# marcinp7/music-style-transfer

Hardware: AMD Instinct MI355X
Metric: style-transfer opt iters/sec (higher is better)
Workload: dtype f32; 1 GPU; one 30 s clip per GPU (BASELINE.json configs[1]): piano-roll C=4,R=16,T=4 (+percussion), full widths (980325 params), fwd+loss+bwd every step, Adam+StepLR every iter_size steps; clips_per_gpu=1, iter_size=2, hip_graph=True, graphs=one joint graph, accumulation=2 concurrent streams, launches_per_pass=77, parallelism=single GPU

## Files before the change

### __graft_entry__.py

```python
import os
import subprocess
import sys

ROOT = os.path.dirname(os.path.abspath(__file__))
PKG = os.path.join(ROOT, 'music-style-transfer_amd')
CSRC = os.path.join(PKG, 'csrc')
BUILD = os.path.join(PKG, 'build')
LIB = os.path.join(PKG, 'libmst_amd.so')
SOURCES = ['gemm', 'lstm', 'combine', 'notes', 'loss_optim', 'plan', 'audio', 'conv', 'lin']
for p in (ROOT, PKG):
    if p not in sys.path:
        sys.path.insert(0, p)


def _hipcc():
    for c in (os.environ.get('HIPCC'), '/opt/rocm/bin/hipcc', 'hipcc'):
        if c and (os.path.isabs(c) and os.path.exists(c) or not os.path.isabs(c)):
            return c
    raise RuntimeError('hipcc not found')


def _stale(target, deps):
    return not os.path.exists(target) or any(os.path.getmtime(d) > os.path.getmtime(target) for d in deps)


def build(force=False):
    os.makedirs(BUILD, exist_ok=True)
    hipcc = _hipcc()
    headers = [os.path.join(CSRC, 'mst_common.h'), os.path.join(ROOT, 'include', 'mst_amd.h')]
    procs, objs = [], []
    for s in SOURCES:
        src, obj = os.path.join(CSRC, s + '.hip'), os.path.join(BUILD, s + '.o')
        objs.append(obj)
        if force or _stale(obj, [src] + headers):
            cmd = [hipcc, '--offload-arch=gfx950', '-O3', '-std=c++17', '-fPIC', '-c', src, '-o', obj]
            procs.append((s, subprocess.Popen(cmd, stdout=subprocess.PIPE, stderr=subprocess.STDOUT)))
    for s, p in procs:
        out, _ = p.communicate()
        if p.returncode:
            raise RuntimeError(f'hipcc failed on {s}.hip:\n{out.decode()}')
    if force or _stale(LIB, objs):
        subprocess.run([hipcc, '--offload-arch=gfx950', '-shared', '-fPIC', '-o', LIB] + objs, check=True)
    import style
    from style import _native
    _native.Native(LIB)


def smoke():
    import numpy as np
    import torch
    from oracle import style_oracle as so
    from tools.synth import synth_clip
    from style import _native as nat
    if not os.path.exists(LIB):
        build()
    assert torch.cuda.is_available(), 'smoke() needs cuda:0'
    dev = torch.device('cuda:0')
    native = nat.get()
    C, R, T = 2, 2, 4
    dims = nat.Dims(C=C, R=R, T=T, beat=64, bar=128, nrf=8, style=256, melody=8, rhythm=32, instr=51,
                    n_instruments=41, has_unpitched=1)
    table = native.param_table(dims)
    g = torch.Generator().manual_seed(0)
    flat = torch.zeros(native.param_floats(dims))
    named = {}
    for name, off, shape in table:
        n = int(np.prod(shape))
        fan = shape[1] if len(shape) > 1 else shape[0]
        flat[off:off + n] = (torch.rand(n, generator=g) * 2 - 1) / fan ** 0.5
        named[name] = flat[off:off + n].view(*shape).clone().requires_grad_(True)
    clip = synth_clip(5, C, R, T, True)
    _, ref_losses = so.iteration(named, clip)
    plan = native.plan(dims, dev)
    plan.set_inputs(mode=clip['mode'], bpm=clip['bpm'], instr=clip['instruments_features'],
                    used=clip['used_instruments'], bpm_target=float(clip['bpm_int']))
    params = flat.to(dev)
    gparams = torch.zeros_like(params)
    losses = torch.zeros(nat.N_LOSSES, device=dev)
    plan.train_iteration(params, gparams, clip['pitched'].to(dev), clip['unpitched'].to(dev), losses)
    torch.cuda.synchronize()
    got = losses.cpu()
    for i, k in enumerate(nat.LOSS_KEYS):
        assert abs(float(got[i]) - ref_losses[k]) < 1e-4, (k, float(got[i]), ref_losses[k])
    gref = torch.cat([(named[n].grad if named[n].grad is not None else torch.zeros_like(named[n])).reshape(-1)
                      for n, _, _ in table])
    err = float((gparams.cpu() - gref).norm() / gref.norm())
    assert err < 1e-4, err
    print(f'smoke ok: total loss {float(got[0]):.6f} (oracle {ref_losses["total"]:.6f}), grad rel-L2 {err:.2e}')


if __name__ == '__main__':
    build()
    print('built', LIB)
```

### include/mst_amd.h

```cpp
#ifndef MST_AMD_H
#define MST_AMD_H
#include <stdint.h>

#ifdef __cplusplus
extern "C" {
#endif

typedef enum {
    MST_OK = 0,
    MST_ERR_ARG = -1,
    MST_ERR_UNSUPPORTED = -2,
    MST_ERR_LAUNCH = -3,
    MST_ERR_ALLOC = -4,
} mst_status;

typedef struct {
    int32_t C, R, T;
    int32_t beat, bar, nrf;
    int32_t style, melody, rhythm;
    int32_t instr;
    int32_t n_instruments;
    int32_t has_unpitched;
    int32_t clips;
} mst_dims;
// ... 39 lines not shown
enum { MST_DEV_OK = 0, MST_DEV_LSTM_TIMEOUT = 1  };
int32_t mst_plan_status(const mst_plan* p, float* ws, int32_t clear, int32_t* status, mst_stream stream);

int32_t mst_forward(const mst_plan* p, int32_t stage_mask, const float* params, float* ws,
                    const float* pitched, const float* unpitched, mst_stream stream);

int32_t mst_backward(const mst_plan* p, int32_t stage_mask, const float* params, float* gparams,
                     float* ws, const float* pitched, const float* unpitched, mst_stream stream);
int32_t mst_zero_grads(const mst_plan* p, int32_t stage_mask, float* ws, mst_stream stream);
int64_t mst_plan_zero_floats(const mst_plan* p, int32_t stage_mask);

#define MST_LOSS_SAVED 512
int64_t mst_loss_scratch_floats(void);
int32_t mst_total_loss_fwd(const float* pitched_pred, const float* pitched_target, int64_t n_pitched_pos,
                           const float* unpitched_pred, const float* unpitched_target, int64_t n_unpitched_pos,
                           const float* instr_logits, const float* instr_target, int32_t n_instr,
                           const float* mode_logits, const float* mode_target,
                           const float* bpm_pred, const float* bpm_target,
                           int32_t normalize, float* losses, float* saved, float* scratch, mst_stream stream);
int32_t mst_total_loss_bwd(const float* pitched_pred, const float* pitched_target, int64_t n_pitched_pos,
                           const float* unpitched_pred, const float* unpitched_target, int64_t n_unpitched_pos,
                           const float* instr_logits, const float* instr_target, int32_t n_instr,
                           const float* mode_logits, const float* mode_target,
                           const float* bpm_pred, const float* bpm_target,
                           const float* saved, const float* grad_losses,
                           float* g_pitched, float* g_unpitched, float* g_instr, float* g_mode, float* g_bpm,
                           mst_stream stream);

int32_t mst_train_iteration(const mst_plan* p, const float* params, float* gparams, float* ws,
                            const float* pitched, const float* unpitched, float* losses, mst_stream stream);

#define MST_MAX_XCHG 8
int32_t mst_tiled_phase_count(const mst_plan* p);
int32_t mst_tiled_phase(const mst_plan* p, int32_t phase, const float* params, float* gparams, float* ws,
                        const float* pitched, const float* unpitched, float* losses, int32_t is_root,
                        mst_stream stream, int64_t xoff[MST_MAX_XCHG], int64_t xlen[MST_MAX_XCHG], int32_t* nx);

int32_t mst_adam_step(float* params, float* grads, float* exp_avg, float* exp_avg_sq, int64_t n,
                      float* state, double lr0, double beta1, double beta2, double eps,
                      int32_t step_size, double gamma, int32_t zero_grad, mst_stream stream);

int32_t mst_adam_step2(float* params, float* grads, float* grads2, float* exp_avg, float* exp_avg_sq, int64_t n,
                       float* state, double lr0, double beta1, double beta2, double eps,
                       int32_t step_size, double gamma, int32_t zero_grad, mst_stream stream);

#define MST_GUARD_WORDS 8
int64_t mst_grad_guard_scratch_bytes(int64_t n);
int32_t mst_grad_norm(const float* grads, const float* grads2 , int64_t n, void* scratch, float* norm,
                      mst_stream stream);
int32_t mst_grad_norms(const float* grads, const float* grads2 , const int64_t* offsets, const int64_t* lengths,
                       int32_t count, float* norms, mst_stream stream);
int32_t mst_adam_step_guarded(float* params, float* grads, float* grads2 , float* exp_avg, float* exp_avg_sq,
                              int64_t n, float* state, float* guard, void* scratch, double lr0, double beta1, double beta2,
                              double eps, int32_t step_size, double gamma, double max_norm ,
                              int32_t skip_nonfinite, int32_t zero_grad, mst_stream stream);

int32_t mst_hard_output(float* x, float* out, int64_t n_pos, int32_t nfeat, mst_stream stream);

int32_t mst_clip_scatter(const int32_t* cells, const float* feats, const int32_t* counts, int32_t capacity, int32_t n_clips,
                         int64_t n_cells, int32_t nfeat, float* out, mst_stream stream);

typedef struct { int32_t first, count, src_bars, r0; } mst_window;
int32_t mst_clip_window(const int32_t* cells, const float* feats, const mst_window* win, int32_t n_clips, int32_t channels,
                        int32_t bars, int64_t bar_cells, int32_t nfeat, float* out, mst_stream stream);

enum { MST_ROLL_NONZERO = 0, MST_ROLL_HARD = 1 };
int64_t mst_roll_slices(int64_t n_cells);
int32_t mst_roll_count(const float* x, int64_t n_cells, int32_t nfeat, int32_t mode, int32_t* ws, mst_stream stream);
int32_t mst_roll_compact(const float* x, int64_t n_cells, int32_t nfeat, int32_t mode, const int32_t* ws,
                         int64_t capacity, int32_t* cells, float* feats, mst_stream stream);

#define MST_METRIC_WORDS 8
int64_t mst_roll_metrics_scratch_bytes(int64_t n_groups, int64_t group_cells);
int32_t mst_roll_metrics(const float* pred, const float* target, int64_t n_groups, int64_t group_cells,
                         int32_t nfeat, void* scratch, double* out, mst_stream stream);

int64_t mst_eval_scratch_bytes(const mst_plan* p);
int32_t mst_eval_iteration(const mst_plan* p, const float* params, float* ws, const float* pitched,
                           const float* unpitched, float* losses, double* metrics, void* scratch, mst_stream stream);

int32_t mst_plan_step_count(const mst_plan* p, int32_t stage_mask, int32_t backward);
int32_t mst_plan_step_info(const mst_plan* p, int32_t stage_mask, int32_t backward, int32_t* info );
int32_t mst_plan_step_carried(const mst_plan* p, int32_t stage_mask, int32_t backward, int32_t* carried);
int32_t mst_plan_step_gemms(const mst_plan* p, int32_t stage_mask, int32_t backward, int32_t step, int32_t* out, int32_t cap);
int32_t mst_plan_time_steps(const mst_plan* p, int32_t stage_mask, int32_t backward, const float* params,
                            float* gparams, float* ws, const float* pitched, const float* unpitched,
                            mst_stream stream, int32_t reps, float* ms, int32_t* kind, double* flops, double* bytes);

typedef struct mst_audio_plan mst_audio_plan;
mst_audio_plan* mst_audio_plan_create(int32_t n_fft , int32_t hop, int64_t n_samples, int32_t* status);
void mst_audio_plan_destroy(mst_audio_plan* p);
int32_t mst_audio_plan_info(const mst_audio_plan* p, int64_t out[6]);
int32_t mst_audio_stft(const mst_audio_plan* p, const float* audio, float* spec, float* mag, mst_stream stream);
int32_t mst_audio_gram(const mst_audio_plan* p, const float* feat, float* gram, float* ws, mst_stream stream);
int32_t mst_audio_style_iteration(const mst_audio_plan* p, float* x, const float* gram_style, float* grad, float* exp_avg,
                                  float* exp_avg_sq, float* state, float* ws, float* loss, double lr, mst_stream stream);

int32_t mst_debug_slab_columns_disjoint(int64_t off_x, int32_t width_x, int64_t off_y, int32_t width_y, int32_t ld);

const char* mst_version(void);

#ifdef __cplusplus
}
#endif
#endif
```

### music-style-transfer_amd/csrc/combine.hip

```cpp
#include "mst_common.h"

template <int MC = COMBINE_MAXC>
__device__ __forceinline__ void block_sum_multi(float* vals, int nv, float (*part)[COMBINE_MAXC + 1], float* red) {
    const int lane = threadIdx.x & 63, wv = threadIdx.x >> 6;
#pragma unroll
    for (int v = 0; v <= MC; ++v) {
        if (v < nv) {
            float x = vals[v];
#pragma unroll
            for (int o = 32; o > 0; o >>= 1) x += __shfl_xor(x, o);
            if (lane == 0) part[wv][v] = x;
        }
    }
    __syncthreads();
    if ((int)threadIdx.x < nv) red[threadIdx.x] = (part[0][threadIdx.x] + part[1][threadIdx.x]) + (part[2][threadIdx.x] + part[3][threadIdx.x]);
    __syncthreads();
}

__device__ __forceinline__ int64_t elem_off(const CombineDesc& d, int e) {
    const unsigned r = (unsigned)e / (unsigned)d.cols;
    return (int64_t)r * d.ld + (int)((unsigned)e - r * (unsigned)d.cols);
}

__global__ __launch_bounds__(256) void combine_sumsq_kernel(const CombineDesc* __restrict__ descs, Bases b) {
    const CombineDesc d = descs[blockIdx.y];
    if ((int)blockIdx.x >= d.nblk) return;
    __shared__ float part[4][COMBINE_MAXC + 1];
    __shared__ float red[COMBINE_MAXC + 1];
    const float* x = b.p[SP_WS] + d.x_off;
    const int64_t n = (int64_t)d.rows * d.cols;
    float acc[COMBINE_MAXC + 1];
#pragma unroll
    for (int c = 0; c <= COMBINE_MAXC; ++c) acc[c] = 0.f;
    for (int e = blockIdx.x * 256 + threadIdx.x; e < (int)n; e += d.nblk * 256) {
        const int64_t eo = elem_off(d, e);
#pragma unroll
        for (int c = 0; c < COMBINE_MAXC; ++c) {
            if (c < d.Cn) { const float v = x[(int64_t)c * d.cs + eo]; acc[c] = fmaf(v, v, acc[c]); }
        }
    }
    block_sum_multi(acc, d.Cn, part, red);
    if ((int)threadIdx.x < d.Cn) b.p[SP_TMP][d.part_off + blockIdx.x * (COMBINE_MAXC + 1) + threadIdx.x] = red[threadIdx.x];
}

__global__ __launch_bounds__(256) void combine_apply_kernel(const CombineDesc* __restrict__ descs, Bases b) {
    const CombineDesc d = descs[blockIdx.y];
    if ((int)blockIdx.x >= d.nblk) return;
    __shared__ float nrm[COMBINE_MAXC + 1];
    __shared__ float part[4][COMBINE_MAXC + 1];
    __shared__ float red[COMBINE_MAXC + 1];
    float* ws = b.p[SP_WS];
    float* tmp = b.p[SP_TMP];
    {
        float vals[COMBINE_MAXC + 1];
#pragma unroll
        for (int c = 0; c <= COMBINE_MAXC; ++c)
            vals[c] = (c < d.Cn && (int)threadIdx.x < d.nblk) ? tmp[d.part_off + threadIdx.x * (COMBINE_MAXC + 1) + c] : 0.f;
        block_sum_multi(vals, d.Cn, part, red);
    }
    if ((int)threadIdx.x < d.Cn) nrm[threadIdx.x] = sqrtf(1.f + red[threadIdx.x]);
    __syncthreads();
    if (threadIdx.x == 0) {
        float S = 0.f;
        for (int c = 0; c < d.Cn; ++c) S += nrm[c];
        nrm[COMBINE_MAXC] = S;
    }
    __syncthreads();
    if (blockIdx.x == 0 && (int)threadIdx.x <= d.Cn)
        tmp[d.stats_off + threadIdx.x] = (int)threadIdx.x < d.Cn ? nrm[threadIdx.x] : nrm[COMBINE_MAXC];
    const float S = nrm[COMBINE_MAXC];
    const int64_t n = (int64_t)d.rows * d.cols;
    for (int e = blockIdx.x * 256 + threadIdx.x; e < (int)n; e += d.nblk * 256) {
        const int64_t eo = elem_off(d, e);
        float acc = 0.f;
        for (int c = 0; c < d.Cn; ++c) acc += ws[d.x_off + (int64_t)c * d.cs + eo] * nrm[c];
        ws[d.out_off + e] = acc / S;
    }
}

__global__ __launch_bounds__(256) void combine_bwd_reduce_kernel(const CombineDesc* __restrict__ descs, Bases b) {
    const CombineDesc d = descs[blockIdx.y];
    if ((int)blockIdx.x >= d.nblk) return;
    __shared__ float part[4][COMBINE_MAXC + 1];
    __shared__ float red[COMBINE_MAXC + 1];
    const float* ws = b.p[SP_WS];
    const float* gr = b.p[SP_GRAD];
    const int64_t n = (int64_t)d.rows * d.cols;
    float acc[COMBINE_MAXC + 1];
#pragma unroll
    for (int c = 0; c <= COMBINE_MAXC; ++c) acc[c] = 0.f;
    for (int e = blockIdx.x * 256 + threadIdx.x; e < (int)n; e += d.nblk * 256) {
        const int64_t eo = elem_off(d, e);
        const float g = gr[d.gout_off + e];
#pragma unroll
        for (int c = 0; c < COMBINE_MAXC; ++c) {
            if (c < d.Cn) acc[c] = fmaf(g, ws[d.x_off + (int64_t)c * d.cs + eo], acc[c]);
        }
        acc[COMBINE_MAXC] = fmaf(g, ws[d.out_off + e], acc[COMBINE_MAXC]);
    }
    float vals[COMBINE_MAXC + 1];
#pragma unroll
    for (int c = 0; c < COMBINE_MAXC; ++c) vals[c] = acc[c];
    vals[COMBINE_MAXC] = 0.f;
#pragma unroll
    for (int c = 0; c <= COMBINE_MAXC; ++c) if (c == d.Cn) vals[c] = acc[COMBINE_MAXC];
    block_sum_multi(vals, d.Cn + 1, part, red);
    if ((int)threadIdx.x <= d.Cn) b.p[SP_TMP][d.part_off + blockIdx.x * (COMBINE_MAXC + 1) + threadIdx.x] = red[threadIdx.x];
}

__global__ __launch_bounds__(256) void combine_bwd_apply_kernel(const CombineDesc* __restrict__ descs, Bases b) {
    const CombineDesc d = descs[blockIdx.y];
    if ((int)blockIdx.x >= d.nblk) return;
    __shared__ float coef[COMBINE_MAXC + 1];
    __shared__ float nc_s[COMBINE_MAXC + 1];
    const float* ws = b.p[SP_WS];
    float* gr = b.p[SP_GRAD];
    const float* tmp = b.p[SP_TMP];
    __shared__ float part[4][COMBINE_MAXC + 1];
    {
        float vals[COMBINE_MAXC + 1];
#pragma unroll
        for (int c = 0; c <= COMBINE_MAXC; ++c)
            vals[c] = (c <= d.Cn && (int)threadIdx.x < d.nblk) ? tmp[d.part_off + threadIdx.x * (COMBINE_MAXC + 1) + c] : 0.f;
        block_sum_multi(vals, d.Cn + 1, part, coef);
    }
    if ((int)threadIdx.x <= d.Cn) nc_s[threadIdx.x] = tmp[d.stats_off + threadIdx.x];
    __syncthreads();
    const float S = nc_s[d.Cn];
    const float bsum = coef[d.Cn];
    __shared__ float fa_s[COMBINE_MAXC], fb_s[COMBINE_MAXC];
    if ((int)threadIdx.x < d.Cn) {
        const float nc = nc_s[threadIdx.x];
        fa_s[threadIdx.x] = nc / S; fb_s[threadIdx.x] = ((coef[threadIdx.x] - bsum) / S) / nc;
    }
    __syncthreads();
    const int64_t n = (int64_t)d.rows * d.cols;
    for (int e = blockIdx.x * 256 + threadIdx.x; e < (int)n; e += d.nblk * 256) {
        const int64_t eo = elem_off(d, e);
        const float g = gr[d.gout_off + e];
        for (int c = 0; c < d.Cn; ++c) {
            const float x = ws[d.x_off + (int64_t)c * d.cs + eo];
            float* gx = gr + d.gx_off + (int64_t)c * d.cs + eo;
            const float v = fmaf(g, fa_s[c], fb_s[c] * x);
            *gx = d.first ? v : *gx + v;
        }
    }
}

template <int MC>
__global__ __launch_bounds__(256) void combine_small_fwd_kernel(const CombineDesc* __restrict__ descs, Bases b) {
    const CombineDesc d = descs[blockIdx.x];
    __shared__ float nrm[COMBINE_MAXC + 1];
    __shared__ float part[4][COMBINE_MAXC + 1];
    __shared__ float red[COMBINE_MAXC + 1];
    float* ws = b.p[SP_WS];
    float* tmp = b.p[SP_TMP];
    const int n = d.rows * d.cols;
    float acc[MC + 1];
#pragma unroll
    for (int c = 0; c <= MC; ++c) acc[c] = 0.f;
    constexpr int U = MC <= 4 ? 4 : 1;
    for (int e0 = threadIdx.x; e0 < n; e0 += 256 * U) {
        float v[U][MC];
#pragma unroll
        for (int u = 0; u < U; ++u) {
            const int e = e0 + 256 * u;
            const bool ok = e < n;
            const int64_t eo = elem_off(d, ok ? e : 0);
#pragma unroll
            for (int c = 0; c < MC; ++c) v[u][c] = (ok && c < d.Cn) ? ws[d.x_off + (int64_t)c * d.cs + eo] : 0.f;
        }
#pragma unroll
        for (int u = 0; u < U; ++u) {
#pragma unroll
            for (int c = 0; c < MC; ++c) acc[c] = fmaf(v[u][c], v[u][c], acc[c]);
        }
    }
    block_sum_multi<MC>(acc, d.Cn, part, red);
    if ((int)threadIdx.x < d.Cn) nrm[threadIdx.x] = sqrtf(1.f + red[threadIdx.x]);
    __syncthreads();
    if (threadIdx.x == 0) {
        float S = 0.f;
        for (int c = 0; c < d.Cn; ++c) S += nrm[c];
        nrm[COMBINE_MAXC] = S;
    }
    __syncthreads();
    if ((int)threadIdx.x <= d.Cn) tmp[d.stats_off + threadIdx.x] = (int)threadIdx.x < d.Cn ? nrm[threadIdx.x] : nrm[COMBINE_MAXC];
    const float S = nrm[COMBINE_MAXC];
    for (int e0 = threadIdx.x; e0 < n; e0 += 256 * U) {
        float v[U][MC];
#pragma unroll
        for (int u = 0; u < U; ++u) {
            const int e = e0 + 256 * u;
            const bool ok = e < n;
            const int64_t eo = elem_off(d, ok ? e : 0);
#pragma unroll
            for (int c = 0; c < MC; ++c) v[u][c] = (ok && c < d.Cn) ? ws[d.x_off + (int64_t)c * d.cs + eo] : 0.f;
        }
#pragma unroll
        for (int u = 0; u < U; ++u) {
            const int e = e0 + 256 * u;
            float a = 0.f;
#pragma unroll
            for (int c = 0; c < MC; ++c) if (c < d.Cn) a += v[u][c] * nrm[c];
            if (e < n) ws[d.out_off + e] = a / S;
        }
    }
}

template <int MC>
__global__ __launch_bounds__(256) void combine_small_bwd_kernel(const CombineDesc* __restrict__ descs, Bases b) {
    const CombineDesc d = descs[blockIdx.x];
    __shared__ float coef[COMBINE_MAXC + 1];
    __shared__ float nc_s[COMBINE_MAXC + 1];
    __shared__ float part[4][COMBINE_MAXC + 1];
    const float* ws = b.p[SP_WS];
    float* gr = b.p[SP_GRAD];
    const float* tmp = b.p[SP_TMP];
    const int n = d.rows * d.cols;
    float acc[MC + 1];
#pragma unroll
    for (int c = 0; c <= MC; ++c) acc[c] = 0.f;
    constexpr int U = MC <= 4 ? 4 : 1;
    for (int e0 = threadIdx.x; e0 < n; e0 += 256 * U) {
        float v[U][MC], g[U], o[U];
#pragma unroll
        for (int u = 0; u < U; ++u) {
            const int e = e0 + 256 * u;
            const bool ok = e < n;
            const int64_t eo = elem_off(d, ok ? e : 0);
            g[u] = ok ? gr[d.gout_off + e] : 0.f;
            o[u] = ok ? ws[d.out_off + e] : 0.f;
#pragma unroll
            for (int c = 0; c < MC; ++c) v[u][c] = (ok && c < d.Cn) ? ws[d.x_off + (int64_t)c * d.cs + eo] : 0.f;
        }
#pragma unroll
        for (int u = 0; u < U; ++u) {
            if (e0 + 256 * u < n) {
#pragma unroll
                for (int c = 0; c < MC; ++c) if (c < d.Cn) acc[c] = fmaf(g[u], v[u][c], acc[c]);
                acc[MC] = fmaf(g[u], o[u], acc[MC]);
            }
        }
    }
    float vals[MC + 1];
#pragma unroll
    for (int c = 0; c < MC; ++c) vals[c] = acc[c];
    vals[MC] = 0.f;
#pragma unroll
    for (int c = 0; c <= MC; ++c) if (c == d.Cn) vals[c] = acc[MC];
    block_sum_multi<MC>(vals, d.Cn + 1, part, coef);
    if ((int)threadIdx.x <= d.Cn) nc_s[threadIdx.x] = tmp[d.stats_off + threadIdx.x];
    __syncthreads();
    const float S = nc_s[d.Cn];
    const float bsum = coef[d.Cn];
    float fa[MC], fb[MC];
#pragma unroll
    for (int c = 0; c < MC; ++c) {
        const float nc = c < d.Cn ? nc_s[c] : 1.f;
        fa[c] = nc / S; fb[c] = c < d.Cn ? ((coef[c] - bsum) / S) / nc : 0.f;
    }
    for (int e0 = threadIdx.x; e0 < n; e0 += 256 * U) {
        float x[U][MC], old[U][MC], g[U];
        int64_t eo[U];
#pragma unroll
        for (int u = 0; u < U; ++u) {
            const int e = e0 + 256 * u;
            const bool ok = e < n;
            eo[u] = elem_off(d, ok ? e : 0);
            g[u] = ok ? gr[d.gout_off + e] : 0.f;
#pragma unroll
            for (int c = 0; c < MC; ++c) {
                const bool okc = ok && c < d.Cn;
                x[u][c] = okc ? ws[d.x_off + (int64_t)c * d.cs + eo[u]] : 0.f;
                old[u][c] = (okc && !d.first) ? gr[d.gx_off + (int64_t)c * d.cs + eo[u]] : 0.f;
            }
        }
#pragma unroll
        for (int u = 0; u < U; ++u) {
            if (e0 + 256 * u < n) {
#pragma unroll
                for (int c = 0; c < MC; ++c) {
                    if (c < d.Cn) {
                        const float v = fmaf(g[u], fa[c], fb[c] * x[u][c]);
                        gr[d.gx_off + (int64_t)c * d.cs + eo[u]] = d.first ? v : old[u][c] + v;
                    }
                }
            }
        }
    }
}

int launch_combine_fwd(const CombineDesc* dev, int count, int max_nblk, int all_small, Bases b, hipStream_t s) {
    if (count <= 0) return 0;
    if (all_small) {
        if (all_small == 2) hipLaunchKernelGGL(combine_small_fwd_kernel<4>, dim3(count), dim3(256), 0, s, dev, b);
        else hipLaunchKernelGGL(combine_small_fwd_kernel<COMBINE_MAXC>, dim3(count), dim3(256), 0, s, dev, b);
        return (int)hipGetLastError();
    }
    hipLaunchKernelGGL(combine_sumsq_kernel, dim3(max_nblk, count), dim3(256), 0, s, dev, b);
    hipLaunchKernelGGL(combine_apply_kernel, dim3(max_nblk, count), dim3(256), 0, s, dev, b);
    return (int)hipGetLastError();
}

int launch_combine_bwd(const CombineDesc* dev, int count, int max_nblk, int all_small, Bases b, hipStream_t s) {
    if (count <= 0) return 0;
    if (all_small) {
        if (all_small == 2) hipLaunchKernelGGL(combine_small_bwd_kernel<4>, dim3(count), dim3(256), 0, s, dev, b);
        else hipLaunchKernelGGL(combine_small_bwd_kernel<COMBINE_MAXC>, dim3(count), dim3(256), 0, s, dev, b);
        return (int)hipGetLastError();
    }
    hipLaunchKernelGGL(combine_bwd_reduce_kernel, dim3(max_nblk, count), dim3(256), 0, s, dev, b);
    hipLaunchKernelGGL(combine_bwd_apply_kernel, dim3(max_nblk, count), dim3(256), 0, s, dev, b);
    return (int)hipGetLastError();
}

int launch_combine_phase(const CombineDesc* dev, int nblk, int which, Bases b, hipStream_t s) {
    if (which == 0) hipLaunchKernelGGL(combine_sumsq_kernel, dim3(nblk, 1), dim3(256), 0, s, dev, b);
    else if (which == 1) hipLaunchKernelGGL(combine_apply_kernel, dim3(nblk, 1), dim3(256), 0, s, dev, b);
    else if (which == 2) hipLaunchKernelGGL(combine_bwd_reduce_kernel, dim3(nblk, 1), dim3(256), 0, s, dev, b);
    else hipLaunchKernelGGL(combine_bwd_apply_kernel, dim3(nblk, 1), dim3(256), 0, s, dev, b);
    return (int)hipGetLastError();
}

__global__ __launch_bounds__(256) void copy_rows_kernel(const CopyDesc* __restrict__ dp, int backward, Bases b) {
    const CopyDesc d = dp[0];
    const int total = d.na * d.nb * d.cols;
    for (int e = blockIdx.x * 256 + threadIdx.x; e < total; e += gridDim.x * 256) {
        const int j = e % d.cols, ab = e / d.cols, bb = ab % d.nb, a = ab / d.nb;
        const int64_t so = d.src_off + (int64_t)a * d.src_sa + (int64_t)bb * d.src_sb + j;
        const int64_t dof = d.dst_off + (int64_t)a * d.dst_sa + (int64_t)bb * d.dst_sb + j;
        if (!backward) b.p[SP_WS][dof] = b.p[SP_WS][so];
        else { float* g = b.p[SP_GRAD] + so; const float v = b.p[SP_GRAD][dof]; *g = d.first ? v : *g + v; }
    }
}

int launch_copy_rows(const CopyDesc* dev, const CopyDesc& host, int backward, Bases b, hipStream_t s) {
    const int total = host.na * host.nb * host.cols;
    int nb = (total + 255) / 256;
    if (nb > 1024) nb = 1024;
    if (nb < 1) return 0;
    hipLaunchKernelGGL(copy_rows_kernel, dim3(nb), dim3(256), 0, s, dev, backward, b);
    return (int)hipGetLastError();
}

__global__ __launch_bounds__(64) void fold_kernel(const FoldDesc* __restrict__ dp, int spread, Bases b) {
    const FoldDesc d = dp[0];
    float* part = b.p[d.space] + d.part_off;
    float* sum = b.p[SP_TMP] + d.sum_off;
    for (int c = threadIdx.x; c < d.ncols; c += 64) {
        if (!spread) {
            float a = 0.f;
            for (int r = 0; r < d.nrows; ++r) a += part[(int64_t)r * d.row_stride + (int64_t)c * d.col_stride];
            sum[c] = a;
        } else {
            part[(int64_t)c * d.col_stride] = sum[c];
            for (int r = 1; r < d.nrows; ++r) part[(int64_t)r * d.row_stride + (int64_t)c * d.col_stride] = 0.f;
        }
    }
}

int launch_fold(const FoldDesc* dev, int spread, Bases b, hipStream_t s) {
    hipLaunchKernelGGL(fold_kernel, dim3(1), dim3(64), 0, s, dev, spread, b);
    return (int)hipGetLastError();
}
```

### music-style-transfer_amd/csrc/gemm.hip

```cpp
#include "mst_common.h"

__device__ __forceinline__ float act_fwd(int act, float z, int col) {
    if (act == ACT_LEAKY) return z > 0.f ? z : z * LEAKY;
    if (act == ACT_SIGOUT) { float s = 1.f / (1.f + expf(-z)); return col == 0 ? 6.f * s : s; }
    if (act == ACT_BPM) { float s = 1.f / (1.f + expf(-z)); return s * 150.f + 50.f; }
    return z;
}

__device__ __forceinline__ float act_bwd(int act, float y, int col) {
    if (act == ACT_LEAKY) return y > 0.f ? 1.f : LEAKY;
    if (act == ACT_SIGOUT) return col == 0 ? y * (1.f - y * (1.f / 6.f)) : y * (1.f - y);
    if (act == ACT_BPM) { float s = (y - 50.f) * (1.f / 150.f); return 150.f * s * (1.f - s); }
    return 1.f;
}

typedef const MST_GLOBAL_AS float* gcptr;
#define GEMM_PAD 1

template <int KIND>
__device__ __forceinline__ int off_of(const Operand& o, int i, int j, bool& ok) {
    if constexpr (KIND == OPK_DENSE) {
        return i * (int)o.si + j * (int)o.sj;
    } else if constexpr (KIND == OPK_ACTGRAD) {
        return o.transposed ? j * o.ld + i : i * o.ld + j;
    } else if constexpr (KIND == OPK_IM2COL) {
        const int p = i >> 3, oc = i & 7;
        const int f = j / (CONV_K * NPF), rem = j - f * (CONV_K * NPF);
        const int e = (NDEG * oc - CONV_PAD) * NPF + rem;
        ok = ok & (e >= 0) & (e < NPN * NPF);
        return p * (NF * NPN * NPF) + f * (NPN * NPF) + e;
    } else if constexpr (KIND == OPK_PERMW) {
        if (o.pb == CONV_K && o.pc == NPF) {
            constexpr int BC = CONV_K * NPF;
            const int a = i / BC, rem = i - a * BC;
            const int bb = rem / NPF, c = rem - bb * NPF;
            return j * o.ld + a * BC + c * CONV_K + bb;
        }
        if (o.pb == NUN && o.pc == NUF) {
            constexpr int BC = NUN * NUF;
            const int a = i / BC, rem = i - a * BC;
            const int bb = rem / NUF, c = rem - bb * NUF;
            return j * o.ld + a * BC + c * NUN + bb;
        }
        const int bc = o.pb * o.pc;
        const int a = i / bc, rem = i - a * bc;
        const int bb = rem / o.pc, c = rem - bb * o.pc;
        return j * o.ld + a * bc + c * o.pb + bb;
    } else {
        return (j >> 3) * (o.oc * NOCT) + i * NOCT + (j & 7);
    }
}

template <int OK>
__device__ __forceinline__ void store_out(const GemmDesc& d, float* cbase, const float* bias, int m, int n, int split, float acc) {
    const OutSpec& o = d.out;
    if constexpr (OK == OUT_STORE) {
        float v = acc;
        if (bias) v += o.bias_div > 0 ? bias[(unsigned)((m / o.bias_div) * o.bias_ld + n)] : bias[n];
        cbase[(unsigned)(m * o.ldc + n)] = act_fwd(o.act, v, n);
    } else if constexpr (OK == OUT_ACCUM) {
        float* c = cbase + (unsigned)(m * o.ldc + n);
        *c = o.first ? acc : *c + acc;
    } else if constexpr (OK == OUT_CONV) {
        cbase[(unsigned)((m >> 3) * o.ldc + n * NOCT + (m & 7))] = act_fwd(ACT_LEAKY, acc + bias[n], 0);
    } else if constexpr (OK == OUT_SLAB) {
        const unsigned idx = n < o.wcols ? (unsigned)(m * o.wcols + n) : (unsigned)(d.M * o.wcols + m);
        cbase[(int64_t)split * o.slab_stride + idx] = acc;
    } else {
        unsigned idx;
        if (n < o.wcols) {
            int a, bb, c, bc;
            if (o.pb == CONV_K && o.pc == NPF) { bc = CONV_K * NPF; a = n / (CONV_K * NPF); const int rem = n - a * (CONV_K * NPF); bb = rem / NPF; c = rem - bb * NPF; }
            else if (o.pb == NUN && o.pc == NUF) { bc = NUN * NUF; a = n / (NUN * NUF); const int rem = n - a * (NUN * NUF); bb = rem / NUF; c = rem - bb * NUF; }
            else { bc = o.pb * o.pc; a = n / bc; const int rem = n - a * bc; bb = rem / o.pc; c = rem - bb * o.pc; }
            idx = (unsigned)(m * o.wcols + a * bc + c * o.pb + bb);
        } else {
            idx = (unsigned)(d.M * o.wcols + m);
        }
        cbase[(int64_t)split * o.slab_stride + idx] = acc;
    }
}

template <int AK, int BKIND, int OK, int AKF, int BKF, int KD>
// ... 449 lines not shown
                for (int kk = 0; kk < MF_KD / 2; ++kk) {
                    const int k = kk * 2 + (lane >> 5);
                    acc = __builtin_amdgcn_mfma_f32_32x32x2f32(As[k][bm * 32 + (lane & 31)], Bs[k][bn * 32 + (lane & 31)], acc, 0, 0, 0);
                }
            } else {
                for (int kk = kk0; kk < min(kk0 + per, live); ++kk) {
                    const int k = kk * 2 + (lane >> 5);
                    acc = __builtin_amdgcn_mfma_f32_32x32x2f32(As[k][bm * 32 + (lane & 31)], Bs[k][bn * 32 + (lane & 31)], acc, 0, 0, 0);
                }
            }
        }
        if (last_k) {
            if (nsl > 1) {
                float* part = smem + buf * 2 * TILE_F;
                MST_LDS_BARRIER();
                if (ks > 0) {
#pragma unroll
                    for (int r = 0; r < 16; ++r) part[((ks - 1) * nblk + blk) * 1024 + r * 64 + lane] = acc[r];
                }
                MST_LDS_BARRIER();
                if (ks == 0) {
                    for (int q = 0; q < nsl - 1; ++q) {
#pragma unroll
                        for (int r = 0; r < 16; ++r) acc[r] += part[(q * nblk + blk) * 1024 + r * 64 + lane];
                    }
                }
            }
            const int n = tn * MF_BN + bn * 32 + (lane & 31);
            if ((ks == 0) & (tm * MF_BM + bm * 32 < M) & (tn * MF_BN + bn * 32 < N)) {
#pragma unroll
                for (int r = 0; r < 16; ++r) {
                    const int m = tm * MF_BM + bm * 32 + (r & 3) + 8 * (r >> 2) + 4 * (lane >> 5);
                    if (m < M && n < N) store_out<OK>(d, cbase, bias, m, n, split, acc[r]);
                }
            }
#pragma unroll
            for (int r = 0; r < 16; ++r) acc[r] = 0.f;
        }
        if (!more) break;
        t = nt; kt = nkt; buf ^= 1;
    }
}

__global__ __launch_bounds__(MF_THREADS, 4) void gemm_mfma_kernel(const GemmDesc* __restrict__ descs, const int* __restrict__ owner, int count, int blocks_per_clip, Bases b) {
    __shared__ float smem[2 * 2 * MF_KD * (MF_BM + GEMM_PAD)];
    float (*As)[MF_BM + GEMM_PAD] = reinterpret_cast<float (*)[MF_BM + GEMM_PAD]>(smem);
    float (*Bs)[MF_BN + GEMM_PAD] = reinterpret_cast<float (*)[MF_BN + GEMM_PAD]>(smem + MF_KD * (MF_BM + GEMM_PAD));
    const int clip = blockIdx.x / blocks_per_clip, lb = blockIdx.x - clip * blocks_per_clip;
    const int lo = owner[lb];
    const GemmDesc d = descs[clip * count + lo];
    const int local = lb - d.blk_begin;
    const int ntile = ((d.M + MF_BM - 1) / MF_BM) * ((d.N + MF_BN - 1) / MF_BN);
    const int run = d.run > 0 ? d.run : 1, nruns = (ntile + run - 1) / run;
    const int split = local / nruns, t_begin = (local - split * nruns) * run, t_end = min(ntile, t_begin + run);
    switch (d.variant) {
    case GV_LIN_FWD: gemm_fast_body<OPK_DENSE, OUT_STORE, 1, 1>(d, b, t_begin, t_end, split, smem); break;
    case GV_LIN_DW: gemm_fast_body<OPK_ACTGRAD, OUT_SLAB, 0, 0>(d, b, t_begin, t_end, split, smem); break;
    case GV_LIN_DW_PERM: gemm_fast_body<OPK_ACTGRAD, OUT_PERMW_SLAB, 0, 0>(d, b, t_begin, t_end, split, smem); break;
    case GV_LIN_DA: gemm_fast_body<OPK_ACTGRAD, OUT_ACCUM, 1, 0>(d, b, t_begin, t_end, split, smem); break;
    case GV_HH_DW: gemm_fast_body<OPK_DENSE, OUT_SLAB, 0, 0>(d, b, t_begin, t_end, split, smem); break;
    case GV_LIN_DA_RAW: gemm_fast_body<OPK_DENSE, OUT_ACCUM, 1, 0>(d, b, t_begin, t_end, split, smem); break;
    default:
        for (int tile = t_begin; tile < t_end; ++tile) {
            if (tile > t_begin) __syncthreads();
            if (d.variant == GV_LIN_FWD_PERM) gemm_mfma_body<OPK_DENSE, OPK_PERMW, OUT_STORE, 1, 1>(d, b, tile, split, As, Bs);
            else if (d.variant == GV_CONV_FWD) gemm_mfma_body<OPK_IM2COL, OPK_PERMW, OUT_CONV, 1, 1>(d, b, tile, split, As, Bs);
            else if (d.variant == GV_CONV_DW) {
                if (d.fold_rows) gemm_mfma_body<OPK_CONVGRAD, OPK_IM2COL, OUT_PERMW_SLAB, 1, 0, true>(d, b, tile, split, As, Bs);
                else gemm_mfma_body<OPK_CONVGRAD, OPK_IM2COL, OUT_PERMW_SLAB, 1, 0>(d, b, tile, split, As, Bs);
            }
        }
        break;
    }
}

int gemm_tile_edge(int mfma) { return mfma ? MF_BM : GEMM_BM; }
int gemm_blocks(const GemmDesc& g, int mfma) {
    const int edge = gemm_tile_edge(mfma);
    const int ntile = ((g.M + edge - 1) / edge) * ((g.N + edge - 1) / edge);
    const int run = (mfma && g.run > 1) ? g.run : 1;
    return ((ntile + run - 1) / run) * g.ksplit;
}

template <int WV> __device__ __forceinline__ void gather_rows(const GatherDesc& d, const int blk, const int nblk, const Bases& b);
__device__ __forceinline__ void segred_group(const SegRedDesc* __restrict__ descs, const int members, const int clip, const int lb, const int t, const Bases& b);

__global__ __launch_bounds__(GEMM_THREADS) void gemm_kernel(const GemmDesc* __restrict__ descs, const int* __restrict__ owner, int count, int blocks_per_clip, Bases b, GemmRiders r) {
    constexpr int TILE_F = GEMM_BK * (GEMM_BM + GEMM_PAD), RED_F = (GEMM_THREADS / 64) * GEMM_BM * GEMM_BN;
    __shared__ float smem[(2 * TILE_F > RED_F) ? 2 * TILE_F : RED_F];
    float (*As)[GEMM_BM + GEMM_PAD] = reinterpret_cast<float (*)[GEMM_BM + GEMM_PAD]>(smem);
    float (*Bs)[GEMM_BN + GEMM_PAD] = reinterpret_cast<float (*)[GEMM_BN + GEMM_PAD]>(smem + TILE_F);
    const int clip = blockIdx.x / blocks_per_clip;
    int lb = blockIdx.x - clip * blocks_per_clip;
    const int seg_blocks = (r.seg_groups + 3) >> 2, gat_blocks = r.gat_members * r.gat_blocks;
    if (lb < seg_blocks) {
        const int grp = lb * 4 + (threadIdx.x >> 8);
        if (grp < r.seg_groups) segred_group(r.segreds, r.seg_members, clip, grp, threadIdx.x & 255, b);
        return;
    }
    lb -= seg_blocks;
    if (lb < gat_blocks) {
        const int m = lb / r.gat_blocks;
        gather_rows<GATHER_RIDER_ROWS>(r.gathers[clip * r.gat_members + m], lb - m * r.gat_blocks, r.gat_blocks, b);
        return;
    }
    lb -= gat_blocks;
    const int lo = owner[lb];
    const GemmDesc d = descs[clip * count + lo];
    const int local = lb - d.blk_begin;
    const int ntile = ((d.M + GEMM_BM - 1) / GEMM_BM) * ((d.N + GEMM_BN - 1) / GEMM_BN);
    const int tile = local % ntile, split = local / ntile;
#define GEMM_CASE(V, A_, B_, O_, AF_, BF_)                                                          \
    case (V) * 3 + 0: gemm_body<A_, B_, O_, AF_, BF_, 32>(d, b, tile, split, As, Bs); break;           \
    case (V) * 3 + 1: gemm_body<A_, B_, O_, AF_, BF_, 64>(d, b, tile, split, As, Bs); break;           \
    case (V) * 3 + 2: gemm_body<A_, B_, O_, AF_, BF_, 128>(d, b, tile, split, As, Bs); break;
    switch (d.variant * 3 + d.kdsel) {
        GEMM_CASE(GV_LIN_FWD, OPK_DENSE, OPK_DENSE, OUT_STORE, 1, 1)
        GEMM_CASE(GV_LIN_FWD_PERM, OPK_DENSE, OPK_PERMW, OUT_STORE, 1, 1)
        GEMM_CASE(GV_LIN_DW, OPK_ACTGRAD, OPK_DENSE, OUT_SLAB, 0, 0)
        GEMM_CASE(GV_LIN_DW_PERM, OPK_ACTGRAD, OPK_DENSE, OUT_PERMW_SLAB, 0, 0)
        GEMM_CASE(GV_LIN_DA, OPK_ACTGRAD, OPK_DENSE, OUT_ACCUM, 1, 0)
        GEMM_CASE(GV_CONV_FWD, OPK_IM2COL, OPK_PERMW, OUT_CONV, 1, 1)
        GEMM_CASE(GV_CONV_DW, OPK_CONVGRAD, OPK_IM2COL, OUT_PERMW_SLAB, 1, 0)
        GEMM_CASE(GV_HH_DW, OPK_DENSE, OPK_DENSE, OUT_SLAB, 0, 0)
        GEMM_CASE(GV_LIN_DA_RAW, OPK_DENSE, OPK_DENSE, OUT_ACCUM, 1, 0)
    default: break;
    }
#undef GEMM_CASE
}

int gemm_variant(const GemmDesc& g) {
    const int a = g.A.kind, bk = g.B.kind, o = g.out.kind;
    if (a == OPK_DENSE && bk == OPK_DENSE && o == OUT_STORE) return GV_LIN_FWD;
    if (a == OPK_DENSE && bk == OPK_PERMW && o == OUT_STORE) return GV_LIN_FWD_PERM;
    if (a == OPK_ACTGRAD && bk == OPK_DENSE && o == OUT_SLAB) return GV_LIN_DW;
    if (a == OPK_ACTGRAD && bk == OPK_DENSE && o == OUT_PERMW_SLAB) return GV_LIN_DW_PERM;
    if (a == OPK_ACTGRAD && bk == OPK_DENSE && o == OUT_ACCUM) return GV_LIN_DA;
    if (a == OPK_IM2COL && bk == OPK_PERMW && o == OUT_CONV) return GV_CONV_FWD;
    if (a == OPK_CONVGRAD && bk == OPK_IM2COL && o == OUT_PERMW_SLAB) return GV_CONV_DW;
    if (a == OPK_DENSE && bk == OPK_DENSE && o == OUT_SLAB) return GV_HH_DW;
    if (a == OPK_DENSE && bk == OPK_DENSE && o == OUT_ACCUM) return GV_LIN_DA_RAW;
    return -1;
}

int gemm_rider_blocks(const GemmRiders& r) { return (r.seg_groups + 3) / 4 + r.gat_members * r.gat_blocks; }

int launch_gemm(const GemmDesc* dev_descs, const int* dev_owner, int members, int blocks_per_clip, int clips, int mfma, Bases b, hipStream_t s, const GemmRiders* riders) {
    if (members <= 0 || blocks_per_clip <= 0 || clips <= 0) return 0;
    GemmRiders r = riders ? *riders : GemmRiders{};
    if (mfma && gemm_rider_blocks(r)) return (int)hipErrorInvalidValue;
    blocks_per_clip += gemm_rider_blocks(r);
    if (mfma) hipLaunchKernelGGL(gemm_mfma_kernel, dim3(blocks_per_clip * clips), dim3(MF_THREADS), 0, s, dev_descs, dev_owner, members, blocks_per_clip, b);
    else hipLaunchKernelGGL(gemm_kernel, dim3(blocks_per_clip * clips), dim3(GEMM_THREADS), 0, s, dev_descs, dev_owner, members, blocks_per_clip, b, r);
    return (int)hipGetLastError();
}

template <int WV>
__device__ __forceinline__ void gather_rows(const GatherDesc& d, const int blk, const int nblk, const Bases& b) {
    const int lane = threadIdx.x & 63, wv = (threadIdx.x >> 6) & (WV - 1);
    for (int row = blk * WV + wv; row < d.rows; row += nblk * WV) {
        unsigned t = (unsigned)row;
        int rc[4];
        rc[3] = t % (unsigned)d.d[3]; t /= (unsigned)d.d[3];
        rc[2] = t % (unsigned)d.d[2]; t /= (unsigned)d.d[2];
        rc[1] = t % (unsigned)d.d[1]; rc[0] = t / (unsigned)d.d[1];
        float* out = b.p[SP_WS] + d.out_off + (int64_t)row * d.K;
        if (d.sum) {
            for (int w = lane; w < d.K; w += 64) {
                float a = 0.f;
                for (int sIdx = 0; sIdx < d.nseg; ++sIdx) {
                    const Seg& sg = d.seg[sIdx];
                    const int srow = rc[0] * sg.s[0] + rc[1] * sg.s[1] + rc[2] * sg.s[2] + rc[3] * sg.s[3];
                    a += b.p[sg.space][sg.off + (int64_t)srow * sg.ld + w];
                }
                out[w] = a;
            }
            continue;
        }
        for (int sIdx = 0; sIdx < d.nseg; ++sIdx) {
            const Seg& sg = d.seg[sIdx];
            const int srow = rc[0] * sg.s[0] + rc[1] * sg.s[1] + rc[2] * sg.s[2] + rc[3] * sg.s[3];
            const float* src = b.p[sg.space] + sg.off + (int64_t)srow * sg.ld;
            for (int w = lane; w < sg.width; w += 64) out[sg.start + w] = src[w];
        }
    }
}

__global__ __launch_bounds__(256) void gather_kernel(const GatherDesc* __restrict__ descs, Bases b) {
    gather_rows<4>(descs[blockIdx.y], blockIdx.x, gridDim.x, b);
}

int launch_gather(const GatherDesc* dev, int count, int max_rows, Bases b, hipStream_t s) {
    if (count <= 0) return 0;
    int gx = (max_rows + 3) / 4;
    if (gx > 2048) gx = 2048;
    hipLaunchKernelGGL(gather_kernel, dim3(gx, count), dim3(256), 0, s, dev, b);
    return (int)hipGetLastError();
}

#define SEGRED_CHUNK 64
template <int E, int R>
__device__ __forceinline__ void segred_body(const SegRedDesc& d, const int item, const Bases& b) {
    const int wgrp = (d.width + E - 1) / E;
    if (item >= d.nidx * d.nchunk * wgrp) return;
    const int w = (item % wgrp) * E, ne = min(E, d.width - w);
    int t = item / wgrp;
    const int chunk = t % d.nchunk, idx = t / d.nchunk;
    int kc[4];
    t = idx;
#pragma unroll
    for (int q = 3; q >= 0; --q) { kc[q] = t % d.kd[q]; t /= d.kd[q]; }
    int rd[4], nred = 1;
#pragma unroll
    for (int q = 0; q < 4; ++q) { rd[q] = d.kd[q] == 1 ? d.d[q] : 1; nred *= rd[q]; }
    const int r_begin = chunk * SEGRED_CHUNK, r_end = min(nred, r_begin + SEGRED_CHUNK);
    int cr[4];
    t = r_begin;
#pragma unroll
    for (int q = 3; q >= 0; --q) { cr[q] = t % rd[q]; t /= rd[q]; }
    const float* src = b.p[SP_GRAD] + d.src_off + d.start + w;
    const float* ysrc = b.p[SP_WS] + d.y_off + d.start + w;
    const int64_t s3 = d.src_ld, s2 = s3 * d.d[3], s1 = s2 * d.d[2], s0 = s1 * d.d[1];
    const int64_t w3 = s2 - rd[3] * s3, w2 = s1 - rd[2] * s2, w1 = s0 - rd[1] * s1;
    int64_t roff = (kc[0] + cr[0]) * s0 + (kc[1] + cr[1]) * s1 + (kc[2] + cr[2]) * s2 + (kc[3] + cr[3]) * s3;
    auto offset = [&]() { return roff; };
    auto advance = [&]() {
        roff += s3;
        if (++cr[3] == rd[3]) { cr[3] = 0; roff += w3; if (++cr[2] == rd[2]) { cr[2] = 0; roff += w2; if (++cr[1] == rd[1]) { cr[1] = 0; roff += w1; ++cr[0]; } } }
    };
    float acc[E];
#pragma unroll
    for (int j = 0; j < E; ++j) acc[j] = 0.f;
    typedef float sr_f4 __attribute__((ext_vector_type(4), aligned(4)));
    auto ldE = [&](const float* p, float (&dst)[E]) {
        if (E == 4 && ne == 4) {
            const sr_f4 t = *reinterpret_cast<const sr_f4*>(p);
// ... 154 lines not shown
```

### music-style-transfer_amd/csrc/mst_common.h

```cpp
#pragma once
#include <hip/hip_runtime.h>
#include <stdint.h>

#include "../../include/mst_amd.h"

#ifndef MST_GLOBAL_AS
#define MST_GLOBAL_AS __attribute__((address_space(1)))
#endif
#ifndef MST_CONST_AS
#define MST_CONST_AS __attribute__((address_space(4)))
#endif
#ifndef MST_UNIFORM
#define MST_UNIFORM(x) __builtin_amdgcn_readfirstlane(x)
#endif
#ifndef MST_FAST_EXP
#define MST_FAST_EXP(x) __expf(x)
#define MST_FAST_RCP(x) __builtin_amdgcn_rcpf(x)
#define MST_PIN(x) asm volatile("" : "+v"(x))
#endif
#ifndef MST_PIN_SGPR
#if defined(__AMDGCN__)
#define MST_PIN_SGPR(p) asm volatile("" : "+s"(p))
#else
#define MST_PIN_SGPR(p) ((void)(p))
// ... 19 lines not shown
#define NUF 2
#define NOCT 8
#define NDEG 7
#define NPN 56
#define NUN 47
#define CONV_K 14
#define CONV_PAD 4
#define LEAKY 0.01f

enum { SP_WS = 0, SP_PAR = 1, SP_GPAR = 2, SP_EXT0 = 3, SP_EXT1 = 4, SP_GRAD = 5, SP_TMP = 6, SP_COUNT = 7 };
enum { MST_BF_LOSS_FUSED = 1,
       MST_BF_ALL_STAGES = 2 };
struct Bases { float* p[SP_COUNT]; int32_t flags; };

enum { ACT_NONE = 0, ACT_LEAKY = 1, ACT_SIGOUT = 2, ACT_BPM = 3 };

enum { OPK_DENSE = 0, OPK_ACTGRAD = 2, OPK_IM2COL = 3, OPK_PERMW = 4, OPK_CONVGRAD = 5 };
#define MAX_SEG 6
struct Seg {
    int32_t space, ld, start, width;
    int64_t off;
    int32_t s[4];
};
struct Operand {
    int32_t kind;
    int32_t space;
    int64_t off;
    int64_t si, sj;
    int32_t ones_at;
    int32_t kfast;
    int32_t space2, ld, act, transposed;
    int64_t off2;
    int32_t oc;
    int32_t pb, pc;
};
enum { OUT_STORE = 0, OUT_ACCUM = 1, OUT_CONV = 2, OUT_SLAB = 3, OUT_PERMW_SLAB = 4 };
struct OutSpec {
    int32_t kind, space, ldc, act;
    int64_t off;
    int32_t bias_space;
    int64_t bias_off;
    int64_t slab_stride;
    int32_t first;
    int32_t wcols;
    int32_t pb, pc;
    int32_t bias_div, bias_ld;
};
struct GemmDesc {
    int32_t M, N, K, ksplit;
    int32_t variant;
    int32_t blk_begin;
    int32_t kdsel;
    int32_t run;
    int32_t fold_rows;
    int64_t acs, acs2, bcs;
    int32_t clip_rows;
    Operand A, B;
    OutSpec out;
};

struct GatherDesc {
    int32_t rows, K, nseg;
    int32_t sum;
    int32_t d[4];
    int64_t out_off;
    Seg seg[MAX_SEG];
};

struct SegRedDesc {
    int64_t src_off; int32_t src_ld; int32_t start, width;
    int64_t dst_off; int32_t dst_ld;
    int32_t d[4];
    int32_t s[4];
    int32_t nidx;
    int32_t kd[4];
    int32_t nchunk;
    int64_t part_off;
    int32_t blk_begin;
    int32_t first;
    int32_t act;
    int64_t y_off;
};

struct GemmRiders {
    const SegRedDesc* segreds; int32_t seg_members, seg_groups;
    const GatherDesc* gathers; int32_t gat_members, gat_blocks;
};

struct LstmDesc {
    int32_t B, S, H, reverse;
    int64_t zx_off;
    int64_t whh_off, bhh_off;
    int64_t out_off; int32_t out_ld;
    int64_t gates_off, c_off, hprev_off;
    int64_t tc_off;
    int64_t gout_off;
    int64_t gzx_off;
    int64_t whht_off;
    int32_t multi;
    int64_t xch_off;
    int64_t status_off;
};
#define LSTM_NB 12
#define LSTM_MH 192
#define LSTM_L2H 256
#define LSTM_WH 1024
static inline int lstm_band(int H) { return H <= 64 ? 0 : (H <= LSTM_L2H ? 1 : 2); }
static inline bool lstm_hidden_supported(int H) { return H >= 1 && H <= LSTM_WH; }

#define COMBINE_MAXC 32
#define COMBINE_MAXBLK 256
#define COMBINE_SMALL 4096
struct CombineDesc {
    int32_t Cn, rows, cols, ld;
    int64_t x_off, cs;
    int64_t out_off;
    int64_t stats_off;
    int64_t part_off;
    int64_t gx_off, gout_off;
    int32_t nblk;
    int32_t first;
};

struct NotesDesc {
    int32_t C, Q;
    int32_t W, CW, ML;
    int64_t oct_off, deg_off;
    int64_t rt_oct_off, rt_deg_off;
    int64_t it_oct_off, it_deg_off;
    int64_t x_off; int32_t x_space;
    int64_t mel_off, g_mel_off;
    int64_t wm_off;
    int64_t ml_off;
    int64_t wc_off, bc_off, wl_off, bl_off;
    int64_t out_off;
    int64_t g_out_off, g_oct_off, g_deg_off, g_ml_off;
    int64_t slab_off; int32_t slab_stride; int32_t nblk;
    int64_t itp_oct_off, itp_deg_off, loss_saved_off, loss_gl_off;
    int32_t fhn;
    int32_t nwc;
    int64_t part_off;
    int64_t stats_off;
};

struct ConvDesc {
    int32_t P, clips, OC, splits;
    int64_t rows_per_split;
    int64_t x1_off, clip_stride;
    int64_t wp_off;
    int64_t w_off, b_off;
    int64_t slab_off, slab_stride;
};
int launch_conv_prep(const ConvDesc& d, Bases b, hipStream_t s);
int launch_conv_fwd(const ConvDesc& d, Bases b, hipStream_t s);
int launch_conv_dw(const ConvDesc& d, Bases b, hipStream_t s);

typedef float mst_f32x16 __attribute__((ext_vector_type(16)));
template <int KT, bool M1 = true, bool N1 = true, int PA = 0, int PB = 0>
__device__ __forceinline__ void mst_mfma_ktile_2x2(const float (*As)[PA], const float (*Bs)[PB], int arow, int bcol, int l31, int kh,
                                                   mst_f32x16 (&acc)[2][2]) {
    float a0[2], a1[2], b0[2], b1[2];
    a0[0] = As[kh][arow + l31]; b0[0] = Bs[kh][bcol + l31];
    if (M1) a1[0] = As[kh][arow + 32 + l31];
    if (N1) b1[0] = Bs[kh][bcol + 32 + l31];
#pragma unroll
    for (int s = 0; s < KT / 2; ++s) {
        const int c = s & 1, n = c ^ 1;
        if (s + 1 < KT / 2) {
            const int k = 2 * (s + 1) + kh;
            a0[n] = As[k][arow + l31]; b0[n] = Bs[k][bcol + l31];
            if (M1) a1[n] = As[k][arow + 32 + l31];
            if (N1) b1[n] = Bs[k][bcol + 32 + l31];
        }
        __builtin_amdgcn_sched_barrier(0);
        acc[0][0] = __builtin_amdgcn_mfma_f32_32x32x2f32(a0[c], b0[c], acc[0][0], 0, 0, 0);
        if (N1) acc[0][1] = __builtin_amdgcn_mfma_f32_32x32x2f32(a0[c], b1[c], acc[0][1], 0, 0, 0);
        if (M1) acc[1][0] = __builtin_amdgcn_mfma_f32_32x32x2f32(a1[c], b0[c], acc[1][0], 0, 0, 0);
        if (M1 && N1) acc[1][1] = __builtin_amdgcn_mfma_f32_32x32x2f32(a1[c], b1[c], acc[1][1], 0, 0, 0);
        __builtin_amdgcn_sched_barrier(0);
    }
}


struct LinDesc {
    int32_t rows, K, N, act, xgrad, clips;
    int32_t x_space, x_ld; int64_t x_off, x_cs;
    int32_t y_ld; int64_t y_off, y_cs;
    int64_t gx_cs;
    int64_t w_off, b_off;
    int64_t slab_off, slab_stride, rows_per_split; int32_t splits;
    int32_t first[2];
};
int launch_lin_fwd(const LinDesc& d, Bases b, hipStream_t s);
int launch_lin_dx(const LinDesc& d, Bases b, int first, hipStream_t s);
int launch_lin_dw(const LinDesc& d, Bases b, hipStream_t s);
int lin_dw_tiles(const LinDesc& d);

struct RowLinDesc {
    int32_t rows, kin, nout, act, xgrad;
    int64_t x_off, y_off;
    int64_t w_off, b_off;
    int64_t slab_off; int32_t slab_stride, nblk;
    int32_t first;
};

struct CopyDesc { int64_t src_off, dst_off; int32_t na, nb, cols, src_sa, src_sb, dst_sa, dst_sb, first; };
struct FoldDesc { int32_t space, nrows, row_stride, ncols, col_stride, pad; int64_t part_off, sum_off ; };
int launch_copy_rows(const CopyDesc* dev, const CopyDesc& host, int backward, Bases b, hipStream_t s);
int launch_fold(const FoldDesc* dev, int spread, Bases b, hipStream_t s);
int launch_combine_phase(const CombineDesc* dev, int nblk, int which, Bases b, hipStream_t s);

struct SlabEntry { int64_t dst, src, stride; int32_t count, splits; int32_t reps; int64_t rep_stride; int32_t width, dst_ld; int32_t single;
                   int64_t base;  };
struct SlabBlock { int32_t entry, start; };

struct Sizes {
    int OC, PCE_IL, H, HB;
    int SE_L, SE_IL, SE_ML, SE_BL;
    int ME_BL, ME_BRL, ME_IL, ME_CW, MEL;
    int RH, PRE_BL, PRE_BRL, PRE_CL, PRE_IL, PRE_ML, PRE_BPL, URE_CL;
    int SIM_BL, NRF, SIM_SI, SIM_RI, SIM_SM, SIM_RM, SIM_SB, SIM_RB, NI;
    int PSA_SL, PSA_RL, PSA_IL, PSA_ML, USA_SL, USA_RL;
    int I, STYLE, BAR;
};
Sizes mst_sizes(const mst_dims& d);

enum { GV_LIN_FWD, GV_LIN_FWD_PERM, GV_LIN_DW, GV_LIN_DW_PERM, GV_LIN_DA, GV_CONV_FWD, GV_CONV_DW, GV_HH_DW, GV_LIN_DA_RAW };
int launch_gather(const GatherDesc* dev, int count, int max_rows, Bases b, hipStream_t s);
int gemm_variant(const GemmDesc& g);
int launch_gemm(const GemmDesc* dev_descs, const int* dev_owner, int members, int blocks_per_clip, int clips, int mfma, Bases b, hipStream_t s,
                const GemmRiders* riders = nullptr);
int gemm_rider_blocks(const GemmRiders& r);
int gemm_tile_edge(int mfma);
int gemm_blocks(const GemmDesc& g, int mfma);
int launch_segred(const SegRedDesc* dev_descs, int members, int blocks_per_clip, int clips, int stage2_blocks, Bases b, hipStream_t s);
int launch_segred2(const SegRedDesc* dev_descs, int count, int stage2_blocks, Bases b, hipStream_t s);
int launch_lstm_transpose(const LstmDesc* dev_descs, int count, int maxH, int multi, Bases b, hipStream_t s);
int launch_lstm_fwd(const LstmDesc* dev_descs, int count, int maxB, int maxH, int multi, Bases b, hipStream_t s);
int launch_lstm_bwd(const LstmDesc* dev_descs, int count, int maxB, int maxH, int multi, Bases b, hipStream_t s);
int lstm_multi_blocks_per_cu();
int launch_combine_fwd(const CombineDesc* dev_descs, int count, int max_nblk, int all_small, Bases b, hipStream_t s);
int launch_combine_bwd(const CombineDesc* dev_descs, int count, int max_nblk, int all_small, Bases b, hipStream_t s);
int launch_me_sumsq(const NotesDesc* dev, const NotesDesc& host, int count, Bases b, hipStream_t s);
int launch_me_notes_fwd(const NotesDesc* dev, const NotesDesc& host, int count, Bases b, hipStream_t s);
int launch_me_bwd_reduce(const NotesDesc* dev, const NotesDesc& host, int count, Bases b, hipStream_t s);
int launch_me_notes_bwd(const NotesDesc* dev, const NotesDesc& host, int count, Bases b, hipStream_t s);
int launch_psa_notes_fwd(const NotesDesc* dev, const NotesDesc& host, int count, Bases b, hipStream_t s);
int launch_psa_notes_bwd(const NotesDesc* dev, const NotesDesc& host, int count, Bases b, hipStream_t s);
int psa_bwd_waves(int C);
struct LossBatch { int32_t clips; int64_t ws, grad, tmp, ext0, ext1; };
int loss_fwd_partials(const float* pp, const float* pt, int64_t np, const float* up, const float* ut, int64_t nu, float* scratch,
                      hipStream_t s);
int loss_fwd_tail(int64_t np, int64_t nu, int has_u, const float* il, const float* it, int ni, const float* mlg, const float* mt,
                  const float* bp, const float* bt, int normalize, float* losses, float* saved, float* scratch, hipStream_t s,
                  float* gl_onehot, float* losses_out);
int loss_blocks(int64_t n);
int loss_fwd_batched(const float* pp, const float* pt, int64_t np, const float* up, const float* ut, int64_t nu, const float* il,
                     const float* it, int ni, const float* mlg, const float* mt, const float* bp, const float* bt, int normalize,
                     float* losses, float* saved, float* scratch, LossBatch lb, hipStream_t s,
                     float* gl_onehot ,
                     float* losses_out );
int loss_bwd_batched(const float* pp, const float* pt, int64_t np, const float* up, const float* ut, int64_t nu, const float* il,
                     const float* it, int ni, const float* mlg, const float* mt, const float* bp, const float* bt,
                     const float* saved, const float* gl, float* gp, float* gu, float* gi, float* gm, float* gb, LossBatch lb,
                     hipStream_t s, float info_scale = 1.f );
int launch_roll_metrics(const float* pred, const float* target, int64_t n_groups, int64_t group_cells, int nfeat, int gpc,
                        int64_t pred_cs, int64_t tgt_cs, void* scratch, hipStream_t s);
struct EvalMetricsArgs {
    const void* part_p; int64_t slices_p, cells_p;
    const void* part_u; int64_t slices_u, cells_u;
    int32_t C, ni;
    const float *il, *it, *mlg, *mt, *bp, *bt;
    int64_t ws_stride;
    double* out;
};
int launch_eval_metrics_finish(const EvalMetricsArgs& a, int clips, hipStream_t s);
bool rowlin_supported(int kin, int nout);
int launch_rowlin_fwd(const RowLinDesc* dev, const RowLinDesc& host, int count, Bases b, hipStream_t s);
int launch_rowlin_bwd(const RowLinDesc* dev, const RowLinDesc& host, int count, Bases b, hipStream_t s);
int launch_slab_reduce(const SlabEntry* dev, const SlabBlock* blocks, int nblocks, Bases b, hipStream_t s);
struct ZeroChunk { int64_t off; int32_t len; int32_t pad; };
int launch_zero(const ZeroChunk* dev, int nchunks, int clips, float* grad_base, int64_t clip_stride, hipStream_t s);
bool notes_widths_supported(int W, int CW, int ML);

#define GEMM_BM 32
#define GEMM_BN 32
#define GEMM_BK 128
#define GEMM_THREADS 1024
#define GATHER_RIDER_ROWS (GEMM_THREADS / 64)
```

### music-style-transfer_amd/csrc/plan.hip

```cpp
#include <cmath>
#include <cstdio>
#include <cstdlib>
#include <cstring>
#include <map>
#include <string>
#include <array>
#include <vector>

#include "mst_common.h"

#define MST_ALIGN_UP(n) (((n) + 63) / 64 * 64)

static int mean_size(double a, double b, double factor = 1.0) { return (int)std::ceil(((a + b) / 2.0) * factor); }

Sizes mst_sizes(const mst_dims& d) {
    Sizes z{};
    z.I = d.instr; z.STYLE = d.style; z.BAR = d.bar; z.H = d.beat; z.HB = d.bar / 2; z.RH = d.rhythm;
    z.MEL = d.melody; z.NRF = d.nrf; z.NI = d.n_instruments;
    z.OC = mean_size(NF * NPF, d.beat);
    z.PCE_IL = mean_size(d.instr, d.beat);
    z.SE_L = mean_size(d.bar, d.style);
    z.SE_IL = mean_size(d.instr, d.style, .25);
    z.SE_ML = mean_size(2, d.style, .1);
    z.SE_BL = mean_size(d.style, 1, .05);
// ... 114 lines not shown
    t.lin(m + ".octave_linear", NPF * 6 * NOCT, z.PSA_SL + z.PSA_RL + z.PSA_IL);
    t.lin(m + ".scale_degree_linear", NPF * 6 * NDEG, z.PSA_SL + z.PSA_RL + z.PSA_IL);
    t.lin(m + ".melody_linear", z.PSA_ML, z.MEL);
    t.lin(m + ".linear", NPF, NPF * 6 + z.PSA_ML);
    m = "unpitched_style_applier";
    t.lin(m + ".style_linear", NF * z.USA_SL, z.STYLE);
    t.lin(m + ".rhythm_linear", z.USA_RL, z.RH);
    t.lin(m + ".notes_linear", NUN * NUF * 4, z.USA_SL + z.USA_RL);
    t.lin(m + ".linear", NUF, NUF * 4);
}

static bool widths_supported(const Sizes& z) {
    for (const int h : {z.H, z.HB, z.SE_L, z.SIM_BL, z.NRF})
        if (!lstm_hidden_supported(h)) return false;
    return notes_widths_supported(z.MEL, z.ME_CW, z.PSA_ML);
}

static bool dims_ok(const mst_dims* d) {
    return d && d->C >= 1 && d->C <= COMBINE_MAXC && d->C <= 24 && d->R >= 1 && d->T >= 1 && d->beat >= 1 && d->bar >= 2 &&
           d->bar % 2 == 0 && d->nrf >= 1 && d->style >= 1 && d->melody >= 1 && d->rhythm >= 1 && d->instr >= 1 &&
           d->n_instruments >= 1 && d->clips >= 0 && d->clips <= 4096;
}

extern "C" int32_t mst_param_count(const mst_dims* d) {
    if (!dims_ok(d)) return MST_ERR_ARG;
    ParamTable t; build_params(*d, mst_sizes(*d), t);
    return (int32_t)t.v.size();
}
extern "C" int64_t mst_param_floats(const mst_dims* d) {
    if (!dims_ok(d)) return MST_ERR_ARG;
    ParamTable t; build_params(*d, mst_sizes(*d), t);
    return t.top;
}
extern "C" int32_t mst_param_info(const mst_dims* d, int32_t i, char* name, int32_t cap, int64_t* off, int32_t* ndim,
                                  int32_t shape[3]) {
    if (!dims_ok(d) || !name || !off || !ndim || !shape) return MST_ERR_ARG;
    ParamTable t; build_params(*d, mst_sizes(*d), t);
    if (i < 0 || i >= (int)t.v.size()) return MST_ERR_ARG;
    const PInfo& p = t.v[i];
    snprintf(name, cap, "%s", p.name.c_str());
    *off = p.off; *ndim = p.ndim;
    for (int k = 0; k < 3; ++k) shape[k] = p.shape[k];
    return MST_OK;
}

struct T { int64_t off; int rows, cols, ld; };
struct SegIn { int space; int64_t off; int ld, width; int s[4]; bool grad; };
enum { K_GEMM, K_GATHER, K_SEGRED, K_LSTM_F, K_LSTM_B, K_COMB_F, K_COMB_B, K_ME_F, K_ME_B, K_PSA_F, K_PSA_B, K_LSTM_T, K_ROW_F, K_ROW_B,
       K_ME_SQ, K_ME_RED,
       K_COMB_F1, K_COMB_F2, K_COMB_B1, K_COMB_B2, K_COPY_F, K_COPY_B, K_FOLD, K_SPREAD, K_XCHG,
       K_GEMM_FOLD,
       K_CONV_P, K_CONV_F, K_CONV_W,
       K_LIN_F, K_LIN_A, K_LIN_W,
       K_COUNT };
enum { F_GEMM, F_GATHER, F_SEGRED, F_LSTM, F_COMB, F_NOTES, F_ROWLIN, F_COPY, F_FOLD, F_XCHG, F_CONV, F_LIN };
struct KindInfo { int kind, fam, sched, per_clip, merge; };
static constexpr KindInfo KINDS[] = {
    {K_GEMM, F_GEMM, 1, 1, 1},     {K_GATHER, F_GATHER, 1, 1, 1}, {K_SEGRED, F_SEGRED, 1, 1, 1}, {K_LSTM_F, F_LSTM, 1, 1, 1},
    {K_LSTM_B, F_LSTM, 1, 1, 1},   {K_COMB_F, F_COMB, 1, 1, 1},   {K_COMB_B, F_COMB, 1, 1, 1},   {K_ME_F, F_NOTES, 1, 1, 0},
    {K_ME_B, F_NOTES, 1, 1, 0},    {K_PSA_F, F_NOTES, 1, 1, 0},   {K_PSA_B, F_NOTES, 1, 1, 0},   {K_LSTM_T, F_LSTM, 1, 1, 1},
    {K_ROW_F, F_ROWLIN, 1, 1, 0},  {K_ROW_B, F_ROWLIN, 1, 1, 0},  {K_ME_SQ, F_NOTES, 1, 1, 0},   {K_ME_RED, F_NOTES, 1, 1, 0},
    {K_COMB_F1, F_COMB, 1, 1, 0},  {K_COMB_F2, F_COMB, 1, 1, 0},  {K_COMB_B1, F_COMB, 1, 1, 0},  {K_COMB_B2, F_COMB, 1, 1, 0},
    {K_COPY_F, F_COPY, 0, 0, 0},   {K_COPY_B, F_COPY, 0, 0, 0},   {K_FOLD, F_FOLD, 0, 0, 0},     {K_SPREAD, F_FOLD, 0, 0, 0},
    {K_XCHG, F_XCHG, 0, 0, 0},     {K_GEMM_FOLD, F_GEMM, 1, 0, 1}, {K_CONV_P, F_CONV, 0, 0, 0},  {K_CONV_F, F_CONV, 0, 0, 0},
    {K_CONV_W, F_CONV, 0, 0, 0},   {K_LIN_F, F_LIN, 0, 0, 0},     {K_LIN_A, F_LIN, 0, 0, 0},     {K_LIN_W, F_LIN, 0, 0, 0}};
static constexpr bool kinds_in_order(int i = 0) { return i == K_COUNT || (KINDS[i].kind == i && kinds_in_order(i + 1)); }
static_assert(sizeof(KINDS) / sizeof(KINDS[0]) == K_COUNT && kinds_in_order(), "KINDS[k] describes step kind k, for every k");

template <class D>
static int up(const std::vector<D>& v, D** dev) {
    *dev = nullptr;
    if (v.empty()) return 0;
    if (hipMalloc((void**)dev, v.size() * sizeof(D)) != hipSuccess) return MST_ERR_ALLOC;
    if (hipMemcpy(*dev, v.data(), v.size() * sizeof(D), hipMemcpyHostToDevice) != hipSuccess) return MST_ERR_ALLOC;
    return 0;
}
template <class D> struct DescTable {
    std::vector<D> host, sched;
    D* dev = nullptr;
    int upload() { return up(sched.empty() ? host : sched, &dev); }
    void release() { hipFree(dev); dev = nullptr; }
};

struct Riders { int seg_first = 0, seg_members = 0, seg_groups = 0, seg_stage2 = 0, gat_first = 0, gat_members = 0, gat_rows = 0; };
struct Step { int kind, first, count, a, b, stage; int c = 0; int lvl = 0; int chain = -1; int signal = -1; int wait[3] = {-1, -1, -1};
              int carried = 0; Riders ride; };
struct Acc { int space; int64_t lo, hi; bool w; bool accum = false, dense = true; };
struct Op { int stage; std::vector<Step> fwd, bwd; };

static int stage_idx(int stage) { return stage == MST_STAGE_EXTRACT ? 0 : stage == MST_STAGE_INFO ? 1 : 2; }

struct mst_plan {
    mst_dims d; Sizes z; ParamTable pt;
    DescTable<GemmDesc> gemms; DescTable<GatherDesc> gathers; DescTable<SegRedDesc> segreds; DescTable<LstmDesc> lstms;
    DescTable<CombineDesc> combines; DescTable<NotesDesc> notes; DescTable<RowLinDesc> rowlins;
    DescTable<ConvDesc> convs; DescTable<LinDesc> lins; DescTable<CopyDesc> copies; DescTable<FoldDesc> folds;
    std::vector<SlabEntry> slabs[3];
    std::vector<Op> ops;
    std::vector<Step> sched[2];
    std::vector<Step> sched_all[2];
    const std::vector<Step>& list(int mask, int backward) const { return mask == MST_STAGE_ALL ? sched_all[backward ? 1 : 0] : sched[backward ? 1 : 0]; }
    std::vector<int> s_gemm_owner; int* d_gemm_owner = nullptr;
    std::map<std::string, T> named;
    int64_t act_top = 0, tmp_top = 0;
    SlabEntry* d_slabs[3] = {nullptr, nullptr, nullptr};
    std::vector<SlabBlock> slab_blocks[3]; SlabBlock* d_slab_blocks[3] = {nullptr, nullptr, nullptr};
    std::vector<SlabEntry> slabs_all; SlabEntry* d_slabs_all = nullptr;
    std::vector<SlabBlock> slab_blocks_all; SlabBlock* d_slab_blocks_all = nullptr;
    bool slabs_all_ok = false;
    T t_losses, t_saved, t_gl; int64_t loss_scratch = 0;
    std::vector<ZeroChunk> zero_stage[3], zero_all;
    ZeroChunk* d_zero_stage[3] = {nullptr, nullptr, nullptr}; ZeroChunk* d_zero_all = nullptr;
    int err = 0;
    mst_plan_options opt{};
    int mfma = 0;

    bool tiled() const { return opt.tile_rows > 0; }
    bool mixes() const { return !mfma && !tiled() && opt.branches != 1 && !opt.no_merge; }
    int Rl() const { return tiled() ? opt.tile_rows : d.R; }
    int P() const { return d.C * Rl() * d.T; }
    int Q() const { return Rl() * d.T; }
    struct Xchg { int space; int64_t off; int32_t len; };
    std::vector<Xchg> xchgs;
    bool tags_in_zero = false;
    std::vector<ZeroChunk> zero_fwd; ZeroChunk* d_zero_fwd = nullptr;
    int64_t loss_sum_off = 0;
    int loss_fold[2] = {-1, -1};
    struct Phase { int what; int pass; int begin, end; int nx; int xchg[MST_MAX_XCHG]; };
    std::vector<Phase> phases;
    int K() const { return d.clips > 1 ? d.clips : 1; }
    static int device_cus() {
#ifdef HIPSIM
        return 16;
#else
        int dev = 0, cus = 0;
        if (hipGetDevice(&dev) != hipSuccess || hipDeviceGetAttribute(&cus, hipDeviceAttributeMultiprocessorCount, dev) != hipSuccess) return 0;
        return cus;
#endif
    }
    static int coresident_slots() {
        const int per_cu = lstm_multi_blocks_per_cu();
        return per_cu > 1 ? (per_cu - 1) * device_cus() : 0;
    }
    int64_t status_off = 0;
    enum { N_SIDE = 3, N_SETS = 4, N_EVENTS = 96 };
    struct SideSet { hipStream_t owner = nullptr; bool used = false; hipStream_t side[N_SIDE] = {}; hipEvent_t ev_fork = nullptr, ev_join[N_SIDE] = {}, ev[N_EVENTS] = {}; };
    mutable SideSet sides[N_SETS];
    bool branches = false;
    SideSet* side_set(hipStream_t main) const {
        for (SideSet& q : sides) if (q.used && q.owner == main) return &q;
        hipStreamCaptureStatus cs = hipStreamCaptureStatusNone;
        if (hipStreamIsCapturing(main, &cs) != hipSuccess || cs != hipStreamCaptureStatusNone) return nullptr;
        for (SideSet& q : sides) {
            if (q.used) continue;
            bool ok = hipEventCreateWithFlags(&q.ev_fork, hipEventDisableTiming) == hipSuccess;
            for (int i = 0; i < N_SIDE; ++i)
                ok = ok && hipStreamCreateWithFlags(&q.side[i], hipStreamNonBlocking) == hipSuccess &&
                     hipEventCreateWithFlags(&q.ev_join[i], hipEventDisableTiming) == hipSuccess;
            for (int i = 0; i < n_signals; ++i) ok = ok && hipEventCreateWithFlags(&q.ev[i], hipEventDisableTiming) == hipSuccess;
            if (!ok) return nullptr;
            q.used = true; q.owner = main;
            return &q;
        }
        return nullptr;
    }
    int64_t ext0_stride() const { return (int64_t)P() * NF * NPN * NPF; }
    int64_t ext1_stride() const { return (int64_t)Q() * NF * NUN * NUF; }
    int64_t shift(int space, int k) const {
        switch (space) {
        case SP_WS: case SP_GRAD: return (int64_t)k * act_top;
        case SP_TMP: return (int64_t)k * tmp_top;
        case SP_EXT0: return (int64_t)k * ext0_stride();
        case SP_EXT1: return (int64_t)k * ext1_stride();
        default: return 0;
        }
    }
    GemmDesc reloc(GemmDesc g, int k) const {
        for (Operand* o : {&g.A, &g.B}) {
            o->off += shift(o->space, k);
            if (o->kind == OPK_ACTGRAD || o->kind == OPK_CONVGRAD) o->off2 += shift(o->space2, k);
        }
        g.out.off += shift(g.out.space, k);
        if (g.out.bias_space >= 0) g.out.bias_off += shift(g.out.bias_space, k);
        return g;
    }
    GatherDesc reloc(GatherDesc g, int k) const {
        g.out_off += shift(SP_WS, k);
        for (int i = 0; i < g.nseg; ++i) g.seg[i].off += shift(g.seg[i].space, k);
        return g;
    }
    SegRedDesc reloc(SegRedDesc r, int k) const {
        r.src_off += shift(SP_GRAD, k); r.dst_off += shift(SP_GRAD, k); r.part_off += shift(SP_TMP, k); r.y_off += shift(SP_WS, k);
        return r;
    }
    LstmDesc reloc(LstmDesc l, int k) const {
        const int64_t a = shift(SP_WS, k), t = shift(SP_TMP, k);
        l.zx_off += a; l.out_off += a; l.gout_off += a; l.gzx_off += a;
        l.gates_off += t; l.c_off += t; l.hprev_off += t; l.tc_off += t; l.xch_off += t;
        return l;
    }
    CombineDesc reloc(CombineDesc c, int k) const {
        const int64_t a = shift(SP_WS, k), t = shift(SP_TMP, k);
        c.x_off += a; c.out_off += a; c.gx_off += a; c.gout_off += a; c.stats_off += t; c.part_off += t;
        return c;
    }
    RowLinDesc reloc(RowLinDesc r, int k) const {
        r.x_off += shift(SP_WS, k); r.y_off += shift(SP_WS, k); r.slab_off += shift(SP_TMP, k);
// ... 924 lines not shown
    for (int i = 0; i < n; ++i) {
        accesses(seq[i], acc[i]);
        for (int j = 0; j < i; ++j)
            if (level[j] >= level[i] && conflicts(acc[i], acc[j])) level[i] = level[j] + 1;
        if (level[i] > maxlevel) maxlevel = level[i];
    }
    std::vector<char> done(n, 0);
    for (int lv = 0; lv <= maxlevel; ++lv) {
        const size_t lv_begin = out.size();
        for (int i = 0; i < n; ++i) {
            if (done[i] || level[i] != lv) continue;
            const Step& s0 = seq[i];
            const KindInfo& ki = KINDS[s0.kind];
            const bool mergeable = !opt.no_merge && ki.merge, is_lstm = ki.fam == F_LSTM;
            Step m = s0; m.count = 0; m.lvl = lv;
            std::vector<int> members;
            for (int j = i; j < n; ++j) {
                if (done[j] || level[j] != lv) continue;
                const Step& s = seq[j];
                if (s.kind != s0.kind || (!across_stages && s.stage != s0.stage)) continue;
                if (is_lstm && lstm_band(s.b) != lstm_band(s0.b)) continue;
                if (is_lstm && j != i && (lstms.host[s.first].multi || lstms.host[s0.first].multi)) continue;
                if (j != i && !mergeable) continue;
                done[j] = 1;
                for (int q = 0; q < s.count; ++q) members.push_back(s.first + q);
                m.stage |= s.stage;
                if (s.a > m.a) m.a = s.a;
                if (s.b > m.b) m.b = s.b;
            }
            const bool shared_T = s0.kind == K_LSTM_T && !lstms.host[s0.first].multi;
            const int reps = ki.per_clip && !shared_T ? K() : 1;
            if (ki.sched)
                with_sched_table(ki.fam, [&](auto& t) {
                    m.first = (int)t.sched.size();
                    for (int k = 0; k < reps; ++k)
                        for (int idx : members) t.sched.push_back(reloc(t.host[idx], k));
                });
            m.count = (int)members.size() * reps;
            if (ki.fam == F_GEMM) {
                for (int q = 0; q < m.count; ++q) {
                    GemmDesc& g = gemms.sched[m.first + q];
                    g.variant = gemm_variant(g);
                    if (g.fold_rows) {
                        g.acs = shift(g.A.space, 1); g.acs2 = (g.A.kind == OPK_ACTGRAD || g.A.kind == OPK_CONVGRAD) ? shift(g.A.space2, 1) : 0; g.bcs = shift(g.B.space, 1);
                        if ((uint64_t)std::max(g.acs, std::max(g.acs2, g.bcs)) * (uint64_t)K() > 0xFFFFFFFFull) err = MST_ERR_UNSUPPORTED;
                    }
                    if (g.clip_rows) {
                        g.M = K();
                        if (g.A.kind == OPK_DENSE) g.A.si = shift(g.A.space, 1);
                        else g.A.ld = (int32_t)shift(g.A.space, 1);
                        g.out.ldc = (int32_t)shift(g.out.space, 1);
                        if ((uint64_t)act_top * (uint64_t)K() > 0x7FFFFFFFull) err = MST_ERR_UNSUPPORTED;
                    }
                    const int kr = (g.K + g.ksplit - 1) / g.ksplit;
                    g.kdsel = kr <= 32 ? 0 : (kr <= 64 ? 1 : 2);
                    g.run = (mfma && opt.gemm_run > 1) ? opt.gemm_run : 1;
                    if (g.variant < 0) err = MST_ERR_UNSUPPORTED;
                }
                const int nm = (int)members.size();
                int total = 0;
                m.c = (int)s_gemm_owner.size();
                for (int q = 0; q < nm; ++q) {
                    const int nb = gemm_blocks(gemms.sched[m.first + q], mfma);
                    for (int k = 0; k < reps; ++k) gemms.sched[m.first + k * nm + q].blk_begin = total;
                    total += nb;
                    s_gemm_owner.insert(s_gemm_owner.end(), nb, q);
                }
                m.a = total; m.b = nm;
            }
            if (m.kind == K_SEGRED) {
                const int nm = (int)members.size();
                int total = 0;
                for (int q = 0; q < nm; ++q) {
                    const SegRedDesc& r0 = segreds.sched[m.first + q];
                    for (int k = 0; k < reps; ++k) segreds.sched[m.first + k * nm + q].blk_begin = total;
                    total += (r0.nidx * r0.nchunk * r0.width + 255) / 256;
                }
                m.a = total;
            }
            out.push_back(m);
        }
        if (!mixes()) continue;
        for (size_t e = lv_begin; e < out.size(); ++e) {
            if (out[e].kind != K_GATHER && out[e].kind != K_SEGRED) continue;
            for (size_t c = lv_begin; c < out.size(); ++c) {
                Step& g = out[c];
                if (g.kind != K_GEMM || (!across_stages && g.stage != out[e].stage)) continue;
                const Step& s = out[e];
                if (s.kind == K_GATHER && !g.ride.gat_members) { g.ride.gat_first = s.first; g.ride.gat_members = s.count / K(); g.ride.gat_rows = s.a; }
                else if (s.kind == K_SEGRED && !g.ride.seg_members) { g.ride.seg_first = s.first; g.ride.seg_members = s.count / K(); g.ride.seg_groups = s.a; g.ride.seg_stage2 = s.b; }
                else continue;
                out[e].carried = 1;
                break;
            }
        }
    }
}

static bool covered(const std::vector<Acc>& have, int64_t lo, int64_t hi) {
    int64_t at = lo;
    bool moved = true;
    while (at < hi && moved) {
        moved = false;
        for (const Acc& a : have)
            if (a.lo <= at && a.hi > at) { at = a.hi; moved = true; }
    }
    return at >= hi;
}
static bool touches(const std::vector<Acc>& have, int64_t lo, int64_t hi) {
    for (const Acc& a : have) if (a.lo < hi && lo < a.hi) return true;
    return false;
}

void mst_plan::first_writers(std::vector<Step>& list, size_t begin, bool per_stage, std::vector<Acc>& zero) {
    std::vector<Acc> have;
    auto external = [&](const char* name) {
        auto it = named.find(name);
        if (it != named.end()) have.push_back(Acc{SP_GRAD, it->second.off, it->second.off + MST_ALIGN_UP((int64_t)it->second.rows * it->second.cols), true});
    };
    for (const char* nm : {"pitched_pred", "unpitched_pred", "instruments_pred", "mode_pred", "bpm_pred"}) external(nm);
    if (per_stage) for (const char* nm : {"style", "melody", "rhythm"}) external(nm);
    for (size_t si = begin; si < list.size(); ++si) {
        Step& m = list[si];
        const int reps = KINDS[m.kind].per_clip ? K() : 1, nm = m.count / reps;
        for (int q = 0; q < nm; ++q) {
            std::vector<Acc> acc;
            Step one = m; one.first = m.first + q; one.count = 1;
            accesses(one, acc, true);
            for (const Acc& a : acc) {
                if (a.space != SP_GRAD || a.w) continue;
                if (!covered(have, a.lo, a.hi)) { Acc z = a; z.w = true; z.space = m.stage; zero.push_back(z); have.push_back(a); }
            }
            int first = 0;
            bool accum = false;
            for (const Acc& a : acc) {
                if (a.space != SP_GRAD || !a.w) continue;
                if (!a.accum) { if (a.dense) have.push_back(a); continue; }
                accum = true;
                if (a.dense && !touches(have, a.lo, a.hi)) { first = 1; have.push_back(a); }
                else if (!covered(have, a.lo, a.hi)) { Acc z = a; z.space = m.stage; zero.push_back(z); have.push_back(a); }
            }
            if (!accum) continue;
            for (int k = 0, idx = m.first + q; k < reps; ++k, idx += nm) {
                switch (KINDS[m.kind].fam) {
                case F_GEMM: gemms.sched[idx].out.first = first; break;     case F_SEGRED: segreds.sched[idx].first = first; break;
                case F_COMB: combines.sched[idx].first = first; break;      case F_ROWLIN: rowlins.sched[idx].first = first; break;
                case F_COPY: copies.host[idx].first = first; break;         case F_LIN: lins.host[idx].first[per_stage ? 0 : 1] = first; break;
                }
            }
        }
    }
}

bool mst_plan::assign_streams(std::vector<Step>& L) {
    const int n = (int)L.size(), NS = 1 + N_SIDE;
    std::vector<std::vector<Acc>> acc(n);
    for (int i = 0; i < n; ++i) accesses(L[i], acc[i], true);
    auto dur = [&](const Step& st) {
        switch (st.kind) {
        case K_LSTM_F: case K_LSTM_B: return lstms.sched[st.first].multi ? 30.0 : 15.0;
        case K_ME_F: case K_ME_B: case K_PSA_F: case K_PSA_B: return 18.0;
        case K_GEMM: case K_GEMM_FOLD: return st.count > 8 ? 10.0 : 5.0;
        case K_SEGRED: return 9.0;
        default: return 5.0;
        }
    };
    const double EDGE_IN = 2.0, EDGE_X = 6.0;
    std::vector<double> fin(n, 0.0);
    std::vector<int> str(n, 0);
    double ready[1 + N_SIDE] = {};
    std::vector<std::array<int, 1 + N_SIDE>> clock(n);
    int tail[1 + N_SIDE]; for (int q = 0; q < NS; ++q) tail[q] = -1;
    for (int i = 0; i < n; ++i) {
        std::vector<int> preds;
        for (int j = 0; j < i; ++j) if (conflicts(acc[i], acc[j])) preds.push_back(j);
        int best = 0; double best_start = 1e30;
        for (int q = 0; q < NS; ++q) {
            double start = ready[q];
            for (int j : preds) start = std::max(start, fin[j] + (str[j] == q ? 0.0 : EDGE_X));
            if (start < best_start - 1e-9) { best_start = start; best = q; }
        }
        const int q = best;
        str[i] = q; L[i].chain = q;
        fin[i] = best_start + dur(L[i]) + EDGE_IN; ready[q] = fin[i];
        std::array<int, 1 + N_SIDE> ck; ck.fill(-1);
        if (tail[q] >= 0) { ck = clock[tail[q]]; ck[q] = tail[q]; }
        int need[1 + N_SIDE]; for (int r = 0; r < NS; ++r) need[r] = -1;
        for (int j : preds) if (str[j] != q && j > ck[str[j]]) need[str[j]] = std::max(need[str[j]], j);
        int nw = 0;
        for (int r = 0; r < NS; ++r) {
            if (need[r] < 0) continue;
            const int j = need[r];
            if (L[j].signal < 0) { if (n_signals >= N_EVENTS) return false; L[j].signal = n_signals++; }
            L[i].wait[nw++] = L[j].signal;
            for (int t = 0; t < NS; ++t) ck[t] = std::max(ck[t], clock[j][t]);
            ck[r] = std::max(ck[r], j);
        }
        clock[i] = ck; tail[q] = i;
    }
    for (int i = 0; i < n; ++i)
        for (int j = 0; j < i; ++j)
            if (conflicts(acc[i], acc[j]) && !(str[j] == str[i] || clock[i][str[j]] >= j)) return false;
    return true;
}

void mst_plan::schedule() {
    mfma = opt.gemm_tile == 64 ? 1 : (opt.gemm_tile == 32 ? 0 : (K() >= 6));
    std::vector<Step> fwd, bwd;
    for (auto& op : ops) for (auto s : op.fwd) { s.stage = op.stage; fwd.push_back(s); }
    for (size_t i = ops.size(); i-- > 0;) for (auto s : ops[i].bwd) { s.stage = ops[i].stage; bwd.push_back(s); }
    schedule_pass(fwd, sched[0], false);
    schedule_pass(bwd, sched[1], false);
    branches = opt.branches == 1 && !tiled();
    schedule_pass(fwd, sched_all[0], true);
    schedule_pass(bwd, sched_all[1], true);
    std::vector<Acc> zs, za;
    first_writers(sched[1], 0, true, zs);
    first_writers(sched_all[1], 0, false, za);
    if (branches && !(assign_streams(sched_all[0]) && assign_streams(sched_all[1]))) {
        branches = false;
        for (int ps = 0; ps < 2; ++ps) for (Step& st : sched_all[ps]) { st.chain = -1; st.signal = -1; st.wait[0] = st.wait[1] = st.wait[2] = -1; }
    }
    auto chunks = [&](const std::vector<Acc>& z, int stage_mask, std::vector<ZeroChunk>& out) {
        for (const Acc& a : z) {
            if (!(a.space & stage_mask)) continue;
            for (int64_t at = a.lo; at < a.hi; at += 16384) out.push_back(ZeroChunk{at, (int32_t)std::min<int64_t>(16384, a.hi - at), 0});
        }
    };
    for (int st = 0; st < 3; ++st) chunks(zs, 1 << st, zero_stage[st]);
    chunks(za, MST_STAGE_ALL, zero_all);
    if (K() == 1)
        for (const LstmDesc& l : lstms.host)
            if (l.multi) { zero_all.push_back(ZeroChunk{act_top + l.xch_off, (int32_t)(2 * (2 * l.H + 8 * l.H)), 0}); tags_in_zero = true; }
    if (!tiled()) return;
    {
        const bool U = d.has_unpitched != 0;
        loss_sum_off = tmp(16);
        const int64_t np = (int64_t)P() * NF * NPN, nu = U ? (int64_t)Q() * NF * NUN : 0;
        FoldDesc f{}; f.space = SP_TMP; f.part_off = loss_scratch; f.nrows = loss_blocks(np); f.row_stride = 8; f.ncols = 7; f.col_stride = 1;
        f.sum_off = loss_sum_off;
        loss_fold[0] = (int)folds.host.size(); folds.host.push_back(f);
        f.part_off = loss_scratch + (mst_loss_scratch_floats() - 64) / 2; f.nrows = U ? loss_blocks(nu) : 1; f.sum_off = loss_sum_off + 8;
        loss_fold[1] = (int)folds.host.size(); folds.host.push_back(f);
    }
    auto mk = [](int what, int pass, int begin, int end) { Phase ph{}; ph.what = what; ph.pass = pass; ph.begin = begin; ph.end = end; ph.nx = 0; return ph; };
    auto split = [&](int pass) {
        const std::vector<Step>& L = sched_all[pass];
        int begin = 0;
        Phase cur = mk(0, pass, 0, 0);
        auto touches_pending = [&](const Step& st) {
            if (!cur.nx) return false;
            std::vector<Acc> acc;
            accesses(st, acc, true);
            for (int q = 0; q < cur.nx; ++q) {
                const Xchg& x = xchgs[cur.xchg[q]];
                for (const Acc& a : acc)
                    if (a.space == x.space && a.lo < x.off + x.len && x.off < a.hi) return true;
            }
            return false;
        };
        for (int i = 0; i < (int)L.size(); ++i) {
            const bool is_x = L[i].kind == K_XCHG;
            if ((is_x && cur.nx == MST_MAX_XCHG) || (!is_x && touches_pending(L[i]))) {
                cur.begin = begin; cur.end = i;
                phases.push_back(cur);
                begin = i; cur = mk(0, pass, 0, 0);
            }
            if (is_x) cur.xchg[cur.nx++] = L[i].first;
        }
        cur.begin = begin; cur.end = (int)L.size();
        phases.push_back(cur);
    };
    split(0);
    const int lx = (int)xchgs.size();
    xchgs.push_back(Xchg{SP_TMP, loss_sum_off, 16});
    { Phase ph = mk(1, 0, 0, 0); ph.nx = 1; ph.xchg[0] = lx; phases.push_back(ph); }
    phases.push_back(mk(2, 0, 0, 0));
    split(1);
}

static bool slab_columns_disjoint(int64_t off_x, int width_x, int64_t off_y, int width_y, int ld) {
    const int64_t cx = off_x % ld, cy = off_y % ld;
    if (cx + width_x > ld || cy + width_y > ld) return false;
    return cx + width_x <= cy || cy + width_y <= cx;
}
extern "C" int32_t mst_debug_slab_columns_disjoint(int64_t off_x, int32_t width_x, int64_t off_y, int32_t width_y, int32_t ld) {
    return slab_columns_disjoint(off_x, width_x, off_y, width_y, ld) ? 1 : 0;
}

int mst_plan::upload() {
    int e = 0;
    e |= gemms.upload(); e |= gathers.upload(); e |= segreds.upload(); e |= lstms.upload();
    e |= combines.upload(); e |= notes.upload(); e |= rowlins.upload();
    e |= up(s_gemm_owner, &d_gemm_owner);
    e |= copies.upload(); e |= folds.upload(); e |= up(zero_fwd, &d_zero_fwd);
    for (int st = 0; st < 3; ++st) e |= up(zero_stage[st], &d_zero_stage[st]);
    e |= up(zero_all, &d_zero_all);
    for (int s = 0; s < 3; ++s) {
        for (auto& ent : slabs[s]) { ent.reps = ent.single ? 1 : K(); ent.rep_stride = tmp_top; }
        e |= up(slabs[s], &d_slabs[s]);
        for (size_t i = 0; i < slabs[s].size(); ++i)
            for (int st = 0; st < slabs[s][i].count; st += 64) slab_blocks[s].push_back(SlabBlock{(int)i, st});
        e |= up(slab_blocks[s], &d_slab_blocks[s]);
    }
    {
        std::vector<std::pair<int64_t, int64_t>> spans;
        for (int s = 0; s < 3; ++s)
            for (auto& ent : slabs[s]) {
                const int64_t hi = ent.width > 0 ? ent.dst + (int64_t)(ent.count / ent.width - 1) * ent.dst_ld + ent.width : ent.dst + ent.count;
                spans.push_back({ent.dst, hi});
                slabs_all.push_back(ent);
            }
        slabs_all_ok = true;
        for (size_t i = 0; i < slabs_all.size() && slabs_all_ok; ++i)
            for (size_t j = i + 1; j < slabs_all.size() && slabs_all_ok; ++j) {
                const SlabEntry& x = slabs_all[i]; const SlabEntry& y = slabs_all[j];
                if (spans[i].second <= spans[j].first || spans[j].second <= spans[i].first) continue;
                slabs_all_ok = x.width > 0 && y.width > 0 && x.dst_ld == y.dst_ld && x.base == y.base &&
                               slab_columns_disjoint(x.dst - x.base, x.width, y.dst - y.base, y.width, x.dst_ld);
            }
        for (size_t i = 0; i < slabs_all.size(); ++i)
            for (int st = 0; st < slabs_all[i].count; st += 64) slab_blocks_all.push_back(SlabBlock{(int)i, st});
        e |= up(slabs_all, &d_slabs_all);
        e |= up(slab_blocks_all, &d_slab_blocks_all);
    }
    return e ? MST_ERR_ALLOC : MST_OK;
}

extern "C" int32_t mst_widths_supported(const mst_dims* d) {
    if (!dims_ok(d)) return MST_ERR_ARG;
    return widths_supported(mst_sizes(*d)) ? MST_OK : MST_ERR_UNSUPPORTED;
}

extern "C" mst_plan* mst_plan_create(const mst_dims* d, int32_t* status) { return mst_plan_create_ex(d, nullptr, status); }

extern "C" mst_plan* mst_plan_create_ex(const mst_dims* d, const mst_plan_options* opt, int32_t* status) {
    int32_t dummy; if (!status) status = &dummy;
    if (!dims_ok(d)) { *status = MST_ERR_ARG; return nullptr; }
    if (opt && ((opt->gemm_tile != 0 && opt->gemm_tile != 32 && opt->gemm_tile != 64) || opt->gemm_run < 0 || opt->gemm_run > 64)) { *status = MST_ERR_ARG; return nullptr; }
    if (opt && (opt->lstm_flavour < 0 || opt->lstm_flavour > 2 || opt->dense_flavour < 0 || opt->dense_flavour > 2 || opt->branches < 0 || opt->branches > 1)) { *status = MST_ERR_ARG; return nullptr; }
    if (opt && (opt->tile_rows < 0 || opt->tile_r0 < 0 || (opt->tile_rows > 0 && (opt->tile_r0 + opt->tile_rows > d->R || d->clips > 1)))) {
        *status = MST_ERR_ARG; return nullptr;
    }
    mst_plan* p = new mst_plan();
    if (opt) p->opt = *opt;
    p->d = *d; p->z = mst_sizes(*d);
    if (p->d.clips < 1) p->d.clips = 1;
    build_params(*d, p->z, p->pt);
    p->build();
    if (!p->err) p->schedule();
    if (p->err) { *status = p->err; delete p; return nullptr; }
    int e = p->upload();
    if (e) { *status = e; mst_plan_destroy(p); return nullptr; }
    *status = MST_OK;
    return p;
}

extern "C" void mst_plan_destroy(mst_plan* p) {
    if (!p) return;
    p->gemms.release(); p->gathers.release(); p->segreds.release(); p->lstms.release(); p->combines.release(); p->notes.release();
    p->rowlins.release(); p->copies.release(); p->folds.release();
    hipFree(p->d_gemm_owner); hipFree(p->d_zero_all); hipFree(p->d_zero_fwd);
    for (int st = 0; st < 3; ++st) hipFree(p->d_zero_stage[st]);
    for (int s = 0; s < 3; ++s) { hipFree(p->d_slabs[s]); hipFree(p->d_slab_blocks[s]); }
    hipFree(p->d_slabs_all); hipFree(p->d_slab_blocks_all);
    for (mst_plan::SideSet& q : p->sides) {
        if (q.ev_fork) hipEventDestroy(q.ev_fork);
        for (int i = 0; i < mst_plan::N_SIDE; ++i) { if (q.ev_join[i]) hipEventDestroy(q.ev_join[i]); if (q.side[i]) hipStreamDestroy(q.side[i]); }
        for (hipEvent_t e : q.ev) if (e) hipEventDestroy(e);
    }
    delete p;
}

extern "C" int64_t mst_plan_workspace_floats(const mst_plan* p) { return p ? (int64_t)p->K() * (2 * p->act_top + p->tmp_top) : MST_ERR_ARG; }

extern "C" int32_t mst_plan_gemm_tile(const mst_plan* p) { return p ? (p->mfma ? 64 : 32) : MST_ERR_ARG; }

extern "C" int32_t mst_plan_layout(const mst_plan* p, int64_t out[4]) {
    if (!p || !out) return MST_ERR_ARG;
    out[0] = p->K(); out[1] = p->act_top; out[2] = p->tmp_top; out[3] = (int64_t)p->K() * p->act_top;
    return MST_OK;
}

extern "C" int32_t mst_plan_tensor(const mst_plan* p, const char* name, int64_t* off, int64_t* goff, int64_t* numel) {
    if (!p || !name) return MST_ERR_ARG;
    auto it = p->named.find(name);
    if (it == p->named.end()) return MST_ERR_ARG;
    if (off) *off = it->second.off;
    if (goff) *goff = (int64_t)p->K() * p->act_top + it->second.off;
    if (numel) *numel = (int64_t)it->second.rows * it->second.cols;
    return MST_OK;
}

extern "C" int32_t mst_plan_launch_count(const mst_plan* p, int32_t mask, int32_t backward) {
    if (!p) return MST_ERR_ARG;
    int n = 0;
    for (auto& s : p->list(mask, backward)) {
        if (!(s.stage & mask)) continue;
        const int stage2 = (((s.kind == K_COMB_F || s.kind == K_COMB_B) && s.b != 0) || (s.kind == K_SEGRED && s.b > 0)) ? 1 : 0;
        n += (s.carried ? 0 : 1) + stage2;
    }
    if (backward) for (int s = 0; s < 3; ++s) if ((mask >> s) & 1) n += 1;
    return n;
}

static Bases make_bases(const mst_plan* p, const float* params, float* gparams, float* ws, const float* pitched,
                        const float* unpitched) {
    Bases b;
    b.p[SP_WS] = ws; b.p[SP_PAR] = const_cast<float*>(params); b.p[SP_GPAR] = gparams;
    b.p[SP_EXT0] = const_cast<float*>(pitched); b.p[SP_EXT1] = const_cast<float*>(unpitched);
    b.p[SP_GRAD] = ws + (int64_t)p->K() * p->act_top; b.p[SP_TMP] = ws + 2 * (int64_t)p->K() * p->act_top;
    b.flags = 0;
    return b;
}

static int run_step(const mst_plan* p, const Step& s, const Bases& b, hipStream_t st) {
    if (s.carried) return 0;
    switch (s.kind) {
    case K_GEMM: case K_GEMM_FOLD: {
        const Riders& q = s.ride;
        const int clips = s.count / s.b, gat_blocks = std::min(512, (q.gat_rows + GATHER_RIDER_ROWS - 1) / GATHER_RIDER_ROWS);
        const GemmRiders r{p->segreds.dev + q.seg_first, q.seg_members, q.seg_groups, p->gathers.dev + q.gat_first, q.gat_members, gat_blocks};
        const int e = launch_gemm(p->gemms.dev + s.first, p->d_gemm_owner + s.c, s.b, s.a, clips, p->mfma, b, st, &r);
        return e ? e : launch_segred2(p->segreds.dev + q.seg_first, q.seg_members * clips, q.seg_stage2, b, st);
    }
    case K_GATHER: return launch_gather(p->gathers.dev + s.first, s.count, s.a, b, st);
    case K_SEGRED: return launch_segred(p->segreds.dev + s.first, s.count / p->K(), s.a, p->K(), s.b, b, st);
    case K_LSTM_T: return launch_lstm_transpose(p->lstms.dev + s.first, s.count, s.b, p->lstms.sched[s.first].multi, b, st);
    case K_LSTM_F: return launch_lstm_fwd(p->lstms.dev + s.first, s.count, s.a, s.b, p->lstms.sched[s.first].multi, b, st);
    case K_LSTM_B: return launch_lstm_bwd(p->lstms.dev + s.first, s.count, s.a, s.b, p->lstms.sched[s.first].multi, b, st);
    case K_COMB_F: return launch_combine_fwd(p->combines.dev + s.first, s.count, s.a, s.b == 0 ? (p->d.C <= 4 ? 2 : 1) : 0, b, st);
    case K_COMB_B: return launch_combine_bwd(p->combines.dev + s.first, s.count, s.a, s.b == 0 ? (p->d.C <= 4 ? 2 : 1) : 0, b, st);
    case K_COMB_F1: return launch_combine_phase(p->combines.dev + s.first, s.a, 0, b, st);
    case K_COMB_F2: return launch_combine_phase(p->combines.dev + s.first, s.a, 1, b, st);
    case K_COMB_B1: return launch_combine_phase(p->combines.dev + s.first, s.a, 2, b, st);
    case K_COMB_B2: return launch_combine_phase(p->combines.dev + s.first, s.a, 3, b, st);
    case K_COPY_F: return launch_copy_rows(p->copies.dev + s.first, p->copies.host[s.first], 0, b, st);
    case K_COPY_B: return launch_copy_rows(p->copies.dev + s.first, p->copies.host[s.first], 1, b, st);
    case K_FOLD: return launch_fold(p->folds.dev + s.first, 0, b, st);
    case K_SPREAD: return launch_fold(p->folds.dev + s.first, 1, b, st);
    case K_XCHG: return MST_ERR_UNSUPPORTED;
    case K_LIN_F: case K_LIN_A: case K_LIN_W: {
        LinDesc l = p->lins.host[s.first];
        l.x_cs = p->shift(l.x_space, 1); l.y_cs = p->act_top; l.gx_cs = p->act_top;
        if (s.kind == K_LIN_F) return launch_lin_fwd(l, b, st);
        if (s.kind == K_LIN_W) return launch_lin_dw(l, b, st);
        return launch_lin_dx(l, b, l.first[(b.flags & MST_BF_ALL_STAGES) ? 1 : 0], st);
    }
    case K_CONV_P: { ConvDesc c = p->convs.host[s.first]; c.clip_stride = p->act_top; return launch_conv_prep(c, b, st); }
    case K_CONV_F: { ConvDesc c = p->convs.host[s.first]; c.clip_stride = p->act_top; return launch_conv_fwd(c, b, st); }
    case K_CONV_W: { ConvDesc c = p->convs.host[s.first]; c.clip_stride = p->act_top; return launch_conv_dw(c, b, st); }
    case K_ROW_F: return launch_rowlin_fwd(p->rowlins.dev + s.first, p->rowlins.sched[s.first], s.count, b, st);
    case K_ROW_B: return launch_rowlin_bwd(p->rowlins.dev + s.first, p->rowlins.sched[s.first], s.count, b, st);
    case K_ME_SQ: return launch_me_sumsq(p->notes.dev + s.first, p->notes.sched[s.first], s.count, b, st);
    case K_ME_RED: return launch_me_bwd_reduce(p->notes.dev + s.first, p->notes.sched[s.first], s.count, b, st);
    case K_ME_F: return launch_me_notes_fwd(p->notes.dev + s.first, p->notes.sched[s.first], s.count, b, st);
    case K_ME_B: return launch_me_notes_bwd(p->notes.dev + s.first, p->notes.sched[s.first], s.count, b, st);
    case K_PSA_F: return launch_psa_notes_fwd(p->notes.dev + s.first, p->notes.sched[s.first], s.count, b, st);
    case K_PSA_B: return launch_psa_notes_bwd(p->notes.dev + s.first, p->notes.sched[s.first], s.count, b, st);
    }
    return MST_ERR_ARG;
}

static int run_pass(const mst_plan* p, const std::vector<Step>& list, int mask, const Bases& b0, hipStream_t main, bool tags_cleared = false) {
    Bases b = b0;
    if (mask == MST_STAGE_ALL) b.flags |= MST_BF_ALL_STAGES;
    auto runs = [&](const Step& s) {
        if (!(s.stage & mask)) return false;
        if (tags_cleared && s.kind == K_LSTM_T && p->lstms.sched[s.first].multi) return false;
        return true;
    };
    mst_plan::SideSet* ss = (p->branches && mask == MST_STAGE_ALL) ? p->side_set(main) : nullptr;
    bool forked = false, used[mst_plan::N_SIDE] = {};
    for (auto& s : list) {
        if (!runs(s)) continue;
        hipStream_t st = main;
        if (ss) {
            if (s.chain > 0) {
                const int c = s.chain - 1;
                if (!forked) { if (hipEventRecord(ss->ev_fork, main) != hipSuccess) return MST_ERR_LAUNCH; forked = true; }
                if (!used[c]) { if (hipStreamWaitEvent(ss->side[c], ss->ev_fork, 0) != hipSuccess) return MST_ERR_LAUNCH; used[c] = true; }
                st = ss->side[c];
            }
            for (int w = 0; w < 3; ++w)
                if (s.wait[w] >= 0 && hipStreamWaitEvent(st, ss->ev[s.wait[w]], 0) != hipSuccess) return MST_ERR_LAUNCH;
        }
        int e = run_step(p, s, b, st);
        if (e) return e < 0 ? e : MST_ERR_LAUNCH;
        if (ss && s.signal >= 0 && hipEventRecord(ss->ev[s.signal], st) != hipSuccess) return MST_ERR_LAUNCH;
    }
    if (ss)
        for (int c = 0; c < mst_plan::N_SIDE; ++c)
            if (used[c] && (hipEventRecord(ss->ev_join[c], ss->side[c]) != hipSuccess || hipStreamWaitEvent(main, ss->ev_join[c], 0) != hipSuccess)) return MST_ERR_LAUNCH;
    return MST_OK;
}

extern "C" int32_t mst_forward(const mst_plan* p, int32_t mask, const float* params, float* ws, const float* pitched,
                               const float* unpitched, mst_stream stream) {
    if (!p || !params || !ws) return MST_ERR_ARG;
    if ((mask & MST_STAGE_EXTRACT) && (!pitched || (p->d.has_unpitched && !unpitched))) return MST_ERR_ARG;
    const Bases b = make_bases(p, params, nullptr, ws, pitched, unpitched);
    return run_pass(p, p->list(mask, 0), mask, b, (hipStream_t)stream);
}

extern "C" int32_t mst_plan_status(const mst_plan* p, float* ws, int32_t clear, int32_t* status, mst_stream stream) {
    if (!p || !ws || !status) return MST_ERR_ARG;
    if (hipStreamSynchronize((hipStream_t)stream) != hipSuccess) return MST_ERR_LAUNCH;
    int32_t word = 0;
    if (hipMemcpy(&word, ws + p->status_off, sizeof(word), hipMemcpyDeviceToHost) != hipSuccess) return MST_ERR_LAUNCH;
    *status = word;
    if (clear && word) {
        const int32_t zero = 0;
        if (hipMemcpy(ws + p->status_off, &zero, sizeof(zero), hipMemcpyHostToDevice) != hipSuccess) return MST_ERR_LAUNCH;
    }
    return MST_OK;
}

extern "C" int32_t mst_zero_grads(const mst_plan* p, int32_t mask, float* ws, mst_stream stream) {
    if (!p || !ws) return MST_ERR_ARG;
    float* g = ws + (int64_t)p->K() * p->act_top;
    if ((mask & MST_STAGE_ALL) == MST_STAGE_ALL)
        return launch_zero(p->d_zero_all, (int)p->zero_all.size(), p->K(), g, p->act_top, (hipStream_t)stream) ? MST_ERR_LAUNCH : MST_OK;
    for (int s = 0; s < 3; ++s) {
        if (!((mask >> s) & 1)) continue;
        if (launch_zero(p->d_zero_stage[s], (int)p->zero_stage[s].size(), p->K(), g, p->act_top, (hipStream_t)stream)) return MST_ERR_LAUNCH;
    }
    return MST_OK;
}

static int32_t backward_impl(const mst_plan* p, int32_t mask, const float* params, float* gparams, float* ws,
                             const float* pitched, const float* unpitched, mst_stream stream, int32_t flags) {
    if (!p || !params || !gparams || !ws) return MST_ERR_ARG;
    if ((mask & MST_STAGE_EXTRACT) && (!pitched || (p->d.has_unpitched && !unpitched))) return MST_ERR_ARG;
    Bases b = make_bases(p, params, gparams, ws, pitched, unpitched);
    b.flags = flags;
    {
        int e = run_pass(p, p->list(mask, 1), mask, b, (hipStream_t)stream);
        if (e) return e;
    }
    if ((mask & MST_STAGE_ALL) == MST_STAGE_ALL && p->slabs_all_ok)
        return launch_slab_reduce(p->d_slabs_all, p->d_slab_blocks_all, (int)p->slab_blocks_all.size(), b, (hipStream_t)stream) ? MST_ERR_LAUNCH : MST_OK;
    for (int s = 2; s >= 0; --s) {
        if (!((mask >> s) & 1)) continue;
        if (launch_slab_reduce(p->d_slabs[s], p->d_slab_blocks[s], (int)p->slab_blocks[s].size(), b, (hipStream_t)stream))
            return MST_ERR_LAUNCH;
    }
    return MST_OK;
}

extern "C" int32_t mst_backward(const mst_plan* p, int32_t mask, const float* params, float* gparams, float* ws,
                                const float* pitched, const float* unpitched, mst_stream stream) {
    return backward_impl(p, mask, params, gparams, ws, pitched, unpitched, stream, 0);
}

extern "C" int32_t mst_train_iteration(const mst_plan* p, const float* params, float* gparams, float* ws,
                                       const float* pitched, const float* unpitched, float* losses, mst_stream stream) {
    if (!p || !params || !gparams || !ws || !pitched) return MST_ERR_ARG;
    hipStream_t st = (hipStream_t)stream;
    int e = mst_zero_grads(p, MST_STAGE_ALL, ws, stream);
    if (e) return e;
    if (p->d.has_unpitched && !unpitched) return MST_ERR_ARG;
    e = run_pass(p, p->list(MST_STAGE_ALL, 0), MST_STAGE_ALL, make_bases(p, params, nullptr, ws, pitched, unpitched), st, p->tags_in_zero);
    if (e) return e;
    const bool U = p->d.has_unpitched != 0;
    const int K = p->K();
    float* g = ws + (int64_t)K * p->act_top;
    auto at = [&](const char* n) { return p->named.at(n).off; };
    const int64_t np = (int64_t)p->P() * NF * NPN, nu = U ? (int64_t)p->Q() * NF * NUN : 0;
    float* lscratch = ws + 2 * (int64_t)K * p->act_top + p->loss_scratch;
    const LossBatch lb = {K, p->act_top, p->act_top, p->tmp_top, p->ext0_stride(), p->ext1_stride()};
    e = loss_fwd_batched(ws + at("pitched_pred"), pitched, np, U ? ws + at("unpitched_pred") : nullptr, U ? unpitched : nullptr,
                         nu, ws + at("instruments_pred"), ws + at("used_instruments"), p->z.NI, ws + at("mode_pred"),
                         ws + at("mode"), ws + at("bpm_pred"), ws + at("bpm_target"), 1, ws + p->t_losses.off,
                         ws + p->t_saved.off, lscratch, lb, st, ws + p->t_gl.off, losses);
    if (e) return e;
    e = loss_bwd_batched(ws + at("pitched_pred"), pitched, np, U ? ws + at("unpitched_pred") : nullptr, U ? unpitched : nullptr,
                         nu, ws + at("instruments_pred"), ws + at("used_instruments"), p->z.NI, ws + at("mode_pred"),
                         ws + at("mode"), ws + at("bpm_pred"), ws + at("bpm_target"), ws + p->t_saved.off,
                         ws + p->t_gl.off, nullptr ,
                         U ? g + at("unpitched_pred") : nullptr,
                         g + at("instruments_pred"), g + at("mode_pred"), g + at("bpm_pred"), lb, st);
    if (e) return e;
    e = backward_impl(p, MST_STAGE_ALL, params, gparams, ws, pitched, unpitched, stream, MST_BF_LOSS_FUSED);
    if (e) return e;
    return hipGetLastError() == hipSuccess ? MST_OK : MST_ERR_LAUNCH;
}

static int64_t eval_slices(const mst_plan* p, bool pitched) {
    return mst_roll_slices(pitched ? (int64_t)p->Q() * NF * NPN : (int64_t)p->Q() * NF * NUN);
}

extern "C" int64_t mst_eval_scratch_bytes(const mst_plan* p) {
    if (!p) return MST_ERR_ARG;
    if (p->tiled()) return MST_ERR_UNSUPPORTED;
    return 32 * (int64_t)p->K() * ((int64_t)p->d.C * eval_slices(p, true) + (p->d.has_unpitched ? eval_slices(p, false) : 0));
}

extern "C" int32_t mst_eval_iteration(const mst_plan* p, const float* params, float* ws, const float* pitched,
                                      const float* unpitched, float* losses, double* metrics, void* scratch, mst_stream stream) {
    if (!p || !params || !ws || !pitched || !metrics || !scratch || ((uintptr_t)metrics & 7) || ((uintptr_t)scratch & 7)) return MST_ERR_ARG;
    if (p->tiled()) return MST_ERR_UNSUPPORTED;
    if (p->d.has_unpitched && !unpitched) return MST_ERR_ARG;
    hipStream_t st = (hipStream_t)stream;
    int e = run_pass(p, p->list(MST_STAGE_ALL, 0), MST_STAGE_ALL, make_bases(p, params, nullptr, ws, pitched, unpitched), st);
    if (e) return e;
    const bool U = p->d.has_unpitched != 0;
    const int K = p->K(), C = p->d.C;
    auto at = [&](const char* n) { return p->named.at(n).off; };
    const int64_t np = (int64_t)p->P() * NF * NPN, nu = U ? (int64_t)p->Q() * NF * NUN : 0;
    float* lscratch = ws + 2 * (int64_t)K * p->act_top + p->loss_scratch;
    const LossBatch lb = {K, p->act_top, p->act_top, p->tmp_top, p->ext0_stride(), p->ext1_stride()};
    e = loss_fwd_batched(ws + at("pitched_pred"), pitched, np, U ? ws + at("unpitched_pred") : nullptr, U ? unpitched : nullptr,
                         nu, ws + at("instruments_pred"), ws + at("used_instruments"), p->z.NI, ws + at("mode_pred"),
                         ws + at("mode"), ws + at("bpm_pred"), ws + at("bpm_target"), 1, ws + p->t_losses.off,
                         ws + p->t_saved.off, lscratch, lb, st, ws + p->t_gl.off, losses);
    if (e) return e;
    EvalMetricsArgs a{};
    a.part_p = scratch; a.slices_p = eval_slices(p, true); a.cells_p = np / C;
    e = launch_roll_metrics(ws + at("pitched_pred"), pitched, (int64_t)K * C, a.cells_p, NPF, C, p->act_top, p->ext0_stride(), scratch, st);
    if (e) return e;
    if (U) {
        void* su = (char*)scratch + 32 * (int64_t)K * C * a.slices_p;
        a.part_u = su; a.slices_u = eval_slices(p, false); a.cells_u = nu;
        e = launch_roll_metrics(ws + at("unpitched_pred"), unpitched, K, nu, NUF, 1, p->act_top, p->ext1_stride(), su, st);
        if (e) return e;
    }
    a.C = C; a.ni = p->z.NI;
    a.il = ws + at("instruments_pred"); a.it = ws + at("used_instruments"); a.mlg = ws + at("mode_pred"); a.mt = ws + at("mode");
    a.bp = ws + at("bpm_pred"); a.bt = ws + at("bpm_target"); a.ws_stride = p->act_top; a.out = metrics;
    return launch_eval_metrics_finish(a, K, st);
}


extern "C" int32_t mst_tiled_phase_count(const mst_plan* p) { return p ? (int32_t)p->phases.size() : MST_ERR_ARG; }

extern "C" int32_t mst_tiled_phase(const mst_plan* p, int32_t phase, const float* params, float* gparams, float* ws,
                                   const float* pitched, const float* unpitched, float* losses, int32_t is_root,
                                   mst_stream stream, int64_t* xoff, int64_t* xlen, int32_t* nx) {
    if (!p || !p->tiled() || phase < 0 || phase >= (int)p->phases.size() || !params || !gparams || !ws || !pitched || !xoff || !xlen || !nx)
        return MST_ERR_ARG;
    hipStream_t st = (hipStream_t)stream;
    const mst_plan::Phase& ph = p->phases[phase];
    Bases b = make_bases(p, params, gparams, ws, pitched, unpitched);
    b.flags |= MST_BF_ALL_STAGES;
    const bool U = p->d.has_unpitched != 0;
// ... 54 lines not shown
        }
        break;
    case K_GATHER:
        for (int i = 0; i < s.count; ++i) { const GatherDesc& g = p->gathers.sched[s.first + i]; b += 8.0 * g.rows * g.K; }
        break;
    case K_LIN_F: case K_LIN_A: case K_LIN_W: {
        const LinDesc& l = p->lins.host[s.first];
        const double rows = (double)l.clips * l.rows;
        f = 2.0 * rows * l.N * l.K;
        b = 4.0 * (rows * l.K + rows * l.N * (s.kind == K_LIN_F ? 1.0 : 2.0) + (double)l.N * l.K);
        break;
    }
    case K_CONV_F: case K_CONV_W: {
        const ConvDesc& c = p->convs.host[s.first];
        const double rows = (double)c.clips * c.P * NOCT, kk = NF * NPF * CONV_K;
        f = 2.0 * rows * c.OC * kk;
        b = 4.0 * (rows / NOCT * NF * NPN * NPF + rows * c.OC * (s.kind == K_CONV_F ? 1.0 : 2.0) + c.OC * kk);
        break;
    }
    case K_SEGRED:
        for (int i = 0; i < s.count; ++i) {
            const SegRedDesc& r = p->segreds.sched[s.first + i];
            const double rows = (double)r.d[0] * r.d[1] * r.d[2] * r.d[3];
            f += rows * r.width; b += 4.0 * (rows * r.width + 2.0 * r.nidx * r.width);
        }
        break;
    case K_LSTM_F: case K_LSTM_B:
        for (int i = 0; i < s.count; ++i) {
            const LstmDesc& l = p->lstms.sched[s.first + i];
            f += (double)l.B * l.S * (8.0 * l.H * l.H + 30.0 * l.H);
            b += 4.0 * ((double)l.B * l.S * 11.0 * l.H + 4.0 * l.H * l.H);
        }
        break;
    case K_COMB_F: case K_COMB_B:
        for (int i = 0; i < s.count; ++i) {
            const CombineDesc& c = p->combines.sched[s.first + i];
            const double n = (double)c.rows * c.cols;
            f += n * c.Cn * (s.kind == K_COMB_F ? 4.0 : 8.0);
            b += 4.0 * n * (s.kind == K_COMB_F ? 2.0 * c.Cn + 1 : 4.0 * c.Cn + 2);
        }
        break;
    case K_ROW_F: case K_ROW_B:
        for (int i = 0; i < s.count; ++i) {
            const RowLinDesc& r = p->rowlins.sched[s.first + i];
            const double mm = 2.0 * r.rows * r.kin * r.nout;
            f += s.kind == K_ROW_F ? mm : 2.0 * mm;
            b += 4.0 * r.rows * (s.kind == K_ROW_F ? r.kin + r.nout : 2.0 * r.kin + 2.0 * r.nout + (r.xgrad ? r.kin : 0));
        }
        break;
    case K_ME_SQ: case K_ME_F: case K_ME_RED: case K_ME_B: {
        const NotesDesc& n = p->notes.sched[s.first];
        const double pos = (double)n.C * n.Q * NF * NPN * s.count, mel = pos / n.C * n.W;
        const double per = 2.0 * n.W + 2.0 * n.CW * NPF + 2.0 * n.W * (n.W + n.CW);
        if (s.kind == K_ME_SQ) { f = pos * (per + 2.0 * n.W); b = 4.0 * pos * NPF; }
        else if (s.kind == K_ME_F) { f = pos * 2.0 * n.W; b = 4.0 * (pos * NPF + mel); }
        else if (s.kind == K_ME_RED) { f = pos * 2.0 * n.W; b = 4.0 * (pos * NPF + 2.0 * mel); }
        else { f = pos * per * 2.0; b = 4.0 * (pos * NPF + mel); }
        break;
    }
    case K_PSA_F: case K_PSA_B: {
        const NotesDesc& n = p->notes.sched[s.first];
        const double pos = (double)n.C * n.Q * NF * NPN * s.count;
        const double per = 2.0 * 30 + 2.0 * NPF * (30 + n.ML);
        f = pos * per * (s.kind == K_PSA_F ? 1.0 : 3.0);
        b = 4.0 * (pos * NPF * (s.kind == K_PSA_F ? 1.0 : 2.0) + (double)s.count * n.C * n.Q * NF * 450 * (s.kind == K_PSA_F ? 1.0 : 2.0) +
                   (double)s.count * n.Q * NF * NPN * n.ML * (s.kind == K_PSA_F ? 1.0 : 2.0));
        break;
    }
    }
    *flops = f; *bytes = b;
}

extern "C" int64_t mst_plan_zero_floats(const mst_plan* p, int32_t mask) {
    if (!p) return MST_ERR_ARG;
    int64_t n = 0;
    if ((mask & MST_STAGE_ALL) == MST_STAGE_ALL) { for (auto& c : p->zero_all) n += c.len; return n; }
    for (int s = 0; s < 3; ++s) if ((mask >> s) & 1) for (auto& c : p->zero_stage[s]) n += c.len;
    return n;
}

extern "C" int32_t mst_plan_step_carried(const mst_plan* p, int32_t mask, int32_t backward, int32_t* carried) {
    if (!p || !carried) return MST_ERR_ARG;
    int n = 0;
    for (auto& s : p->list(mask, backward)) if (s.stage & mask) carried[n++] = !s.carried ? 0 : ((s.kind == K_SEGRED && s.b > 0) ? 2 : 1);
    return n;
}

extern "C" int32_t mst_plan_step_count(const mst_plan* p, int32_t mask, int32_t backward) {
    if (!p) return MST_ERR_ARG;
    int n = 0;
    for (auto& s : p->list(mask, backward)) if (s.stage & mask) ++n;
    return n;
}

extern "C" int32_t mst_plan_step_info(const mst_plan* p, int32_t mask, int32_t backward, int32_t* info ) {
    if (!p || !info) return MST_ERR_ARG;
    std::vector<const Step*> steps;
    for (auto& s : p->list(mask, backward)) if (s.stage & mask) steps.push_back(&s);
    int idx = 0;
    for (const Step* s : steps) {
        int32_t* o = info + 8 * idx++;
        o[0] = o[1] = o[2] = o[3] = 0; o[4] = s->count; o[5] = s->kind; o[6] = s->lvl; o[7] = s->chain;
        if (s->kind == K_GEMM || s->kind == K_GEMM_FOLD) { const GemmDesc& g = p->gemms.sched[s->first]; o[0] = g.M; o[1] = g.N; o[2] = g.K; o[3] = g.ksplit; }
        else if (KINDS[s->kind].fam == F_LIN) { const LinDesc& l = p->lins.host[s->first]; o[0] = l.rows; o[1] = l.N; o[2] = l.K; o[3] = l.splits; }
        else if (s->kind == K_LSTM_F || s->kind == K_LSTM_B) { const LstmDesc& l = p->lstms.sched[s->first]; o[0] = l.B; o[1] = l.S; o[2] = l.H; o[3] = l.multi; }
        else if (s->kind == K_GATHER) { const GatherDesc& g = p->gathers.sched[s->first]; o[0] = g.rows; o[1] = g.K; o[2] = g.nseg; }
        else if (s->kind == K_SEGRED) { const SegRedDesc& r = p->segreds.sched[s->first]; o[0] = s->a; o[1] = r.width; o[2] = r.d[0] * r.d[1] * r.d[2] * r.d[3]; }
        else if (s->kind == K_COMB_F || s->kind == K_COMB_B) { const CombineDesc& c = p->combines.sched[s->first]; o[0] = c.Cn; o[1] = c.rows; o[2] = c.cols; o[3] = c.nblk; }
    }
    return idx;
}

extern "C" int32_t mst_plan_step_gemms(const mst_plan* p, int32_t mask, int32_t backward, int32_t step, int32_t* out, int32_t cap) {
    if (!p || !out) return MST_ERR_ARG;
    int idx = 0;
    for (auto& s : p->list(mask, backward)) {
        if (!(s.stage & mask)) continue;
        if (idx++ != step) continue;
        if (s.kind != K_GEMM && s.kind != K_GEMM_FOLD) return 0;
        int n = 0;
        for (int q = 0; q < s.b && n < cap; ++q, ++n) {
            const GemmDesc& g = p->gemms.sched[s.first + q];
            int32_t* o = out + 6 * n;
            o[0] = g.M; o[1] = g.N; o[2] = g.K; o[3] = g.ksplit; o[4] = g.fold_rows; o[5] = gemm_blocks(g, p->mfma);
        }
        return n;
    }
    return MST_ERR_ARG;
}

extern "C" int32_t mst_plan_time_steps(const mst_plan* p, int32_t mask, int32_t backward, const float* params, float* gparams,
                                       float* ws, const float* pitched, const float* unpitched, mst_stream stream,
                                       int32_t reps, float* ms, int32_t* kind, double* flops, double* bytes) {
    if (!p || !params || !ws || !ms || !kind || !flops || !bytes || reps < 1) return MST_ERR_ARG;
    hipStream_t st = (hipStream_t)stream;
    Bases b = make_bases(p, params, gparams, ws, pitched, unpitched);
    if (backward && !p->tiled()) b.flags = MST_BF_LOSS_FUSED;
    if ((mask & MST_STAGE_ALL) == MST_STAGE_ALL) b.flags |= MST_BF_ALL_STAGES;
    hipEvent_t e0, e1;
    if (hipEventCreate(&e0) != hipSuccess || hipEventCreate(&e1) != hipSuccess) return MST_ERR_ALLOC;
    std::vector<const Step*> steps;
    for (auto& s : p->list(mask, backward)) if (s.stage & mask) steps.push_back(&s);
    int idx = 0;
    for (const Step* s : steps) {
        if (s->carried) {
            ms[idx] = 0.f; kind[idx] = s->kind;
            step_cost(p, *s, &flops[idx], &bytes[idx]);
            ++idx;
            continue;
        }
        run_step(p, *s, b, st);
        hipEventRecord(e0, st);
        for (int r = 0; r < reps; ++r) run_step(p, *s, b, st);
        hipEventRecord(e1, st);
        hipEventSynchronize(e1);
        float t = 0.f;
        hipEventElapsedTime(&t, e0, e1);
        ms[idx] = t / reps; kind[idx] = s->kind == K_GEMM_FOLD ? K_GEMM : s->kind;
        step_cost(p, *s, &flops[idx], &bytes[idx]);
        ++idx;
    }
    hipEventDestroy(e0); hipEventDestroy(e1);
    return idx;
}

extern "C" const char* mst_version(void) { return "mst_amd 0.1 (gfx950)"; }
```

### music-style-transfer_amd/style/_native.py

```python
import collections
import ctypes as C
import os

import torch

_HERE = os.path.dirname(os.path.abspath(__file__))
DEFAULT_LIB = os.path.join(os.path.dirname(_HERE), 'libmst_amd.so')

STAGE_EXTRACT, STAGE_INFO, STAGE_APPLY, STAGE_ALL = 1, 2, 4, 7
LOSS_SAVED = 512
LOSS_KEYS = [
    'total', 'channels_loss_total', 'channels_loss_pitched_total', 'channels_loss_pitched_notes_loss',
    'channels_loss_pitched_velocity_loss', 'channels_loss_pitched_duration_loss',
    'channels_loss_pitched_accidentals_loss', 'channels_loss_unpitched_total',
    'channels_loss_unpitched_notes_loss', 'channels_loss_unpitched_velocity_loss',
    'channels_loss_unpitched_duration_loss', 'song_info_loss_total', 'song_info_loss_instruments_loss',
    'song_info_loss_mode_loss', 'song_info_loss_bpm_loss',
]
N_LOSSES = len(LOSS_KEYS)


class MstError(RuntimeError):
    pass

# ... 9 lines not shown
class PlanOptions(C.Structure):
    _fields_ = [('gemm_tile', C.c_int32), ('no_merge', C.c_int32), ('gemm_run', C.c_int32), ('tile_r0', C.c_int32),
                ('tile_rows', C.c_int32), ('lstm_flavour', C.c_int32), ('dense_flavour', C.c_int32), ('branches', C.c_int32)]


DEV_LSTM_TIMEOUT = 1
ROLL_NONZERO, ROLL_HARD = 0, 1
WINDOW_WORDS = 4
METRIC_WORDS = 8


def describe_status(word):
    parts = []
    if word & DEV_LSTM_TIMEOUT:
        parts.append('a granule of the multi-workgroup LSTM exchange did not arrive within 0.2 s (MST_DEV_LSTM_TIMEOUT): the '
                     'launch was not fully resident — something else occupied the GPU next to a batched plan; results since then '
                     'are NaN.  Plan option lstm_flavour=1 (MST_LSTM_FLAVOUR=1) takes the single-workgroup kernels')
    if word & ~DEV_LSTM_TIMEOUT:
        parts.append(f'unknown status bits {word & ~DEV_LSTM_TIMEOUT:#x}')
    return '; '.join(parts)


def options_from_env():
    ge = os.environ.get('MST_GEMM')
    if ge not in (None, '', 'mfma', 'valu'):
        raise MstError(f'MST_GEMM={ge!r}: expected mfma or valu')
    return dict(gemm_tile={'mfma': 64, 'valu': 32}.get(ge, 0), no_merge=int(bool(os.environ.get('MST_NO_MERGE'))),
                gemm_run=int(os.environ.get('MST_GEMM_RUN', '0')), lstm_flavour=int(os.environ.get('MST_LSTM_FLAVOUR', '0')),
                dense_flavour=int(os.environ.get('MST_DENSE_FLAVOUR', '0')), branches=int(os.environ.get('MST_BRANCHES', '0')))


_P = C.c_void_p
_SIGS = {
    'mst_param_count': (C.c_int32, [C.POINTER(Dims)]),
    'mst_param_floats': (C.c_int64, [C.POINTER(Dims)]),
    'mst_param_info': (C.c_int32, [C.POINTER(Dims), C.c_int32, C.c_char_p, C.c_int32, C.POINTER(C.c_int64),
                                   C.POINTER(C.c_int32), C.POINTER(C.c_int32 * 3)]),
    'mst_widths_supported': (C.c_int32, [C.POINTER(Dims)]),
    'mst_plan_create': (_P, [C.POINTER(Dims), C.POINTER(C.c_int32)]),
    'mst_plan_create_ex': (_P, [C.POINTER(Dims), C.POINTER(PlanOptions), C.POINTER(C.c_int32)]),
    'mst_plan_gemm_tile': (C.c_int32, [_P]),
    'mst_plan_destroy': (None, [_P]),
    'mst_plan_workspace_floats': (C.c_int64, [_P]),
    'mst_plan_tensor': (C.c_int32, [_P, C.c_char_p, C.POINTER(C.c_int64), C.POINTER(C.c_int64), C.POINTER(C.c_int64)]),
    'mst_plan_launch_count': (C.c_int32, [_P, C.c_int32, C.c_int32]),
    'mst_plan_layout': (C.c_int32, [_P, C.POINTER(C.c_int64 * 4)]),
    'mst_plan_status': (C.c_int32, [_P, _P, C.c_int32, C.POINTER(C.c_int32), _P]),
    'mst_debug_slab_columns_disjoint': (C.c_int32, [C.c_int64, C.c_int32, C.c_int64, C.c_int32, C.c_int32]),
    'mst_forward': (C.c_int32, [_P, C.c_int32, _P, _P, _P, _P, _P]),
    'mst_backward': (C.c_int32, [_P, C.c_int32, _P, _P, _P, _P, _P, _P]),
    'mst_zero_grads': (C.c_int32, [_P, C.c_int32, _P, _P]),
    'mst_plan_zero_floats': (C.c_int64, [_P, C.c_int32]),
    'mst_loss_scratch_floats': (C.c_int64, []),
    'mst_total_loss_fwd': (C.c_int32, [_P, _P, C.c_int64, _P, _P, C.c_int64, _P, _P, C.c_int32, _P, _P, _P, _P,
                                       C.c_int32, _P, _P, _P, _P]),
    'mst_total_loss_bwd': (C.c_int32, [_P, _P, C.c_int64, _P, _P, C.c_int64, _P, _P, C.c_int32, _P, _P, _P, _P,
                                       _P, _P, _P, _P, _P, _P, _P, _P]),
    'mst_train_iteration': (C.c_int32, [_P, _P, _P, _P, _P, _P, _P, _P]),
    'mst_tiled_phase_count': (C.c_int32, [_P]),
    'mst_tiled_phase': (C.c_int32, [_P, C.c_int32, _P, _P, _P, _P, _P, _P, C.c_int32, _P, C.POINTER(C.c_int64 * 8), C.POINTER(C.c_int64 * 8),
                        C.POINTER(C.c_int32)]),
    'mst_adam_step': (C.c_int32, [_P, _P, _P, _P, C.c_int64, _P, C.c_double, C.c_double, C.c_double, C.c_double,
                                  C.c_int32, C.c_double, C.c_int32, _P]),
    'mst_adam_step2': (C.c_int32, [_P, _P, _P, _P, _P, C.c_int64, _P, C.c_double, C.c_double, C.c_double, C.c_double,
                                   C.c_int32, C.c_double, C.c_int32, _P]),
    'mst_grad_guard_scratch_bytes': (C.c_int64, [C.c_int64]),
    'mst_grad_norm': (C.c_int32, [_P, _P, C.c_int64, _P, _P, _P]),
    'mst_grad_norms': (C.c_int32, [_P, _P, _P, _P, C.c_int32, _P, _P]),
    'mst_adam_step_guarded': (C.c_int32, [_P, _P, _P, _P, _P, C.c_int64, _P, _P, _P, C.c_double, C.c_double, C.c_double, C.c_double,
                                          C.c_int32, C.c_double, C.c_double, C.c_int32, C.c_int32, _P]),
    'mst_hard_output': (C.c_int32, [_P, _P, C.c_int64, C.c_int32, _P]),
    'mst_clip_scatter': (C.c_int32, [_P, _P, _P, C.c_int32, C.c_int32, C.c_int64, C.c_int32, _P, _P]),
    'mst_clip_window': (C.c_int32, [_P, _P, _P, C.c_int32, C.c_int32, C.c_int32, C.c_int64, C.c_int32, _P, _P]),
    'mst_roll_slices': (C.c_int64, [C.c_int64]),
    'mst_roll_count': (C.c_int32, [_P, C.c_int64, C.c_int32, C.c_int32, _P, _P]),
    'mst_roll_compact': (C.c_int32, [_P, C.c_int64, C.c_int32, C.c_int32, _P, C.c_int64, _P, _P, _P]),
    'mst_roll_metrics_scratch_bytes': (C.c_int64, [C.c_int64, C.c_int64]),
    'mst_roll_metrics': (C.c_int32, [_P, _P, C.c_int64, C.c_int64, C.c_int32, _P, _P, _P]),
    'mst_eval_scratch_bytes': (C.c_int64, [_P]),
    'mst_eval_iteration': (C.c_int32, [_P, _P, _P, _P, _P, _P, _P, _P, _P]),
    'mst_plan_step_count': (C.c_int32, [_P, C.c_int32, C.c_int32]),
    'mst_plan_step_info': (C.c_int32, [_P, C.c_int32, C.c_int32, _P]),
    'mst_plan_step_carried': (C.c_int32, [_P, C.c_int32, C.c_int32, _P]),
    'mst_plan_step_gemms': (C.c_int32, [_P, C.c_int32, C.c_int32, C.c_int32, _P, C.c_int32]),
    'mst_plan_time_steps': (C.c_int32, [_P, C.c_int32, C.c_int32, _P, _P, _P, _P, _P, _P, C.c_int32, _P, _P, _P, _P]),
    'mst_audio_plan_create': (_P, [C.c_int32, C.c_int32, C.c_int64, C.POINTER(C.c_int32)]),
    'mst_audio_plan_destroy': (None, [_P]),
    'mst_audio_plan_info': (C.c_int32, [_P, C.POINTER(C.c_int64 * 6)]),
    'mst_audio_stft': (C.c_int32, [_P, _P, _P, _P, _P]),
    'mst_audio_gram': (C.c_int32, [_P, _P, _P, _P, _P]),
    'mst_audio_style_iteration': (C.c_int32, [_P, _P, _P, _P, _P, _P, _P, _P, _P, C.c_double, _P]),
    'mst_version': (C.c_char_p, []),
}


def ptr(t):
    if t is None:
        return None
    if t.dtype != torch.float32 or not t.is_contiguous():
        raise MstError('mst_amd kernels take contiguous float32 tensors')
    return t.data_ptr()


def check(status, what):
    if status != 0:
        names = {-1: 'MST_ERR_ARG', -2: 'MST_ERR_UNSUPPORTED', -3: 'MST_ERR_LAUNCH', -4: 'MST_ERR_ALLOC'}
        raise MstError(f'{what} failed: {names.get(status, status)}')


class Native:
    def __init__(self, path=None):
        path = path or DEFAULT_LIB
        if not os.path.exists(path):
            raise MstError(
                f'{path} not found: the HIP library has not been built. Run `python -c "import __graft_entry__ as g; '
                f'g.build()"` (hipcc --offload-arch=gfx950). There is no CPU fallback.')
        self.path = path
        self.lib = C.CDLL(path)
        for name, (res, args) in _SIGS.items():
            fn = getattr(self.lib, name)
            fn.restype, fn.argtypes = res, args
        self._plans = collections.OrderedDict()
        self._plan_cap = int(os.environ.get('MST_PLAN_CACHE', '16'))

    def param_table(self, dims):
        n = self.lib.mst_param_count(C.byref(dims))
        if n <= 0:
            raise MstError('bad dims')
        out = []
        buf = C.create_string_buffer(256)
        off, nd, shp = C.c_int64(), C.c_int32(), (C.c_int32 * 3)()
        for i in range(n):
            check(self.lib.mst_param_info(C.byref(dims), i, buf, 256, C.byref(off), C.byref(nd), C.byref(shp)), 'mst_param_info')
            out.append((buf.value.decode(), off.value, tuple(shp[k] for k in range(nd.value))))
        return out

    def param_floats(self, dims):
        return self.lib.mst_param_floats(C.byref(dims))

    def clip_scatter(self, cells, feats, counts, out, n_cells, nfeat, n_clips=1, capacity=None, stream=None):
        if capacity is None:
            capacity = cells.numel() // n_clips
        addr = lambda t: t if t is None or isinstance(t, int) else t.data_ptr()
        check(self.lib.mst_clip_scatter(addr(cells), addr(feats), addr(counts), int(capacity), int(n_clips), int(n_cells), int(nfeat),
                                        addr(out), stream), 'mst_clip_scatter')

    def clip_window(self, cells, feats, win, out, n_clips, channels, bars, bar_cells, nfeat, stream=None):
        addr = lambda t: t if t is None or isinstance(t, int) else t.data_ptr()
        check(self.lib.mst_clip_window(addr(cells), addr(feats), addr(win), int(n_clips), int(channels), int(bars), int(bar_cells),
                                       int(nfeat), addr(out), stream), 'mst_clip_window')

    def roll_slices(self, n_cells):
        n = self.lib.mst_roll_slices(int(n_cells))
        if n <= 0:
            raise MstError(f'mst_roll_slices({n_cells}): need 1 <= n_cells < 2**31')
        return n

    def roll_count(self, x, n_cells, nfeat, mode, ws, stream=None):
        addr = lambda t: t if t is None or isinstance(t, int) else t.data_ptr()
        check(self.lib.mst_roll_count(addr(x), int(n_cells), int(nfeat), int(mode), addr(ws), stream), 'mst_roll_count')

    def roll_compact(self, x, n_cells, nfeat, mode, ws, capacity, cells, feats, stream=None):
        addr = lambda t: t if t is None or isinstance(t, int) else t.data_ptr()
        check(self.lib.mst_roll_compact(addr(x), int(n_cells), int(nfeat), int(mode), addr(ws), int(capacity), addr(cells), addr(feats),
                                        stream), 'mst_roll_compact')

# ... 73 lines not shown
        return torch.zeros_like(self.ws)

    def acquire_ws(self):
        return self._free_ws.pop() if self._free_ws else self.new_ws()

    def release_ws(self, ws):
        if ws is not self.ws and len(self._free_ws) < self.WS_POOL_CAP:
            self._free_ws.append(ws)

    def view(self, name, shape=None, ws=None, clip=0):
        off, _, n = self.slot(name)
        off += clip * self.clip_stride
        t = (self.ws if ws is None else ws)[off:off + n]
        return t.view(*shape) if shape is not None else t

    def grad(self, name, shape=None, ws=None, clip=0):
        _, goff, n = self.slot(name)
        goff += clip * self.clip_stride
        t = (self.ws if ws is None else ws)[goff:goff + n]
        return t.view(*shape) if shape is not None else t

    def set_inputs(self, mode=None, bpm=None, instr=None, used=None, bpm_target=None, ws=None, clip=0):
        for name, t in (('mode', mode), ('bpm', bpm), ('instr', instr), ('used_instruments', used), ('bpm_target', bpm_target)):
            if t is not None:
                self.view(name, ws=ws, clip=clip).copy_(torch.as_tensor(t, dtype=torch.float32).reshape(-1), non_blocking=True)

    def status(self, ws=None, clear=True):
        word = C.c_int32()
        check(self.lib.mst_plan_status(self.handle, ptr(self.ws if ws is None else ws), int(bool(clear)), C.byref(word),
                                       current_stream(self.device)), 'mst_plan_status')
        return word.value

    def check_status(self, ws=None):
        word = self.status(ws)
        if word:
            raise MstError('device status: ' + describe_status(word))

    def _touch(self, ws):
        if self.branches and self.device.type == 'cuda' and torch.cuda.is_current_stream_capturing():
            raise MstError('a plan made with branches=1 cannot run under torch.cuda.graph capture; capture needs branches=0')
        ws = self.ws if ws is None else ws
        self._touched[id(ws)] = ws
        return ws

    def check_touched(self):
        touched, self._touched = self._touched, {}
        for ws in touched.values():
            self.check_status(ws)

    def launch_count(self, mask=STAGE_ALL, backward=False):
        return self.lib.mst_plan_launch_count(self.handle, mask, int(backward))

    def forward(self, mask, params, pitched, unpitched, ws=None):
        check(self.lib.mst_forward(self.handle, mask, ptr(params), ptr(self._touch(ws)), ptr(pitched),
                                   ptr(unpitched), current_stream(self.device)), 'mst_forward')

    def backward(self, mask, params, gparams, pitched, unpitched, ws=None):
        check(self.lib.mst_backward(self.handle, mask, ptr(params), ptr(gparams), ptr(self._touch(ws)),
                                    ptr(pitched), ptr(unpitched), current_stream(self.device)), 'mst_backward')

    def zero_grads(self, mask, ws=None):
        check(self.lib.mst_zero_grads(self.handle, mask, ptr(self.ws if ws is None else ws), current_stream(self.device)),
              'mst_zero_grads')

    def time_steps(self, mask, backward, params, gparams, pitched, unpitched, reps=20):
        import numpy as np
        n = self.lib.mst_plan_step_count(self.handle, mask, int(backward))
        ms, kind = np.zeros(n, np.float32), np.zeros(n, np.int32)
        fl, by = np.zeros(n, np.float64), np.zeros(n, np.float64)
        got = self.lib.mst_plan_time_steps(self.handle, mask, int(backward), ptr(params), ptr(gparams), ptr(self.ws),
                                           ptr(pitched), ptr(unpitched), current_stream(self.device), reps,
                                           ms.ctypes.data, kind.ctypes.data, fl.ctypes.data, by.ctypes.data)
        if got != n:
            check(got if got < 0 else -1, 'mst_plan_time_steps')
        return list(zip(kind.tolist(), ms.tolist(), fl.tolist(), by.tolist()))

    def step_carried(self, mask=STAGE_ALL, backward=False):
        import numpy as np
        n = self.lib.mst_plan_step_count(self.handle, mask, int(backward))
        out = np.zeros(n, np.int32)
        got = self.lib.mst_plan_step_carried(self.handle, mask, int(backward), out.ctypes.data)
        check(got if got < 0 else 0, 'mst_plan_step_carried')
        return out.tolist()

    def step_gemms(self, mask, backward, step, cap=2048):
        import numpy as np
        out = np.zeros((cap, 6), np.int32)
        n = self.lib.mst_plan_step_gemms(self.handle, mask, int(backward), step, out.ctypes.data, cap)
        check(n if n < 0 else 0, 'mst_plan_step_gemms')
        return [tuple(r) for r in out[:n].tolist()]

    def tiled_train_iteration(self, params, gparams, pitched, unpitched, losses=None, is_root=True, all_reduce=None):
        if all_reduce is None:
            import torch.distributed as dist
            all_reduce = lambda t: dist.all_reduce(t, op=dist.ReduceOp.SUM)
        xoff, xlen, nx = (C.c_int64 * 8)(), (C.c_int64 * 8)(), C.c_int32()
        self._touch(None)
        for ph in range(self.lib.mst_tiled_phase_count(self.handle)):
            check(self.lib.mst_tiled_phase(self.handle, ph, ptr(params), ptr(gparams), ptr(self.ws), ptr(pitched), ptr(unpitched),
                                           ptr(losses), int(bool(is_root)), current_stream(self.device), C.byref(xoff), C.byref(xlen),
                                           C.byref(nx)), f'mst_tiled_phase({ph})')
            if nx.value == 1:
                all_reduce(self.ws[xoff[0]:xoff[0] + xlen[0]])
            elif nx.value > 1:
                parts = [self.ws[xoff[q]:xoff[q] + xlen[q]] for q in range(nx.value)]
                total = sum(int(xlen[q]) for q in range(nx.value))
                if getattr(self, '_xstage', None) is None or self._xstage.numel() < total:
                    self._xstage = torch.empty(total, dtype=torch.float32, device=self.device)
                stage = self._xstage[:total]
                torch.cat(parts, out=stage)
                all_reduce(stage)
                at = 0
                for t in parts:
                    t.copy_(stage[at:at + t.numel()])
                    at += t.numel()

    def train_iteration(self, params, gparams, pitched, unpitched, losses=None, ws=None):
        check(self.lib.mst_train_iteration(self.handle, ptr(params), ptr(gparams), ptr(self._touch(ws)),
                                           ptr(pitched), ptr(unpitched), ptr(losses), current_stream(self.device)),
              'mst_train_iteration')

    def eval_scratch(self):
        if getattr(self, '_eval_scratch', None) is None:
            n = self.lib.mst_eval_scratch_bytes(self.handle)
            if n <= 0:
                check(int(n) or -1, 'mst_eval_scratch_bytes')
            self._eval_scratch = torch.zeros(n // 8, dtype=torch.float64, device=self.device)
        return self._eval_scratch

    def eval_iteration(self, params, pitched, unpitched, losses, metrics, ws=None):
        if metrics.dtype != torch.float64 or not metrics.is_contiguous() or \
                metrics.numel() != self.clips * (self.dims.C + 2) * METRIC_WORDS:
            raise MstError('eval_iteration: metrics must be a contiguous float64 tensor of clips x (C + 2) x 8')
        check(self.lib.mst_eval_iteration(self.handle, ptr(params), ptr(self._touch(ws)), ptr(pitched), ptr(unpitched), ptr(losses),
                                          metrics.data_ptr(), self.eval_scratch().data_ptr(), current_stream(self.device)),
              'mst_eval_iteration')


_native = None


def get():
    global _native
    if _native is None:
        _native = Native()
    return _native
```

Measured before the change: 2528 iters/s.

## Fold combine-norm kernels and gradient zeroing into preceding GEMM launches as riders

Moves the combine (column-norm weighted sum) kernel bodies into a shared header so the GEMM kernel can run small combine sites and the first phase of large ones as extra work alongside its own tiles. Gradient zeroing is also carried by a GEMM step instead of being a separate launch. The combine kernels gain a whole_small path and an MC=4 specialization. The aim is fewer kernel launches and fewer serialization points in the per-step graph. In exchange the GEMM kernel becomes more complex, which may raise register pressure or unbalance its blocks.

```diff
diff --git a/__graft_entry__.py b/__graft_entry__.py
--- a/__graft_entry__.py
+++ b/__graft_entry__.py
@@ -27,7 +27,7 @@
 def build(force=False):
     os.makedirs(BUILD, exist_ok=True)
     hipcc = _hipcc()
-    headers = [os.path.join(CSRC, 'mst_common.h'), os.path.join(ROOT, 'include', 'mst_amd.h')]
+    headers = [os.path.join(CSRC, 'mst_common.h'), os.path.join(CSRC, 'combine_body.h'), os.path.join(ROOT, 'include', 'mst_amd.h')]
     procs, objs = [], []
     for s in SOURCES:
         src, obj = os.path.join(CSRC, s + '.hip'), os.path.join(BUILD, s + '.o')
diff --git a/include/mst_amd.h b/include/mst_amd.h
--- a/include/mst_amd.h
+++ b/include/mst_amd.h
@@ -145,6 +145,8 @@
 int32_t mst_plan_step_count(const mst_plan* p, int32_t stage_mask, int32_t backward);
 int32_t mst_plan_step_info(const mst_plan* p, int32_t stage_mask, int32_t backward, int32_t* info );
 int32_t mst_plan_step_carried(const mst_plan* p, int32_t stage_mask, int32_t backward, int32_t* carried);
+int32_t mst_plan_step_riders(const mst_plan* p, int32_t stage_mask, int32_t backward, int32_t* out);
+int32_t mst_plan_zero_rides(const mst_plan* p);
 int32_t mst_plan_step_gemms(const mst_plan* p, int32_t stage_mask, int32_t backward, int32_t step, int32_t* out, int32_t cap);
 int32_t mst_plan_time_steps(const mst_plan* p, int32_t stage_mask, int32_t backward, const float* params,
                             float* gparams, float* ws, const float* pitched, const float* unpitched,
diff --git a/music-style-transfer_amd/csrc/combine.hip b/music-style-transfer_amd/csrc/combine.hip
--- a/music-style-transfer_amd/csrc/combine.hip
+++ b/music-style-transfer_amd/csrc/combine.hip
@@ -1,211 +1,61 @@
-#include "mst_common.h"
+#include "combine_body.h"
 
-template <int MC = COMBINE_MAXC>
-__device__ __forceinline__ void block_sum_multi(float* vals, int nv, float (*part)[COMBINE_MAXC + 1], float* red) {
-    const int lane = threadIdx.x & 63, wv = threadIdx.x >> 6;
-#pragma unroll
-    for (int v = 0; v <= MC; ++v) {
-        if (v < nv) {
-            float x = vals[v];
-#pragma unroll
-            for (int o = 32; o > 0; o >>= 1) x += __shfl_xor(x, o);
-            if (lane == 0) part[wv][v] = x;
-        }
-    }
-    __syncthreads();
-    if ((int)threadIdx.x < nv) red[threadIdx.x] = (part[0][threadIdx.x] + part[1][threadIdx.x]) + (part[2][threadIdx.x] + part[3][threadIdx.x]);
-    __syncthreads();
-}
-
-__device__ __forceinline__ int64_t elem_off(const CombineDesc& d, int e) {
-    const unsigned r = (unsigned)e / (unsigned)d.cols;
-    return (int64_t)r * d.ld + (int)((unsigned)e - r * (unsigned)d.cols);
-}
-
-__global__ __launch_bounds__(256) void combine_sumsq_kernel(const CombineDesc* __restrict__ descs, Bases b) {
+template <int MC>
+__global__ __launch_bounds__(256) void combine_sumsq_kernel(const CombineDesc* __restrict__ descs, Bases b, int whole_small) {
     const CombineDesc d = descs[blockIdx.y];
     if ((int)blockIdx.x >= d.nblk) return;
     __shared__ float part[4][COMBINE_MAXC + 1];
     __shared__ float red[COMBINE_MAXC + 1];
-    const float* x = b.p[SP_WS] + d.x_off;
-    const int64_t n = (int64_t)d.rows * d.cols;
-    float acc[COMBINE_MAXC + 1];
-#pragma unroll
-    for (int c = 0; c <= COMBINE_MAXC; ++c) acc[c] = 0.f;
-    for (int e = blockIdx.x * 256 + threadIdx.x; e < (int)n; e += d.nblk * 256) {
-        const int64_t eo = elem_off(d, e);
-#pragma unroll
-        for (int c = 0; c < COMBINE_MAXC; ++c) {
-            if (c < d.Cn) { const float v = x[(int64_t)c * d.cs + eo]; acc[c] = fmaf(v, v, acc[c]); }
-        }
+    if (whole_small && combine_site_small(d)) {
+        if (blockIdx.x == 0) combine_small_fwd_body<MC>(d, threadIdx.x, true, b, part, red);
+        return;
     }
-    block_sum_multi(acc, d.Cn, part, red);
-    if ((int)threadIdx.x < d.Cn) b.p[SP_TMP][d.part_off + blockIdx.x * (COMBINE_MAXC + 1) + threadIdx.x] = red[threadIdx.x];
+    combine_sumsq_body<MC>(d, blockIdx.x, threadIdx.x, true, b, part, red);
 }
 
-__global__ __launch_bounds__(256) void combine_apply_kernel(const CombineDesc* __restrict__ descs, Bases b) {
+template <int MC>
+__global__ __launch_bounds__(256) void combine_apply_kernel(const CombineDesc* __restrict__ descs, Bases b, int whole_small) {
+    const CombineDesc d = descs[blockIdx.y];
+    if ((int)blockIdx.x >= d.nblk || (whole_small && combine_site_small(d))) return;
+    __shared__ float part[4][COMBINE_MAXC + 1];
+    __shared__ float red[COMBINE_MAXC + 1];
+    combine_apply_body<MC>(d, blockIdx.x, threadIdx.x, b, part, red);
+}
+
+template <int MC>
+__global__ __launch_bounds__(256) void combine_bwd_reduce_kernel(const CombineDesc* __restrict__ descs, Bases b, int whole_small) {
     const CombineDesc d = descs[blockIdx.y];
     if ((int)blockIdx.x >= d.nblk) return;
-    __shared__ float nrm[COMBINE_MAXC + 1];
+    __shared__ float nc_s[COMBINE_MAXC + 1];
     __shared__ float part[4][COMBINE_MAXC + 1];
     __shared__ float red[COMBINE_MAXC + 1];
-    float* ws = b.p[SP_WS];
-    float* tmp = b.p[SP_TMP];
-    {
-        float vals[COMBINE_MAXC + 1];
-#pragma unroll
-        for (int c = 0; c <= COMBINE_MAXC; ++c)
-            vals[c] = (c < d.Cn && (int)threadIdx.x < d.nblk) ? tmp[d.part_off + threadIdx.x * (COMBINE_MAXC + 1) + c] : 0.f;
-        block_sum_multi(vals, d.Cn, part, red);
+    if (whole_small && combine_site_small(d)) {
+        if (blockIdx.x == 0) {
+            if (d.first) combine_small_bwd_body<MC, true>(d, threadIdx.x, true, b, red, nc_s, part);
+            else combine_small_bwd_body<MC, false>(d, threadIdx.x, true, b, red, nc_s, part);
+        }
+        return;
     }
-    if ((int)threadIdx.x < d.Cn) nrm[threadIdx.x] = sqrtf(1.f + red[threadIdx.x]);
-    __syncthreads();
-    if (threadIdx.x == 0) {
-        float S = 0.f;
-        for (int c = 0; c < d.Cn; ++c) S += nrm[c];
-        nrm[COMBINE_MAXC] = S;
-    }
-    __syncthreads();
-    if (blockIdx.x == 0 && (int)threadIdx.x <= d.Cn)
-        tmp[d.stats_off + threadIdx.x] = (int)threadIdx.x < d.Cn ? nrm[threadIdx.x] : nrm[COMBINE_MAXC];
-    const float S = nrm[COMBINE_MAXC];
-    const int64_t n = (int64_t)d.rows * d.cols;
-    for (int e = blockIdx.x * 256 + threadIdx.x; e < (int)n; e += d.nblk * 256) {
-        const int64_t eo = elem_off(d, e);
-        float acc = 0.f;
-        for (int c = 0; c < d.Cn; ++c) acc += ws[d.x_off + (int64_t)c * d.cs + eo] * nrm[c];
-        ws[d.out_off + e] = acc / S;
-    }
+    combine_bwd_reduce_body<MC>(d, blockIdx.x, threadIdx.x, true, b, part, red);
 }
 
-__global__ __launch_bounds__(256) void combine_bwd_reduce_kernel(const CombineDesc* __restrict__ descs, Bases b) {
+template <int MC>
+__global__ __launch_bounds__(256) void combine_bwd_apply_kernel(const CombineDesc* __restrict__ descs, Bases b, int whole_small) {
     const CombineDesc d = descs[blockIdx.y];
-    if ((int)blockIdx.x >= d.nblk) return;
-    __shared__ float part[4][COMBINE_MAXC + 1];
-    __shared__ float red[COMBINE_MAXC + 1];
-    const float* ws = b.p[SP_WS];
-    const float* gr = b.p[SP_GRAD];
-    const int64_t n = (int64_t)d.rows * d.cols;
-    float acc[COMBINE_MAXC + 1];
-#pragma unroll
-    for (int c = 0; c <= COMBINE_MAXC; ++c) acc[c] = 0.f;
-    for (int e = blockIdx.x * 256 + threadIdx.x; e < (int)n; e += d.nblk * 256) {
-        const int64_t eo = elem_off(d, e);
-        const float g = gr[d.gout_off + e];
-#pragma unroll
-        for (int c = 0; c < COMBINE_MAXC; ++c) {
-            if (c < d.Cn) acc[c] = fmaf(g, ws[d.x_off + (int64_t)c * d.cs + eo], acc[c]);
-        }
-        acc[COMBINE_MAXC] = fmaf(g, ws[d.out_off + e], acc[COMBINE_MAXC]);
-    }
-    float vals[COMBINE_MAXC + 1];
-#pragma unroll
-    for (int c = 0; c < COMBINE_MAXC; ++c) vals[c] = acc[c];
-    vals[COMBINE_MAXC] = 0.f;
-#pragma unroll
-    for (int c = 0; c <= COMBINE_MAXC; ++c) if (c == d.Cn) vals[c] = acc[COMBINE_MAXC];
-    block_sum_multi(vals, d.Cn + 1, part, red);
-    if ((int)threadIdx.x <= d.Cn) b.p[SP_TMP][d.part_off + blockIdx.x * (COMBINE_MAXC + 1) + threadIdx.x] = red[threadIdx.x];
-}
-
-__global__ __launch_bounds__(256) void combine_bwd_apply_kernel(const CombineDesc* __restrict__ descs, Bases b) {
-    const CombineDesc d = descs[blockIdx.y];
-    if ((int)blockIdx.x >= d.nblk) return;
+    if ((int)blockIdx.x >= d.nblk || (whole_small && combine_site_small(d))) return;
     __shared__ float coef[COMBINE_MAXC + 1];
     __shared__ float nc_s[COMBINE_MAXC + 1];
-    const float* ws = b.p[SP_WS];
-    float* gr = b.p[SP_GRAD];
-    const float* tmp = b.p[SP_TMP];
     __shared__ float part[4][COMBINE_MAXC + 1];
-    {
-        float vals[COMBINE_MAXC + 1];
-#pragma unroll
-        for (int c = 0; c <= COMBINE_MAXC; ++c)
-            vals[c] = (c <= d.Cn && (int)threadIdx.x < d.nblk) ? tmp[d.part_off + threadIdx.x * (COMBINE_MAXC + 1) + c] : 0.f;
-        block_sum_multi(vals, d.Cn + 1, part, coef);
-    }
-    if ((int)threadIdx.x <= d.Cn) nc_s[threadIdx.x] = tmp[d.stats_off + threadIdx.x];
-    __syncthreads();
-    const float S = nc_s[d.Cn];
-    const float bsum = coef[d.Cn];
-    __shared__ float fa_s[COMBINE_MAXC], fb_s[COMBINE_MAXC];
-    if ((int)threadIdx.x < d.Cn) {
-        const float nc = nc_s[threadIdx.x];
-        fa_s[threadIdx.x] = nc / S; fb_s[threadIdx.x] = ((coef[threadIdx.x] - bsum) / S) / nc;
-    }
-    __syncthreads();
-    const int64_t n = (int64_t)d.rows * d.cols;
-    for (int e = blockIdx.x * 256 + threadIdx.x; e < (int)n; e += d.nblk * 256) {
-        const int64_t eo = elem_off(d, e);
-        const float g = gr[d.gout_off + e];
-        for (int c = 0; c < d.Cn; ++c) {
-            const float x = ws[d.x_off + (int64_t)c * d.cs + eo];
-            float* gx = gr + d.gx_off + (int64_t)c * d.cs + eo;
-            const float v = fmaf(g, fa_s[c], fb_s[c] * x);
-            *gx = d.first ? v : *gx + v;
-        }
-    }
+    if (d.first) combine_bwd_apply_body<MC, true>(d, blockIdx.x, threadIdx.x, b, coef, nc_s, part);
+    else combine_bwd_apply_body<MC, false>(d, blockIdx.x, threadIdx.x, b, coef, nc_s, part);
 }
 
 template <int MC>
 __global__ __launch_bounds__(256) void combine_small_fwd_kernel(const CombineDesc* __restrict__ descs, Bases b) {
     const CombineDesc d = descs[blockIdx.x];
-    __shared__ float nrm[COMBINE_MAXC + 1];
     __shared__ float part[4][COMBINE_MAXC + 1];
     __shared__ float red[COMBINE_MAXC + 1];
-    float* ws = b.p[SP_WS];
-    float* tmp = b.p[SP_TMP];
-    const int n = d.rows * d.cols;
-    float acc[MC + 1];
-#pragma unroll
-    for (int c = 0; c <= MC; ++c) acc[c] = 0.f;
-    constexpr int U = MC <= 4 ? 4 : 1;
-    for (int e0 = threadIdx.x; e0 < n; e0 += 256 * U) {
-        float v[U][MC];
-#pragma unroll
-        for (int u = 0; u < U; ++u) {
-            const int e = e0 + 256 * u;
-            const bool ok = e < n;
-            const int64_t eo = elem_off(d, ok ? e : 0);
-#pragma unroll
-            for (int c = 0; c < MC; ++c) v[u][c] = (ok && c < d.Cn) ? ws[d.x_off + (int64_t)c * d.cs + eo] : 0.f;
-        }
-#pragma unroll
-        for (int u = 0; u < U; ++u) {
-#pragma unroll
-            for (int c = 0; c < MC; ++c) acc[c] = fmaf(v[u][c], v[u][c], acc[c]);
-        }
-    }
-    block_sum_multi<MC>(acc, d.Cn, part, red);
-    if ((int)threadIdx.x < d.Cn) nrm[threadIdx.x] = sqrtf(1.f + red[threadIdx.x]);
-    __syncthreads();
-    if (threadIdx.x == 0) {
-        float S = 0.f;
-        for (int c = 0; c < d.Cn; ++c) S += nrm[c];
-        nrm[COMBINE_MAXC] = S;
-    }
-    __syncthreads();
-    if ((int)threadIdx.x <= d.Cn) tmp[d.stats_off + threadIdx.x] = (int)threadIdx.x < d.Cn ? nrm[threadIdx.x] : nrm[COMBINE_MAXC];
-    const float S = nrm[COMBINE_MAXC];
-    for (int e0 = threadIdx.x; e0 < n; e0 += 256 * U) {
-        float v[U][MC];
-#pragma unroll
-        for (int u = 0; u < U; ++u) {
-            const int e = e0 + 256 * u;
-            const bool ok = e < n;
-            const int64_t eo = elem_off(d, ok ? e : 0);
-#pragma unroll
-            for (int c = 0; c < MC; ++c) v[u][c] = (ok && c < d.Cn) ? ws[d.x_off + (int64_t)c * d.cs + eo] : 0.f;
-        }
-#pragma unroll
-        for (int u = 0; u < U; ++u) {
-            const int e = e0 + 256 * u;
-            float a = 0.f;
-#pragma unroll
-            for (int c = 0; c < MC; ++c) if (c < d.Cn) a += v[u][c] * nrm[c];
-            if (e < n) ws[d.out_off + e] = a / S;
-        }
-    }
+    combine_small_fwd_body<MC>(d, threadIdx.x, true, b, part, red);
 }
 
 template <int MC>
@@ -214,112 +64,40 @@
     __shared__ float coef[COMBINE_MAXC + 1];
     __shared__ float nc_s[COMBINE_MAXC + 1];
     __shared__ float part[4][COMBINE_MAXC + 1];
-    const float* ws = b.p[SP_WS];
-    float* gr = b.p[SP_GRAD];
-    const float* tmp = b.p[SP_TMP];
-    const int n = d.rows * d.cols;
-    float acc[MC + 1];
-#pragma unroll
-    for (int c = 0; c <= MC; ++c) acc[c] = 0.f;
-    constexpr int U = MC <= 4 ? 4 : 1;
-    for (int e0 = threadIdx.x; e0 < n; e0 += 256 * U) {
-        float v[U][MC], g[U], o[U];
-#pragma unroll
-        for (int u = 0; u < U; ++u) {
-            const int e = e0 + 256 * u;
-            const bool ok = e < n;
-            const int64_t eo = elem_off(d, ok ? e : 0);
-            g[u] = ok ? gr[d.gout_off + e] : 0.f;
-            o[u] = ok ? ws[d.out_off + e] : 0.f;
-#pragma unroll
-            for (int c = 0; c < MC; ++c) v[u][c] = (ok && c < d.Cn) ? ws[d.x_off + (int64_t)c * d.cs + eo] : 0.f;
-        }
-#pragma unroll
-        for (int u = 0; u < U; ++u) {
-            if (e0 + 256 * u < n) {
-#pragma unroll
-                for (int c = 0; c < MC; ++c) if (c < d.Cn) acc[c] = fmaf(g[u], v[u][c], acc[c]);
-                acc[MC] = fmaf(g[u], o[u], acc[MC]);
-            }
-        }
-    }
-    float vals[MC + 1];
-#pragma unroll
-    for (int c = 0; c < MC; ++c) vals[c] = acc[c];
-    vals[MC] = 0.f;
-#pragma unroll
-    for (int c = 0; c <= MC; ++c) if (c == d.Cn) vals[c] = acc[MC];
-    block_sum_multi<MC>(vals, d.Cn + 1, part, coef);
-    if ((int)threadIdx.x <= d.Cn) nc_s[threadIdx.x] = tmp[d.stats_off + threadIdx.x];
-    __syncthreads();
-    const float S = nc_s[d.Cn];
-    const float bsum = coef[d.Cn];
-    float fa[MC], fb[MC];
-#pragma unroll
-    for (int c = 0; c < MC; ++c) {
-        const float nc = c < d.Cn ? nc_s[c] : 1.f;
-        fa[c] = nc / S; fb[c] = c < d.Cn ? ((coef[c] - bsum) / S) / nc : 0.f;
-    }
-    for (int e0 = threadIdx.x; e0 < n; e0 += 256 * U) {
-        float x[U][MC], old[U][MC], g[U];
-        int64_t eo[U];
-#pragma unroll
-        for (int u = 0; u < U; ++u) {
-            const int e = e0 + 256 * u;
-            const bool ok = e < n;
-            eo[u] = elem_off(d, ok ? e : 0);
-            g[u] = ok ? gr[d.gout_off + e] : 0.f;
-#pragma unroll
-            for (int c = 0; c < MC; ++c) {
-                const bool okc = ok && c < d.Cn;
-                x[u][c] = okc ? ws[d.x_off + (int64_t)c * d.cs + eo[u]] : 0.f;
-                old[u][c] = (okc && !d.first) ? gr[d.gx_off + (int64_t)c * d.cs + eo[u]] : 0.f;
-            }
-        }
-#pragma unroll
-        for (int u = 0; u < U; ++u) {
-            if (e0 + 256 * u < n) {
-#pragma unroll
-                for (int c = 0; c < MC; ++c) {
-                    if (c < d.Cn) {
-                        const float v = fmaf(g[u], fa[c], fb[c] * x[u][c]);
-                        gr[d.gx_off + (int64_t)c * d.cs + eo[u]] = d.first ? v : old[u][c] + v;
-                    }
-                }
-            }
-        }
-    }
+    if (d.first) combine_small_bwd_body<MC, true>(d, threadIdx.x, true, b, coef, nc_s, part);
+    else combine_small_bwd_body<MC, false>(d, threadIdx.x, true, b, coef, nc_s, part);
 }
 
-int launch_combine_fwd(const CombineDesc* dev, int count, int max_nblk, int all_small, Bases b, hipStream_t s) {
+int launch_combine_fwd(const CombineDesc* dev, int count, int max_nblk, int all_small, int mc4, Bases b, hipStream_t s) {
     if (count <= 0) return 0;
     if (all_small) {
         if (all_small == 2) hipLaunchKernelGGL(combine_small_fwd_kernel<4>, dim3(count), dim3(256), 0, s, dev, b);
         else hipLaunchKernelGGL(combine_small_fwd_kernel<COMBINE_MAXC>, dim3(count), dim3(256), 0, s, dev, b);
         return (int)hipGetLastError();
     }
-    hipLaunchKernelGGL(combine_sumsq_kernel, dim3(max_nblk, count), dim3(256), 0, s, dev, b);
-    hipLaunchKernelGGL(combine_apply_kernel, dim3(max_nblk, count), dim3(256), 0, s, dev, b);
-    return (int)hipGetLastError();
+    if (int e = launch_combine_phase(dev, max_nblk, 0, b, s, count, mc4, 1)) return e;
+    return launch_combine_phase(dev, max_nblk, 1, b, s, count, mc4, 1);
 }
 
-int launch_combine_bwd(const CombineDesc* dev, int count, int max_nblk, int all_small, Bases b, hipStream_t s) {
+int launch_combine_bwd(const CombineDesc* dev, int count, int max_nblk, int all_small, int mc4, Bases b, hipStream_t s) {
     if (count <= 0) return 0;
     if (all_small) {
         if (all_small == 2) hipLaunchKernelGGL(combine_small_bwd_kernel<4>, dim3(count), dim3(256), 0, s, dev, b);
         else hipLaunchKernelGGL(combine_small_bwd_kernel<COMBINE_MAXC>, dim3(count), dim3(256), 0, s, dev, b);
         return (int)hipGetLastError();
     }
-    hipLaunchKernelGGL(combine_bwd_reduce_kernel, dim3(max_nblk, count), dim3(256), 0, s, dev, b);
-    hipLaunchKernelGGL(combine_bwd_apply_kernel, dim3(max_nblk, count), dim3(256), 0, s, dev, b);
-    return (int)hipGetLastError();
+    if (int e = launch_combine_phase(dev, max_nblk, 2, b, s, count, mc4, 1)) return e;
+    return launch_combine_phase(dev, max_nblk, 3, b, s, count, mc4, 1);
 }
 
-int launch_combine_phase(const CombineDesc* dev, int nblk, int which, Bases b, hipStream_t s) {
-    if (which == 0) hipLaunchKernelGGL(combine_sumsq_kernel, dim3(nblk, 1), dim3(256), 0, s, dev, b);
-    else if (which == 1) hipLaunchKernelGGL(combine_apply_kernel, dim3(nblk, 1), dim3(256), 0, s, dev, b);
-    else if (which == 2) hipLaunchKernelGGL(combine_bwd_reduce_kernel, dim3(nblk, 1), dim3(256), 0, s, dev, b);
-    else hipLaunchKernelGGL(combine_bwd_apply_kernel, dim3(nblk, 1), dim3(256), 0, s, dev, b);
+int launch_combine_phase(const CombineDesc* dev, int nblk, int which, Bases b, hipStream_t s, int count, int mc4, int whole_small) {
+    const dim3 grid(nblk, count), lanes(256);
+#define COMBINE_PHASE(K) do { if (mc4) hipLaunchKernelGGL(K<4>, grid, lanes, 0, s, dev, b, whole_small); else hipLaunchKernelGGL(K<COMBINE_MAXC>, grid, lanes, 0, s, dev, b, whole_small); } while (0)
+    if (which == 0) COMBINE_PHASE(combine_sumsq_kernel);
+    else if (which == 1) COMBINE_PHASE(combine_apply_kernel);
+    else if (which == 2) COMBINE_PHASE(combine_bwd_reduce_kernel);
+    else COMBINE_PHASE(combine_bwd_apply_kernel);
+#undef COMBINE_PHASE
     return (int)hipGetLastError();
 }
 
diff --git a/music-style-transfer_amd/csrc/combine_body.h b/music-style-transfer_amd/csrc/combine_body.h
--- /dev/null
+++ b/music-style-transfer_amd/csrc/combine_body.h
@@ -0,0 +1,336 @@
+#pragma once
+#include "mst_common.h"
+
+typedef const MST_GLOBAL_AS float* comb_gptr;
+template <int MC> struct CombineTrips { static constexpr int U = MC <= 4 ? 4 : 1; };
+
+template <int MC = COMBINE_MAXC>
+__device__ __forceinline__ void block_sum_multi(float* vals, int nv, float (*part)[COMBINE_MAXC + 1], float* red, const int t, const bool live = true) {
+    const int lane = t & 63, wv = t >> 6;
+#pragma unroll
+    for (int v = 0; v <= MC; ++v) {
+        if (MC <= 4 || v < nv) {
+            float x = vals[v];
+#pragma unroll
+            for (int o = 32; o > 0; o >>= 1) x += __shfl_xor(x, o);
+            if (lane == 0 && live && v < nv) part[wv][v] = x;
+        }
+    }
+    __syncthreads();
+    if (t < nv && live) red[t] = (part[0][t] + part[1][t]) + (part[2][t] + part[3][t]);
+    __syncthreads();
+}
+
+__device__ __forceinline__ int64_t elem_off(const CombineDesc& d, int e) {
+    const unsigned r = (unsigned)e / (unsigned)d.cols;
+    return (int64_t)r * d.ld + (int)((unsigned)e - r * (unsigned)d.cols);
+}
+
+__device__ __forceinline__ bool combine_site_small(const CombineDesc& d) { return (int64_t)d.rows * d.cols <= COMBINE_SMALL; }
+
+template <int MC, int U>
+__device__ __forceinline__ void combine_load_x(const CombineDesc& d, comb_gptr x, const unsigned e0, const unsigned stride, const unsigned n,
+                                               float (&v)[U][MC], int64_t (&eo)[U]) {
+#pragma unroll
+    for (int u = 0; u < U; ++u) {
+        const unsigned e = e0 + u * stride;
+        eo[u] = elem_off(d, e < n ? (int)e : 0);
+    }
+#pragma unroll
+    for (int u = 0; u < U; ++u) {
+#pragma unroll
+        for (int c = 0; c < MC; ++c) {
+            if (MC <= 4) v[u][c] = x[(int64_t)(c < d.Cn ? c : 0) * d.cs + eo[u]];
+            else v[u][c] = c < d.Cn ? x[(int64_t)c * d.cs + eo[u]] : 0.f;
+        }
+    }
+}
+
+template <int MC>
+__device__ __forceinline__ void combine_sumsq_body(const CombineDesc& d, const int blk, const int t, const bool live, const Bases& b,
+                                                   float (*part)[COMBINE_MAXC + 1], float* red) {
+    constexpr int U = CombineTrips<MC>::U;
+    comb_gptr x = (comb_gptr)b.p[SP_WS] + d.x_off;
+    const unsigned n = live ? (unsigned)(d.rows * d.cols) : 0u, stride = (unsigned)d.nblk * 256u;
+    float acc[MC + 1];
+#pragma unroll
+    for (int c = 0; c <= MC; ++c) acc[c] = 0.f;
+    for (unsigned e0 = (unsigned)blk * 256u + t; e0 < n; e0 += stride * U) {
+        float v[U][MC];
+        int64_t eo[U];
+        combine_load_x<MC, U>(d, x, e0, stride, n, v, eo);
+#pragma unroll
+        for (int u = 0; u < U; ++u) {
+            const bool ok = e0 + u * stride < n;
+#pragma unroll
+            for (int c = 0; c < MC; ++c) acc[c] = (ok && c < d.Cn) ? fmaf(v[u][c], v[u][c], acc[c]) : acc[c];
+        }
+    }
+    block_sum_multi<MC>(acc, d.Cn, part, red, t, live);
+    if (live && t < d.Cn) b.p[SP_TMP][d.part_off + blk * (COMBINE_MAXC + 1) + t] = red[t];
+}
+
+template <int MC>
+__device__ __forceinline__ void combine_norms(const CombineDesc& d, const float* red, float (&nc)[MC], float& S) {
+    S = 0.f;
+#pragma unroll
+    for (int c = 0; c < MC; ++c) {
+        nc[c] = c < d.Cn ? sqrtf(1.f + red[c]) : 0.f;
+        if (c < d.Cn) S += nc[c];
+    }
+}
+
+template <int MC>
+__device__ __forceinline__ void combine_load_partials(const CombineDesc& d, comb_gptr tmp, const int t, const int nv, float (&vals)[MC + 1]) {
+    comb_gptr p = tmp + d.part_off + (t < d.nblk ? t : 0) * (COMBINE_MAXC + 1);
+#pragma unroll
+    for (int c = 0; c <= MC; ++c) {
+        if (MC <= 4) vals[c] = p[c < nv ? c : 0];
+        else vals[c] = c < nv ? p[c] : 0.f;
+    }
+#pragma unroll
+    for (int c = 0; c <= MC; ++c) vals[c] = (c < nv && t < d.nblk) ? vals[c] : 0.f;
+}
+
+template <int MC>
+__device__ __forceinline__ void combine_apply_body(const CombineDesc& d, const int blk, const int t, const Bases& b,
+                                                   float (*part)[COMBINE_MAXC + 1], float* red) {
+    constexpr int U = CombineTrips<MC>::U;
+    float* ws = b.p[SP_WS];
+    float* tmp = b.p[SP_TMP];
+    comb_gptr x = (comb_gptr)ws + d.x_off;
+    const unsigned n = (unsigned)(d.rows * d.cols), stride = (unsigned)d.nblk * 256u;
+    unsigned e0 = (unsigned)blk * 256u + t;
+    float v[U][MC];
+    int64_t eo[U];
+    {
+        float vals[MC + 1];
+        combine_load_x<MC, U>(d, x, e0, stride, n, v, eo);
+        combine_load_partials<MC>(d, (comb_gptr)tmp, t, d.Cn, vals);
+        MST_SCHED_FENCE();
+        block_sum_multi<MC>(vals, d.Cn, part, red, t);
+    }
+    float nc[MC], S;
+    combine_norms<MC>(d, red, nc, S);
+    if (blk == 0 && t <= d.Cn) tmp[d.stats_off + t] = t < d.Cn ? sqrtf(1.f + red[t]) : S;
+    while (e0 < n) {
+#pragma unroll
+        for (int u = 0; u < U; ++u) {
+            const unsigned e = e0 + u * stride;
+            float a = 0.f;
+#pragma unroll
+            for (int c = 0; c < MC; ++c) if (c < d.Cn) a += v[u][c] * nc[c];
+            if (e < n) ws[d.out_off + e] = a / S;
+        }
+        e0 += stride * U;
+        if (e0 < n) combine_load_x<MC, U>(d, x, e0, stride, n, v, eo);
+    }
+}
+
+template <int MC>
+__device__ __forceinline__ void combine_bwd_reduce_body(const CombineDesc& d, const int blk, const int t, const bool live, const Bases& b,
+                                                        float (*part)[COMBINE_MAXC + 1], float* red) {
+    constexpr int U = CombineTrips<MC>::U;
+    comb_gptr x = (comb_gptr)b.p[SP_WS] + d.x_off;
+    comb_gptr out = (comb_gptr)b.p[SP_WS] + d.out_off;
+    comb_gptr go = (comb_gptr)b.p[SP_GRAD] + d.gout_off;
+    const unsigned n = live ? (unsigned)(d.rows * d.cols) : 0u, stride = (unsigned)d.nblk * 256u;
+    float acc[MC + 1];
+#pragma unroll
+    for (int c = 0; c <= MC; ++c) acc[c] = 0.f;
+    for (unsigned e0 = (unsigned)blk * 256u + t; e0 < n; e0 += stride * U) {
+        float v[U][MC], g[U], o[U];
+        int64_t eo[U];
+#pragma unroll
+        for (int u = 0; u < U; ++u) {
+            const unsigned e = e0 + u * stride, ec = e < n ? e : 0u;
+            g[u] = go[ec];
+            o[u] = out[ec];
+        }
+        combine_load_x<MC, U>(d, x, e0, stride, n, v, eo);
+#pragma unroll
+        for (int u = 0; u < U; ++u) {
+            const bool ok = e0 + u * stride < n;
+#pragma unroll
+            for (int c = 0; c < MC; ++c) acc[c] = (ok && c < d.Cn) ? fmaf(g[u], v[u][c], acc[c]) : acc[c];
+            acc[MC] = ok ? fmaf(g[u], o[u], acc[MC]) : acc[MC];
+        }
+    }
+    float vals[MC + 1];
+#pragma unroll
+    for (int c = 0; c < MC; ++c) vals[c] = acc[c];
+    vals[MC] = 0.f;
+#pragma unroll
+    for (int c = 0; c <= MC; ++c) if (c == d.Cn) vals[c] = acc[MC];
+    block_sum_multi<MC>(vals, d.Cn + 1, part, red, t, live);
+    if (live && t <= d.Cn) b.p[SP_TMP][d.part_off + blk * (COMBINE_MAXC + 1) + t] = red[t];
+}
+
+template <int MC, int U, bool FIRST>
+__device__ __forceinline__ void combine_load_bwd(const CombineDesc& d, comb_gptr x, comb_gptr go, comb_gptr gx, const unsigned e0, const unsigned stride,
+                                                 const unsigned n, float (&v)[U][MC], float (&old)[U][MC], float (&g)[U], int64_t (&eo)[U]) {
+#pragma unroll
+    for (int u = 0; u < U; ++u) {
+        const unsigned e = e0 + u * stride;
+        g[u] = go[e < n ? e : 0u];
+    }
+    combine_load_x<MC, U>(d, x, e0, stride, n, v, eo);
+    if (!FIRST) combine_load_x<MC, U>(d, gx, e0, stride, n, old, eo);
+}
+
+template <int MC, bool FIRST>
+__device__ __forceinline__ void combine_bwd_apply_body(const CombineDesc& d, const int blk, const int t, const Bases& b,
+                                                       float* coef, float* nc_s, float (*part)[COMBINE_MAXC + 1]) {
+    constexpr int U = CombineTrips<MC>::U;
+    float* gr = b.p[SP_GRAD];
+    comb_gptr tmp = (comb_gptr)b.p[SP_TMP];
+    comb_gptr x = (comb_gptr)b.p[SP_WS] + d.x_off;
+    comb_gptr go = (comb_gptr)gr + d.gout_off;
+    comb_gptr gx = (comb_gptr)gr + d.gx_off;
+    const unsigned n = (unsigned)(d.rows * d.cols), stride = (unsigned)d.nblk * 256u;
+    unsigned e0 = (unsigned)blk * 256u + t;
+    float v[U][MC], old[U][MC], g[U];
+    int64_t eo[U];
+    {
+        float vals[MC + 1];
+        combine_load_bwd<MC, U, FIRST>(d, x, go, gx, e0, stride, n, v, old, g, eo);
+        combine_load_partials<MC>(d, tmp, t, d.Cn + 1, vals);
+        const float st = tmp[d.stats_off + (t <= d.Cn ? t : 0)];
+        MST_SCHED_FENCE();
+        if (t <= d.Cn) nc_s[t] = st;
+        block_sum_multi<MC>(vals, d.Cn + 1, part, coef, t);
+    }
+    const float S = nc_s[d.Cn];
+    const float bsum = coef[d.Cn];
+    float fa[MC], fb[MC];
+#pragma unroll
+    for (int c = 0; c < MC; ++c) {
+        const float nc = c < d.Cn ? nc_s[c] : 1.f;
+        fa[c] = nc / S; fb[c] = c < d.Cn ? ((coef[c] - bsum) / S) / nc : 0.f;
+    }
+    while (e0 < n) {
+#pragma unroll
+        for (int u = 0; u < U; ++u) {
+            if (e0 + u * stride < n) {
+#pragma unroll
+                for (int c = 0; c < MC; ++c) {
+                    if (c < d.Cn) {
+                        const float w = fmaf(g[u], fa[c], fb[c] * v[u][c]);
+                        gr[d.gx_off + (int64_t)c * d.cs + eo[u]] = FIRST ? w : old[u][c] + w;
+                    }
+                }
+            }
+        }
+        e0 += stride * U;
+        if (e0 < n) combine_load_bwd<MC, U, FIRST>(d, x, go, gx, e0, stride, n, v, old, g, eo);
+    }
+}
+
+template <int MC>
+__device__ __forceinline__ void combine_small_fwd_body(const CombineDesc& d, const int t, const bool live, const Bases& b,
+                                                       float (*part)[COMBINE_MAXC + 1], float* red) {
+    constexpr int U = CombineTrips<MC>::U;
+    float* ws = b.p[SP_WS];
+    float* tmp = b.p[SP_TMP];
+    comb_gptr x = (comb_gptr)ws + d.x_off;
+    const unsigned n = live ? (unsigned)(d.rows * d.cols) : 0u;
+    float acc[MC + 1];
+#pragma unroll
+    for (int c = 0; c <= MC; ++c) acc[c] = 0.f;
+    for (unsigned e0 = t; e0 < n; e0 += 256 * U) {
+        float v[U][MC];
+        int64_t eo[U];
+        combine_load_x<MC, U>(d, x, e0, 256u, n, v, eo);
+#pragma unroll
+        for (int u = 0; u < U; ++u) {
+            const bool ok = e0 + 256 * u < n;
+#pragma unroll
+            for (int c = 0; c < MC; ++c) acc[c] = (ok && c < d.Cn) ? fmaf(v[u][c], v[u][c], acc[c]) : acc[c];
+        }
+    }
+    block_sum_multi<MC>(acc, d.Cn, part, red, t, live);
+    float nc[MC], S;
+    combine_norms<MC>(d, red, nc, S);
+    if (live && t <= d.Cn) tmp[d.stats_off + t] = t < d.Cn ? sqrtf(1.f + red[t]) : S;
+    for (unsigned e0 = t; e0 < n; e0 += 256 * U) {
+        float v[U][MC];
+        int64_t eo[U];
+        combine_load_x<MC, U>(d, x, e0, 256u, n, v, eo);
+#pragma unroll
+        for (int u = 0; u < U; ++u) {
+            const unsigned e = e0 + 256 * u;
+            float a = 0.f;
+#pragma unroll
+            for (int c = 0; c < MC; ++c) if (c < d.Cn) a += v[u][c] * nc[c];
+            if (e < n) ws[d.out_off + e] = a / S;
+        }
+    }
+}
+
+template <int MC, bool FIRST>
+__device__ __forceinline__ void combine_small_bwd_body(const CombineDesc& d, const int t, const bool live, const Bases& b,
+                                                       float* coef, float* nc_s, float (*part)[COMBINE_MAXC + 1]) {
+    constexpr int U = CombineTrips<MC>::U;
+    float* gr = b.p[SP_GRAD];
+    comb_gptr tmp = (comb_gptr)b.p[SP_TMP];
+    comb_gptr x = (comb_gptr)b.p[SP_WS] + d.x_off;
+    comb_gptr out = (comb_gptr)b.p[SP_WS] + d.out_off;
+    comb_gptr go = (comb_gptr)gr + d.gout_off;
+    comb_gptr gx = (comb_gptr)gr + d.gx_off;
+    const unsigned n = live ? (unsigned)(d.rows * d.cols) : 0u;
+    const float st = live ? tmp[d.stats_off + (t <= d.Cn ? t : 0)] : 0.f;
+    float acc[MC + 1];
+#pragma unroll
+    for (int c = 0; c <= MC; ++c) acc[c] = 0.f;
+    for (unsigned e0 = t; e0 < n; e0 += 256 * U) {
+        float v[U][MC], g[U], o[U];
+        int64_t eo[U];
+#pragma unroll
+        for (int u = 0; u < U; ++u) {
+            const unsigned e = e0 + 256 * u, ec = e < n ? e : 0u;
+            g[u] = go[ec];
+            o[u] = out[ec];
+        }
+        combine_load_x<MC, U>(d, x, e0, 256u, n, v, eo);
+#pragma unroll
+        for (int u = 0; u < U; ++u) {
+            const bool ok = e0 + 256 * u < n;
+#pragma unroll
+            for (int c = 0; c < MC; ++c) acc[c] = (ok && c < d.Cn) ? fmaf(g[u], v[u][c], acc[c]) : acc[c];
+            acc[MC] = ok ? fmaf(g[u], o[u], acc[MC]) : acc[MC];
+        }
+    }
+    float vals[MC + 1];
+#pragma unroll
+    for (int c = 0; c < MC; ++c) vals[c] = acc[c];
+    vals[MC] = 0.f;
+#pragma unroll
+    for (int c = 0; c <= MC; ++c) if (c == d.Cn) vals[c] = acc[MC];
+    if (live && t <= d.Cn) nc_s[t] = st;
+    block_sum_multi<MC>(vals, d.Cn + 1, part, coef, t, live);
+    const float S = nc_s[d.Cn];
+    const float bsum = coef[d.Cn];
+    float fa[MC], fb[MC];
+#pragma unroll
+    for (int c = 0; c < MC; ++c) {
+        const float nc = c < d.Cn ? nc_s[c] : 1.f;
+        fa[c] = nc / S; fb[c] = c < d.Cn ? ((coef[c] - bsum) / S) / nc : 0.f;
+    }
+    for (unsigned e0 = t; e0 < n; e0 += 256 * U) {
+        float v[U][MC], old[U][MC], g[U];
+        int64_t eo[U];
+        combine_load_bwd<MC, U, FIRST>(d, x, go, gx, e0, 256u, n, v, old, g, eo);
+#pragma unroll
+        for (int u = 0; u < U; ++u) {
+            if (e0 + 256 * u < n) {
+#pragma unroll
+                for (int c = 0; c < MC; ++c) {
+                    if (c < d.Cn) {
+                        const float w = fmaf(g[u], fa[c], fb[c] * v[u][c]);
+                        gr[d.gx_off + (int64_t)c * d.cs + eo[u]] = FIRST ? w : old[u][c] + w;
+                    }
+                }
+            }
+        }
+    }
+}
diff --git a/music-style-transfer_amd/csrc/gemm.hip b/music-style-transfer_amd/csrc/gemm.hip
--- a/music-style-transfer_amd/csrc/gemm.hip
+++ b/music-style-transfer_amd/csrc/gemm.hip
@@ -1,4 +1,4 @@
-#include "mst_common.h"
+#include "combine_body.h"
 
 __device__ __forceinline__ float act_fwd(int act, float z, int col) {
     if (act == ACT_LEAKY) return z > 0.f ? z : z * LEAKY;
@@ -614,29 +614,73 @@
     return ((ntile + run - 1) / run) * g.ksplit;
 }
 
+__device__ __forceinline__ void combine_rider(const CombineDesc d, const int cb, int kind, const Bases& b, float* smem) {
+    constexpr int ROW = COMBINE_MAXC + 1;
+    const int tid = threadIdx.x;
+    if ((kind == COMB_RIDE_SUMSQ || kind == COMB_RIDE_REDUCE) && combine_site_small(d)) {
+        if (cb != 0) return;
+        kind = kind == COMB_RIDE_SUMSQ ? COMB_RIDE_SMALL_F : COMB_RIDE_SMALL_B;
+    }
+    if (kind == COMB_RIDE_SMALL_F) {
+        combine_small_fwd_body<4>(d, tid, tid < 256, b, reinterpret_cast<float (*)[ROW]>(smem), smem + 4 * ROW);
+    } else if (kind == COMB_RIDE_SMALL_B) {
+        if (d.first) combine_small_bwd_body<4, true>(d, tid, tid < 256, b, smem, smem + ROW, reinterpret_cast<float (*)[ROW]>(smem + 2 * ROW));
+        else combine_small_bwd_body<4, false>(d, tid, tid < 256, b, smem, smem + ROW, reinterpret_cast<float (*)[ROW]>(smem + 2 * ROW));
+    } else {
+        const int gi = tid >> 8, grp = cb * 4 + gi;
+        float* slice = smem + gi * 5 * ROW;
+        if (kind == COMB_RIDE_SUMSQ) combine_sumsq_body<4>(d, grp, tid & 255, grp < d.nblk, b, reinterpret_cast<float (*)[ROW]>(slice), slice + 4 * ROW);
+        else combine_bwd_reduce_body<4>(d, grp, tid & 255, grp < d.nblk, b, reinterpret_cast<float (*)[ROW]>(slice), slice + 4 * ROW);
+    }
+}
+
 template <int WV> __device__ __forceinline__ void gather_rows(const GatherDesc& d, const int blk, const int nblk, const Bases& b);
 __device__ __forceinline__ void segred_group(const SegRedDesc* __restrict__ descs, const int members, const int clip, const int lb, const int t, const Bases& b);
 
-__global__ __launch_bounds__(GEMM_THREADS) void gemm_kernel(const GemmDesc* __restrict__ descs, const int* __restrict__ owner, int count, int blocks_per_clip, Bases b, GemmRiders r) {
+__device__ __forceinline__ void gemm_rider_block(const GemmRiders& r, const int clip, int lb, const Bases& b, float* smem) {
+    const int seg_blocks = (r.seg_groups + 3) >> 2, gat_blocks = r.gat_members * r.gat_blocks;
+#pragma unroll
+    for (int q = 0; q < 2; ++q) {
+        const GemmRiders::Comb& cr = r.comb[q];
+        const int comb_blocks = cr.sites * cr.blocks;
+        if (lb < comb_blocks) {
+            const int m = lb / cr.blocks;
+            combine_rider(cr.descs[clip * cr.sites + m], lb - m * cr.blocks, cr.kind, b, smem);
+            return;
+        }
+        lb -= comb_blocks;
+    }
+    if (lb < seg_blocks) {
+        const int grp = lb * 4 + (threadIdx.x >> 8);
+        if (grp < r.seg_groups) segred_group(r.segreds, r.seg_members, clip, grp, threadIdx.x & 255, b);
+        return;
+    }
+    lb -= seg_blocks;
+    if (lb < gat_blocks) {
+        const int m = lb / r.gat_blocks;
+        gather_rows<GATHER_RIDER_ROWS>(r.gathers[clip * r.gat_members + m], lb - m * r.gat_blocks, r.gat_blocks, b);
+        return;
+    }
+    lb -= gat_blocks;
+    if (lb < r.zero_chunks) {
+        const ZeroChunk c = r.zero[lb];
+        float* p = b.p[SP_GRAD] + (int64_t)clip * r.zero_stride + c.off;
+        for (int i = threadIdx.x; i < c.len; i += GEMM_THREADS) p[i] = 0.f;
+    }
+}
+
+__global__ __launch_bounds__(GEMM_THREADS) void gemm_kernel(const GemmDesc* __restrict__ descs, const int* __restrict__ owner, int count, int blocks_per_clip, int rider_blocks, Bases b, GemmRiders r) {
     constexpr int TILE_F = GEMM_BK * (GEMM_BM + GEMM_PAD), RED_F = (GEMM_THREADS / 64) * GEMM_BM * GEMM_BN;
     __shared__ float smem[(2 * TILE_F > RED_F) ? 2 * TILE_F : RED_F];
     float (*As)[GEMM_BM + GEMM_PAD] = reinterpret_cast<float (*)[GEMM_BM + GEMM_PAD]>(smem);
     float (*Bs)[GEMM_BN + GEMM_PAD] = reinterpret_cast<float (*)[GEMM_BN + GEMM_PAD]>(smem + TILE_F);
     const int clip = blockIdx.x / blocks_per_clip;
     int lb = blockIdx.x - clip * blocks_per_clip;
-    const int seg_blocks = (r.seg_groups + 3) >> 2, gat_blocks = r.gat_members * r.gat_blocks;
-    if (lb < seg_blocks) {
-        const int grp = lb * 4 + (threadIdx.x >> 8);
-        if (grp < r.seg_groups) segred_group(r.segreds, r.seg_members, clip, grp, threadIdx.x & 255, b);
+    if (lb < rider_blocks) {
+        gemm_rider_block(r, clip, lb, b, smem);
         return;
     }
-    lb -= seg_blocks;
-    if (lb < gat_blocks) {
-        const int m = lb / r.gat_blocks;
-        gather_rows<GATHER_RIDER_ROWS>(r.gathers[clip * r.gat_members + m], lb - m * r.gat_blocks, r.gat_blocks, b);
-        return;
-    }
-    lb -= gat_blocks;
+    lb -= rider_blocks;
     const int lo = owner[lb];
     const GemmDesc d = descs[clip * count + lo];
     const int local = lb - d.blk_begin;
@@ -675,7 +719,7 @@
     return -1;
 }
 
-int gemm_rider_blocks(const GemmRiders& r) { return (r.seg_groups + 3) / 4 + r.gat_members * r.gat_blocks; }
+int gemm_rider_blocks(const GemmRiders& r) { return r.comb[0].sites * r.comb[0].blocks + r.comb[1].sites * r.comb[1].blocks + (r.seg_groups + 3) / 4 + r.gat_members * r.gat_blocks + r.zero_chunks; }
 
 int launch_gemm(const GemmDesc* dev_descs, const int* dev_owner, int members, int blocks_per_clip, int clips, int mfma, Bases b, hipStream_t s, const GemmRiders* riders) {
     if (members <= 0 || blocks_per_clip <= 0 || clips <= 0) return 0;
@@ -683,7 +727,7 @@
     if (mfma && gemm_rider_blocks(r)) return (int)hipErrorInvalidValue;
     blocks_per_clip += gemm_rider_blocks(r);
     if (mfma) hipLaunchKernelGGL(gemm_mfma_kernel, dim3(blocks_per_clip * clips), dim3(MF_THREADS), 0, s, dev_descs, dev_owner, members, blocks_per_clip, b);
-    else hipLaunchKernelGGL(gemm_kernel, dim3(blocks_per_clip * clips), dim3(GEMM_THREADS), 0, s, dev_descs, dev_owner, members, blocks_per_clip, b, r);
+    else hipLaunchKernelGGL(gemm_kernel, dim3(blocks_per_clip * clips), dim3(GEMM_THREADS), 0, s, dev_descs, dev_owner, members, blocks_per_clip, gemm_rider_blocks(r), b, r);
     return (int)hipGetLastError();
 }
 
diff --git a/music-style-transfer_amd/csrc/mst_common.h b/music-style-transfer_amd/csrc/mst_common.h
--- a/music-style-transfer_amd/csrc/mst_common.h
+++ b/music-style-transfer_amd/csrc/mst_common.h
@@ -125,9 +125,14 @@
     int64_t y_off;
 };
 
+struct CombineDesc;
+struct ZeroChunk;
+enum { COMB_RIDE_NONE = 0, COMB_RIDE_SMALL_F, COMB_RIDE_SMALL_B, COMB_RIDE_SUMSQ, COMB_RIDE_REDUCE };
 struct GemmRiders {
     const SegRedDesc* segreds; int32_t seg_members, seg_groups;
     const GatherDesc* gathers; int32_t gat_members, gat_blocks;
+    struct Comb { const CombineDesc* descs; int32_t sites, blocks, kind; } comb[2];
+    const ZeroChunk* zero; int32_t zero_chunks; int64_t zero_stride;
 };
 
 struct LstmDesc {
@@ -251,7 +256,7 @@
 struct FoldDesc { int32_t space, nrows, row_stride, ncols, col_stride, pad; int64_t part_off, sum_off ; };
 int launch_copy_rows(const CopyDesc* dev, const CopyDesc& host, int backward, Bases b, hipStream_t s);
 int launch_fold(const FoldDesc* dev, int spread, Bases b, hipStream_t s);
-int launch_combine_phase(const CombineDesc* dev, int nblk, int which, Bases b, hipStream_t s);
+int launch_combine_phase(const CombineDesc* dev, int nblk, int which, Bases b, hipStream_t s, int count = 1, int mc4 = 0, int whole_small = 0);
 
 struct SlabEntry { int64_t dst, src, stride; int32_t count, splits; int32_t reps; int64_t rep_stride; int32_t width, dst_ld; int32_t single;
                    int64_t base;  };
@@ -282,8 +287,8 @@
 int launch_lstm_fwd(const LstmDesc* dev_descs, int count, int maxB, int maxH, int multi, Bases b, hipStream_t s);
 int launch_lstm_bwd(const LstmDesc* dev_descs, int count, int maxB, int maxH, int multi, Bases b, hipStream_t s);
 int lstm_multi_blocks_per_cu();
-int launch_combine_fwd(const CombineDesc* dev_descs, int count, int max_nblk, int all_small, Bases b, hipStream_t s);
-int launch_combine_bwd(const CombineDesc* dev_descs, int count, int max_nblk, int all_small, Bases b, hipStream_t s);
+int launch_combine_fwd(const CombineDesc* dev_descs, int count, int max_nblk, int all_small, int mc4, Bases b, hipStream_t s);
+int launch_combine_bwd(const CombineDesc* dev_descs, int count, int max_nblk, int all_small, int mc4, Bases b, hipStream_t s);
 int launch_me_sumsq(const NotesDesc* dev, const NotesDesc& host, int count, Bases b, hipStream_t s);
 int launch_me_notes_fwd(const NotesDesc* dev, const NotesDesc& host, int count, Bases b, hipStream_t s);
 int launch_me_bwd_reduce(const NotesDesc* dev, const NotesDesc& host, int count, Bases b, hipStream_t s);
diff --git a/music-style-transfer_amd/csrc/plan.hip b/music-style-transfer_amd/csrc/plan.hip
--- a/music-style-transfer_amd/csrc/plan.hip
+++ b/music-style-transfer_amd/csrc/plan.hip
@@ -220,7 +220,8 @@
     void release() { hipFree(dev); dev = nullptr; }
 };
 
-struct Riders { int seg_first = 0, seg_members = 0, seg_groups = 0, seg_stage2 = 0, gat_first = 0, gat_members = 0, gat_rows = 0; };
+struct CombRide { int first = 0, sites = 0, nblk = 0, bwd = 0; };
+struct Riders { int seg_first = 0, seg_members = 0, seg_groups = 0, seg_stage2 = 0, gat_first = 0, gat_members = 0, gat_rows = 0; CombRide comb[2]; };
 struct Step { int kind, first, count, a, b, stage; int c = 0; int lvl = 0; int chain = -1; int signal = -1; int wait[3] = {-1, -1, -1};
               int carried = 0; Riders ride; };
 struct Acc { int space; int64_t lo, hi; bool w; bool accum = false, dense = true; };
@@ -255,12 +256,15 @@
 
     bool tiled() const { return opt.tile_rows > 0; }
     bool mixes() const { return !mfma && !tiled() && opt.branches != 1 && !opt.no_merge; }
+    int mc4() const { return d.C <= 4 ? 1 : 0; }
     int Rl() const { return tiled() ? opt.tile_rows : d.R; }
     int P() const { return d.C * Rl() * d.T; }
     int Q() const { return Rl() * d.T; }
     struct Xchg { int space; int64_t off; int32_t len; };
     std::vector<Xchg> xchgs;
     bool tags_in_zero = false;
+    int zero_ride = -1;
+    void find_zero_ride();
     std::vector<ZeroChunk> zero_fwd; ZeroChunk* d_zero_fwd = nullptr;
     int64_t loss_sum_off = 0;
     int loss_fold[2] = {-1, -1};
@@ -1351,13 +1355,15 @@
         }
         if (!mixes()) continue;
         for (size_t e = lv_begin; e < out.size(); ++e) {
-            if (out[e].kind != K_GATHER && out[e].kind != K_SEGRED) continue;
+            const bool comb = (out[e].kind == K_COMB_F || out[e].kind == K_COMB_B) && mc4();
+            if (out[e].kind != K_GATHER && out[e].kind != K_SEGRED && !comb) continue;
             for (size_t c = lv_begin; c < out.size(); ++c) {
                 Step& g = out[c];
                 if (g.kind != K_GEMM || (!across_stages && g.stage != out[e].stage)) continue;
                 const Step& s = out[e];
                 if (s.kind == K_GATHER && !g.ride.gat_members) { g.ride.gat_first = s.first; g.ride.gat_members = s.count / K(); g.ride.gat_rows = s.a; }
                 else if (s.kind == K_SEGRED && !g.ride.seg_members) { g.ride.seg_first = s.first; g.ride.seg_members = s.count / K(); g.ride.seg_groups = s.a; g.ride.seg_stage2 = s.b; }
+                else if (comb && !g.ride.comb[s.b != 0].sites) g.ride.comb[s.b != 0] = CombRide{s.first, s.count / K(), s.a, s.kind == K_COMB_B};
                 else continue;
                 out[e].carried = 1;
                 break;
@@ -1501,6 +1507,7 @@
     if (K() == 1)
         for (const LstmDesc& l : lstms.host)
             if (l.multi) { zero_all.push_back(ZeroChunk{act_top + l.xch_off, (int32_t)(2 * (2 * l.H + 8 * l.H)), 0}); tags_in_zero = true; }
+    find_zero_ride();
     if (!tiled()) return;
     {
         const bool U = d.has_unpitched != 0;
@@ -1548,6 +1555,33 @@
     split(1);
 }
 
+void mst_plan::find_zero_ride() {
+    zero_ride = -1;
+    if (!mixes() || zero_all.empty()) return;
+    const std::vector<Step>& L = sched_all[0];
+    int first = -1;
+    for (int i = 0; i < (int)L.size() && first < 0; ++i) {
+        if (L[i].carried) continue;
+        if (tags_in_zero && L[i].kind == K_LSTM_T && lstms.sched[L[i].first].multi) continue;
+        first = i;
+    }
+    if (first < 0 || L[first].kind != K_GEMM) return;
+    auto base = [&](int space) -> int64_t { return space == SP_WS ? 0 : space == SP_GRAD ? (int64_t)K() * act_top : space == SP_TMP ? 2 * (int64_t)K() * act_top : -1; };
+    std::vector<Acc> acc;
+    accesses(L[first], acc, true);
+    for (const Step& s : L) if (s.carried && s.lvl == L[first].lvl) accesses(s, acc, true);
+    for (const Acc& a : acc) {
+        const int64_t ab = base(a.space);
+        if (ab < 0) continue;
+        for (int k = 0; k < K(); ++k)
+            for (const ZeroChunk& c : zero_all) {
+                const int64_t lo = base(SP_GRAD) + shift(SP_GRAD, k) + c.off;
+                if (ab + a.lo < lo + c.len && lo < ab + a.hi) return;
+            }
+    }
+    zero_ride = first;
+}
+
 static bool slab_columns_disjoint(int64_t off_x, int width_x, int64_t off_y, int width_y, int ld) {
     const int64_t cx = off_x % ld, cy = off_y % ld;
     if (cx + width_x > ld || cy + width_y > ld) return false;
@@ -1683,27 +1717,37 @@
     return b;
 }
 
-static int run_step(const mst_plan* p, const Step& s, const Bases& b, hipStream_t st) {
+static int run_step(const mst_plan* p, const Step& s, const Bases& b, hipStream_t st, bool with_zero = false) {
     if (s.carried) return 0;
     switch (s.kind) {
     case K_GEMM: case K_GEMM_FOLD: {
         const Riders& q = s.ride;
         const int clips = s.count / s.b, gat_blocks = std::min(512, (q.gat_rows + GATHER_RIDER_ROWS - 1) / GATHER_RIDER_ROWS);
-        const GemmRiders r{p->segreds.dev + q.seg_first, q.seg_members, q.seg_groups, p->gathers.dev + q.gat_first, q.gat_members, gat_blocks};
-        const int e = launch_gemm(p->gemms.dev + s.first, p->d_gemm_owner + s.c, s.b, s.a, clips, p->mfma, b, st, &r);
-        return e ? e : launch_segred2(p->segreds.dev + q.seg_first, q.seg_members * clips, q.seg_stage2, b, st);
+        GemmRiders r{p->segreds.dev + q.seg_first, q.seg_members, q.seg_groups, p->gathers.dev + q.gat_first, q.gat_members, gat_blocks};
+        for (int large = 0; large < 2; ++large) {
+            const CombRide& c = q.comb[large];
+            if (!c.sites) continue;
+            r.comb[large] = {p->combines.dev + c.first, c.sites, large ? (c.nblk + 3) / 4 : 1,
+                             large ? (c.bwd ? COMB_RIDE_REDUCE : COMB_RIDE_SUMSQ) : (c.bwd ? COMB_RIDE_SMALL_B : COMB_RIDE_SMALL_F)};
+        }
+        if (with_zero) { r.zero = p->d_zero_all; r.zero_chunks = (int)p->zero_all.size(); r.zero_stride = p->act_top; }
+        int e = launch_gemm(p->gemms.dev + s.first, p->d_gemm_owner + s.c, s.b, s.a, clips, p->mfma, b, st, &r);
+        if (!e) e = launch_segred2(p->segreds.dev + q.seg_first, q.seg_members * clips, q.seg_stage2, b, st);
+        if (!e && q.comb[1].sites)
+            e = launch_combine_phase(p->combines.dev + q.comb[1].first, q.comb[1].nblk, q.comb[1].bwd ? 3 : 1, b, st, q.comb[1].sites * clips, 1, 1);
+        return e;
     }
     case K_GATHER: return launch_gather(p->gathers.dev + s.first, s.count, s.a, b, st);
     case K_SEGRED: return launch_segred(p->segreds.dev + s.first, s.count / p->K(), s.a, p->K(), s.b, b, st);
     case K_LSTM_T: return launch_lstm_transpose(p->lstms.dev + s.first, s.count, s.b, p->lstms.sched[s.first].multi, b, st);
     case K_LSTM_F: return launch_lstm_fwd(p->lstms.dev + s.first, s.count, s.a, s.b, p->lstms.sched[s.first].multi, b, st);
     case K_LSTM_B: return launch_lstm_bwd(p->lstms.dev + s.first, s.count, s.a, s.b, p->lstms.sched[s.first].multi, b, st);
-    case K_COMB_F: return launch_combine_fwd(p->combines.dev + s.first, s.count, s.a, s.b == 0 ? (p->d.C <= 4 ? 2 : 1) : 0, b, st);
-    case K_COMB_B: return launch_combine_bwd(p->combines.dev + s.first, s.count, s.a, s.b == 0 ? (p->d.C <= 4 ? 2 : 1) : 0, b, st);
-    case K_COMB_F1: return launch_combine_phase(p->combines.dev + s.first, s.a, 0, b, st);
-    case K_COMB_F2: return launch_combine_phase(p->combines.dev + s.first, s.a, 1, b, st);
-    case K_COMB_B1: return launch_combine_phase(p->combines.dev + s.first, s.a, 2, b, st);
-    case K_COMB_B2: return launch_combine_phase(p->combines.dev + s.first, s.a, 3, b, st);
+    case K_COMB_F: return launch_combine_fwd(p->combines.dev + s.first, s.count, s.a, s.b == 0 ? (p->mc4() ? 2 : 1) : 0, p->mc4(), b, st);
+    case K_COMB_B: return launch_combine_bwd(p->combines.dev + s.first, s.count, s.a, s.b == 0 ? (p->mc4() ? 2 : 1) : 0, p->mc4(), b, st);
+    case K_COMB_F1: return launch_combine_phase(p->combines.dev + s.first, s.a, 0, b, st, 1, p->mc4());
+    case K_COMB_F2: return launch_combine_phase(p->combines.dev + s.first, s.a, 1, b, st, 1, p->mc4());
+    case K_COMB_B1: return launch_combine_phase(p->combines.dev + s.first, s.a, 2, b, st, 1, p->mc4());
+    case K_COMB_B2: return launch_combine_phase(p->combines.dev + s.first, s.a, 3, b, st, 1, p->mc4());
     case K_COPY_F: return launch_copy_rows(p->copies.dev + s.first, p->copies.host[s.first], 0, b, st);
     case K_COPY_B: return launch_copy_rows(p->copies.dev + s.first, p->copies.host[s.first], 1, b, st);
     case K_FOLD: return launch_fold(p->folds.dev + s.first, 0, b, st);
@@ -1731,7 +1775,8 @@
     return MST_ERR_ARG;
 }
 
-static int run_pass(const mst_plan* p, const std::vector<Step>& list, int mask, const Bases& b0, hipStream_t main, bool tags_cleared = false) {
+static int run_pass(const mst_plan* p, const std::vector<Step>& list, int mask, const Bases& b0, hipStream_t main, bool tags_cleared = false,
+                    int zero_step = -1 ) {
     Bases b = b0;
     if (mask == MST_STAGE_ALL) b.flags |= MST_BF_ALL_STAGES;
     auto runs = [&](const Step& s) {
@@ -1754,7 +1799,7 @@
             for (int w = 0; w < 3; ++w)
                 if (s.wait[w] >= 0 && hipStreamWaitEvent(st, ss->ev[s.wait[w]], 0) != hipSuccess) return MST_ERR_LAUNCH;
         }
-        int e = run_step(p, s, b, st);
+        int e = run_step(p, s, b, st, zero_step >= 0 && &s == &list[zero_step]);
         if (e) return e < 0 ? e : MST_ERR_LAUNCH;
         if (ss && s.signal >= 0 && hipEventRecord(ss->ev[s.signal], st) != hipSuccess) return MST_ERR_LAUNCH;
     }
@@ -1826,10 +1871,10 @@
                                        const float* pitched, const float* unpitched, float* losses, mst_stream stream) {
     if (!p || !params || !gparams || !ws || !pitched) return MST_ERR_ARG;
     hipStream_t st = (hipStream_t)stream;
-    int e = mst_zero_grads(p, MST_STAGE_ALL, ws, stream);
+    int e = p->zero_ride >= 0 ? 0 : mst_zero_grads(p, MST_STAGE_ALL, ws, stream);
     if (e) return e;
     if (p->d.has_unpitched && !unpitched) return MST_ERR_ARG;
-    e = run_pass(p, p->list(MST_STAGE_ALL, 0), MST_STAGE_ALL, make_bases(p, params, nullptr, ws, pitched, unpitched), st, p->tags_in_zero);
+    e = run_pass(p, p->list(MST_STAGE_ALL, 0), MST_STAGE_ALL, make_bases(p, params, nullptr, ws, pitched, unpitched), st, p->tags_in_zero, p->zero_ride);
     if (e) return e;
     const bool U = p->d.has_unpitched != 0;
     const int K = p->K();
@@ -2050,9 +2095,23 @@
 extern "C" int32_t mst_plan_step_carried(const mst_plan* p, int32_t mask, int32_t backward, int32_t* carried) {
     if (!p || !carried) return MST_ERR_ARG;
     int n = 0;
-    for (auto& s : p->list(mask, backward)) if (s.stage & mask) carried[n++] = !s.carried ? 0 : ((s.kind == K_SEGRED && s.b > 0) ? 2 : 1);
+    for (auto& s : p->list(mask, backward))
+        if (s.stage & mask) carried[n++] = (!s.carried || (s.kind != K_GATHER && s.kind != K_SEGRED)) ? 0 : ((s.kind == K_SEGRED && s.b > 0) ? 2 : 1);
     return n;
 }
+
+extern "C" int32_t mst_plan_step_riders(const mst_plan* p, int32_t mask, int32_t backward, int32_t* out) {
+    if (!p || !out) return MST_ERR_ARG;
+    int n = 0;
+    for (auto& s : p->list(mask, backward)) {
+        if (!(s.stage & mask)) continue;
+        const bool two = (s.kind == K_SEGRED && s.b > 0) || ((s.kind == K_COMB_F || s.kind == K_COMB_B) && s.b != 0);
+        out[n++] = !s.carried ? 0 : (two ? 2 : 1);
+    }
+    return n;
+}
+
+extern "C" int32_t mst_plan_zero_rides(const mst_plan* p) { return !p ? MST_ERR_ARG : (p->zero_ride >= 0 ? 1 : 0); }
 
 extern "C" int32_t mst_plan_step_count(const mst_plan* p, int32_t mask, int32_t backward) {
     if (!p) return MST_ERR_ARG;
diff --git a/music-style-transfer_amd/style/_native.py b/music-style-transfer_amd/style/_native.py
--- a/music-style-transfer_amd/style/_native.py
+++ b/music-style-transfer_amd/style/_native.py
@@ -115,6 +115,8 @@
     'mst_plan_step_count': (C.c_int32, [_P, C.c_int32, C.c_int32]),
     'mst_plan_step_info': (C.c_int32, [_P, C.c_int32, C.c_int32, _P]),
     'mst_plan_step_carried': (C.c_int32, [_P, C.c_int32, C.c_int32, _P]),
+    'mst_plan_step_riders': (C.c_int32, [_P, C.c_int32, C.c_int32, _P]),
+    'mst_plan_zero_rides': (C.c_int32, [_P]),
     'mst_plan_step_gemms': (C.c_int32, [_P, C.c_int32, C.c_int32, C.c_int32, _P, C.c_int32]),
     'mst_plan_time_steps': (C.c_int32, [_P, C.c_int32, C.c_int32, _P, _P, _P, _P, _P, _P, C.c_int32, _P, _P, _P, _P]),
     'mst_audio_plan_create': (_P, [C.c_int32, C.c_int32, C.c_int64, C.POINTER(C.c_int32)]),
@@ -354,6 +356,19 @@
         got = self.lib.mst_plan_step_carried(self.handle, mask, int(backward), out.ctypes.data)
         check(got if got < 0 else 0, 'mst_plan_step_carried')
         return out.tolist()
+
+    def step_riders(self, mask=STAGE_ALL, backward=False):
+        import numpy as np
+        n = self.lib.mst_plan_step_count(self.handle, mask, int(backward))
+        out = np.zeros(n, np.int32)
+        got = self.lib.mst_plan_step_riders(self.handle, mask, int(backward), out.ctypes.data)
+        check(got if got < 0 else 0, 'mst_plan_step_riders')
+        return out.tolist()
+
+    def zero_rides(self):
+        got = self.lib.mst_plan_zero_rides(self.handle)
+        check(got if got < 0 else 0, 'mst_plan_zero_rides')
+        return got
 
     def step_gemms(self, mask, backward, step, cap=2048):
         import numpy as np
```

Measured after the change: 2749 iters/s (median of 6 runs). 1.09x the previous value.
